# amathislab/HOISDF

Hardware: AMD Instinct MI355X
Metric: samples/sec (img + 2048 SDF queries) fwd+bwd at 1/2/4/8 MI355X (higher is better)
Workload: dtype f32 (emulated contractions, f32 accumulate, f16x2 form: operands as scaled hi + lo f16 pieces x 3 products - 22 operand bits, one power-of-two scale per ROW of a linear layer's row operand, per (sample, head) of the attention operands, per weight matrix; the attention backward's dS as three pieces x

## Files before the change

### hoisdf_amd/_lib.py

```python
from __future__ import annotations

import ctypes as C
import os
from typing import Dict, List

_HERE = os.path.dirname(os.path.abspath(__file__))
LIB_PATH = os.environ.get("HOISDF_LIB", os.path.join(_HERE, "libhoisdf_hip.so"))
HEADER_PATH = os.path.join(os.path.dirname(_HERE), "include", "hoisdf.h")
MAX_LEVELS = 8


class HoisdfLibraryError(RuntimeError):
    pass


class HoisdfError(RuntimeError):
    def __init__(self, code: int, msg: str):
        super().__init__(f"libhoisdf_hip status {code}: {msg}")
        self.code = code


class Pyramid(C.Structure):
    _fields_ = [("n_levels", C.c_int), ("B", C.c_int), ("data", C.c_void_p * MAX_LEVELS),
                ("C", C.c_int * MAX_LEVELS), ("H", C.c_int * MAX_LEVELS), ("W", C.c_int * MAX_LEVELS)]
# ... 7 lines not shown
                ("emu_img", C.c_void_p * 6), ("emu_img_t", C.c_void_p * 6)]


class EncoderLayerDesc(C.Structure):
    _fields_ = [("B", C.c_int), ("S", C.c_int), ("E", C.c_int), ("F", C.c_int), ("H", C.c_int), ("n_query", C.c_int),
                ("n_inter", C.c_int), ("eps", C.c_float), ("drop_p", C.c_float), ("seed", C.c_uint64 * 4), ("attention", C.c_int),
                ("attention_bwd_emulated", C.c_int), ("training", C.c_int), ("x_mag", C.c_void_p)]


_ENC_W = ("w_in", "b_in", "w_out", "b_out", "g1", "be1", "w1", "b1", "w2", "b2", "g2", "be2", "g3", "be3")
_ENC_IMG = ("img_in", "img_in_q", "img_in_kv", "img_out", "img_1", "img_2")


class EncoderLayerWeights(C.Structure):
    _fields_ = [(n, C.c_void_p) for n in _ENC_W + _ENC_IMG + tuple(n.replace("img_", "img_t_") for n in _ENC_IMG)]


class DecoderLayerDesc(C.Structure):
    _fields_ = [("B", C.c_int), ("Q", C.c_int), ("S", C.c_int), ("E", C.c_int), ("F", C.c_int), ("H", C.c_int), ("kv_len", C.c_int),
                ("eps", C.c_float), ("drop_p", C.c_float), ("seed", C.c_uint64 * 6), ("training", C.c_int)]


_DEC_W = ("sa_w_in", "sa_b_in", "sa_w_out", "sa_b_out", "ca_w_in", "ca_b_in", "ca_w_out", "ca_b_out", "w1", "b1", "w2", "b2",
          "g1", "be1", "g2", "be2", "g3", "be3", "g4", "be4")


class DecoderLayerWeights(C.Structure):
    _fields_ = [(n, C.c_void_p) for n in _DEC_W + ("img_ca_kv", "img_t_ca_kv")]


class DecoderLayerGrads(C.Structure):
    _fields_ = [("d" + n, C.c_void_p) for n in _DEC_W]


class EncoderLayerGrads(C.Structure):
    _fields_ = [("d" + n, C.c_void_p) for n in _ENC_W]


_SDF_G = ("d_sdfin_w0", "d_sdfin_b0", "d_sdfin_w1", "d_sdfin_b1", "d_dec_w0", "d_dec_b0", "d_dec_w1", "d_dec_b1", "d_dec_w2", "d_dec_b2",
          "d_dec_w3", "d_dec_b3", "d_dec_w4", "d_dec_b4")


class SdfWeightGrads(C.Structure):
    _fields_ = [(n, C.c_void_p) for n in _SDF_G]


MLP_MAX_LAYERS = 4


class Mlp(C.Structure):
    _fields_ = [("n_layers", C.c_int), ("act_last", C.c_int), ("dims", C.c_int * (MLP_MAX_LAYERS + 1)),
                ("w", C.c_void_p * MLP_MAX_LAYERS), ("b", C.c_void_p * MLP_MAX_LAYERS),
                ("img", C.c_void_p * MLP_MAX_LAYERS), ("img_t", C.c_void_p * MLP_MAX_LAYERS)]


class EmuPrepItem(C.Structure):
    _fields_ = [("W", C.c_void_p), ("image", C.c_void_p), ("first_block", C.c_long), ("ldw", C.c_int), ("N", C.c_int),
                ("K", C.c_int), ("transpose", C.c_int)]


class MlpGrads(C.Structure):
    _fields_ = [("dw", C.c_void_p * MLP_MAX_LAYERS), ("db", C.c_void_p * MLP_MAX_LAYERS)]


POSE_MAX_LAYERS = 12


class PoseDesc(C.Structure):
    _fields_ = [("B", C.c_int), ("num_samp_hand", C.c_int), ("num_samp_obj", C.c_int), ("bins_n", C.c_int), ("img_h", C.c_int),
                ("img_w", C.c_int), ("hand_sdf_scale", C.c_float), ("obj_sdf_scale", C.c_float), ("clamping_distance", C.c_float),
                ("hidden_dim", C.c_int), ("nheads", C.c_int), ("dim_feedforward", C.c_int), ("enc_layers", C.c_int),
                ("dec_layers", C.c_int), ("C", C.c_int), ("use_inverse_kinematics", C.c_int), ("pre_norm", C.c_int),
                ("classifier_branch", C.c_int), ("attention", C.c_int)]


class SdfDecoderParams(C.Structure):
    _fields_ = [("weight_v", C.c_void_p * 4), ("weight_g", C.c_void_p * 4), ("bias", C.c_void_p * 4),
                ("linh4_weight", C.c_void_p), ("linh4_bias", C.c_void_p)]


class PoseWeights(C.Structure):
    _fields_ = [("linear_sdfin", Mlp), ("hand_sdf_decoder", SdfDecoderParams), ("obj_sdf_decoder", SdfDecoderParams),
                ("linear_transformerin", Mlp), ("hand_sigmoid_beta", C.c_void_p), ("obj_sigmoid_beta", C.c_void_p),
                ("hand_encoder", EncoderLayerWeights * POSE_MAX_LAYERS), ("obj_encoder", EncoderLayerWeights * POSE_MAX_LAYERS),
                ("hand_decoder", DecoderLayerWeights * POSE_MAX_LAYERS), ("mano_query_embed", C.c_void_p),
                ("linear_pose", Mlp), ("linear_shape", Mlp), ("linear_handvote", Mlp), ("linear_handcls", Mlp),
                ("linear_obj_rot", Mlp), ("linear_obj_rel_trans", Mlp),
                ("mano_shapedirs", C.c_void_p), ("mano_posedirs", C.c_void_p), ("mano_weights", C.c_void_p),
                ("mano_v_template", C.c_void_p), ("mano_j_regressor", C.c_void_p), ("mano_hands_mean", C.c_void_p)]


class EncoderDesc(C.Structure):
    _fields_ = [("B", C.c_int), ("img_h", C.c_int), ("img_w", C.c_int), ("resnet_type", C.c_int), ("big_decoder", C.c_int)]


_POSE_OUT = ("hand_joints_out", "obj_rot_out", "obj_trans_out", "mano_mesh_out", "mano_joints_out", "mano_shape_out",
             "hand_points_out", "obj_points_out", "hand_sdf_out", "obj_sdf_out")


class PoseOutputs(C.Structure):
    _fields_ = [(n, C.c_void_p) for n in _POSE_OUT]


_P, _I, _L, _F, _U64, _D = C.c_void_p, C.c_int, C.c_long, C.c_float, C.c_uint64, C.c_double
_PYR = C.POINTER(Pyramid)
_SDFW = C.POINTER(SdfWeights)

SIGNATURES: Dict[str, List] = {
    "hoisdf_project_gather_fwd": [_PYR, _P, _P, _L, _I, _P, _P, _F, _I, _I, _P, _I, _P, _P, _P],
    "hoisdf_project_gather_bwd": [_PYR, _P, _P, _L, _I, _P, _P, _F, _I, _I, _P, _I, _P],
    "hoisdf_linear_fwd": [_P, _I, _P, _I, _P, _P, _I, _L, _I, _I, _I, _F, _U64, _P, _P],
    "hoisdf_linear_bwd_input": [_P, _I, _P, _F, _P, _I, _P, _I, _L, _I, _I, _I, _P],
    "hoisdf_linear_bwd_weight": [_P, _I, _P, _F, _P, _I, _P, _I, _P, _L, _I, _I, _P, _L, _P],
    "hoisdf_linear_emu_prepare": [_P, _I, _I, _I, _I, _P, _P],
    "hoisdf_linear_emu_prepare_batch": [_P, _I, _L, _P],
    "hoisdf_linear_fwd_emu": [_P, _I, _P, _P, _P, _I, _L, _I, _I, _I, _F, _U64, _P, _P],
    "hoisdf_mag_measure": [_P, _L, _L, _I, _P, _P],
    "hoisdf_head_mag_measure": [_P, _L, _L, _I, _I, _P, _P],
    "hoisdf_linear_fwd_emu_heads": [_P, _I, _P, _P, _P, _I, _L, _I, _I, _P, _P, _P, _I, _P],
    "hoisdf_linear_bwd_input_emu_heads": [_P, _I, _P, _P, _I, _L, _I, _I, _P, _P, _P, _I, _P],
    "hoisdf_linear_fwd_emu_mag": [_P, _I, _P, _P, _P, _I, _L, _I, _I, _I, _F, _U64, _P, _P, _P, _P],
    "hoisdf_linear_bwd_input_emu": [_P, _I, _P, _F, _P, _P, _I, _L, _I, _I, _I, _P],
    "hoisdf_linear_bwd_input_emu_mag": [_P, _I, _P, _F, _P, _P, _I, _L, _I, _I, _I, _P, _P, _P],
    "hoisdf_linear_fwd_emu_small": [_P, _I, _P, _I, _P, _P, _I, _L, _I, _I, _I, _F, _U64, _P, _P],
    "hoisdf_linear_bwd_input_emu_small": [_P, _I, _P, _F, _P, _I, _P, _I, _L, _I, _I, _I, _P],
    "hoisdf_linear_bwd_weight_emu_small": [_P, _I, _P, _F, _P, _I, _P, _I, _P, _L, _I, _I, _P],
    "hoisdf_linear_bwd_weight_emu": [_P, _I, _P, _F, _P, _I, _P, _I, _P, _L, _I, _I, _P, _L, _P],
    "hoisdf_linear_bwd_weight_emu_mag": [_P, _I, _P, _F, _P, _I, _P, _I, _P, _L, _I, _I, _P, _L, _P, _P, _P],
    "hoisdf_relu_dropout_bwd": [_P, _I, _P, _I, _P, _I, _L, _I, _F, _P],
    "hoisdf_posenc_fwd": [_P, _L, _P, _I, _I, _P, _P],
    "hoisdf_sdf_query_fwd": [_PYR, _P, _P, _L, _I, _P, _P, _F, _I, _I, _P, _P, _SDFW, _F, _F, _U64, _P, _P, _P, _P, _P, _L, _P],
    "hoisdf_weightnorm_fwd": [_P, _P, _P, _I, _P, _I, _I, _P],
    "hoisdf_weightnorm_bwd": [_P, _P, _P, _I, _P, _P, _I, _I, _P],
    "hoisdf_sdf_head_fwd": [_P, _I, _P, _P, _P, _P, _L, _I, _F, _P],
    "hoisdf_sdf_head_bwd": [_P, _P, _P, _I, _P, _P, _I, _P, _P, _L, _I, _F, _P],
    "hoisdf_lattice_count": [_P, _P, _P, _F, _I, _I, _P, _P],
    "hoisdf_lattice_fill": [_P, _P, _P, _F, _I, _I, _P, _P, _P, _P, _P],
    "hoisdf_select_smallest_abs": [_P, _P, _P, _I, _I, _P, _P],
    "hoisdf_gather_rows": [_P, _I, _P, _L, _I, _P, _I, _P],
    "hoisdf_sdf_sample_keys": [_P, _I, _P, _P, _P, _P, _I, _I, _F, _U64, _P, _P, _P],
    "hoisdf_adamw_step": [_P, _I, _D, _D, _D, _D, _D, _L, _F, _P],
    "hoisdf_aux_image_losses_fwd": [_P, _L, _L, _L, _L, _P, _P, _P, _I, _I, _I, _I, _F, _P, _P, _P, _P, _P],
    "hoisdf_aux_image_losses_bwd": [_P, _L, _L, _L, _L, _P, _P, _P, _P, _P, _P, _I, _I, _I, _P, _P],
    "hoisdf_bn_stats": [_P, _L, _L, _I, _P, _P, _P, _P, _F, _F, _P, _L, _P],
    "hoisdf_bn_apply_fwd": [_P, _L, _P, _L, _P, _P, _I, _F, _P, _P, _I, _P, _P, _L, _I, _P],
    "hoisdf_bn_bwd": [_P, _L, _P, _L, _P, _P, _P, _P, _P, _P, _P, _P, _L, _I, _P, _L, _P],
    "hoisdf_token_build_fwd": [_P, _P, _P, _P, _I, _P, _P, _P, _I, _I, _I, _I, _I, _P],
    "hoisdf_token_build_bwd": [_P, _P, _I, _P, _P, _P, _I, _P, _I, _I, _I, _I, _I, _P],
    "hoisdf_token_build_bwd_ordered": [_P, _P, _I, _P, _P, _P, _I, _P, _P, _I, _I, _I, _I, _I, _P],
    "hoisdf_attention_fwd": [_P, _I, _P, _I, _P, _I, _P, _I, _P, _I, _I, _I, _I, _I, _F, _U64, _P],
    "hoisdf_attention_bwd": [_P, _I, _P, _I, _P, _I, _P, _I, _P, _I, _P, _P, _P, _P, _P, _I, _I, _I, _I,
                             _I, _F, _U64, _P],
    "hoisdf_attention_fwd_bf16x2": [_P, _I, _P, _I, _P, _I, _P, _I, _I, _I, _I, _I, _I, _P, _L, _P],
    "hoisdf_attention_fwd_emu": [_P, _I, _P, _I, _P, _I, _P, _I, _P, _I, _I, _I, _I, _I, _F, _U64, _P, _L, _I, _P],
    "hoisdf_attention_fwd_emu_mag": [_P, _I, _P, _I, _P, _I, _P, _I, _P, _I, _I, _I, _I, _I, _F, _U64, _P, _L, _I, _P, _P, _P, _P, _P],
    "hoisdf_attention_bwd_emu": [_P, _I, _P, _I, _P, _I, _P, _I, _P, _I, _P, _P, _P, _P, _P, _I, _I, _I, _I, _I, _F, _U64, _P, _P,
                                 _L, _P],
    "hoisdf_attention_bwd_emu_mag": [_P, _I, _P, _I, _P, _I, _P, _I, _P, _I, _P, _P, _P, _P, _P, _I, _I, _I, _I, _I, _F, _U64, _P, _P,
                                 _L, _P, _P, _P, _P, _P, _P],
    "hoisdf_attention_small_fwd": [_P, _I, _P, _I, _P, _I, _P, _P, _I, _P, _I, _I, _I, _I, _F, _U64, _P],
    "hoisdf_attention_small_bwd": [_P, _I, _P, _I, _P, _I, _P, _P, _I, _P, _P, _P, _I, _I, _I, _I, _F,
                                   _U64, _P],
    "hoisdf_add_layernorm_fwd": [_P, _P, _P, _P, _P, _P, _P, _L, _I, _F, _F, _U64, _P],
    "hoisdf_add_layernorm_bwd": [_P, _P, _P, _P, _P, _P, _P, _P, _P, _P, _P, _L, _I, _F, _U64, _P],
    "hoisdf_residual_dropout": [_P, _P, _P, _L, _I, _F, _U64, _P],
    "hoisdf_layernorm_rows_fwd": [_P, _P, _P, _P, _P, _P, _L, _I, _I, _I, _F, _P],
    "hoisdf_layernorm_rows_bwd": [_P, _P, _P, _P, _P, _P, _P, _P, _P, _L, _I, _I, _I, _P],
    "hoisdf_sdf_query_train_fwd": [_PYR, _P, _P, _L, _I, _P, _P, _F, _I, _I, _SDFW, _F, _F, _U64, _P, _P, _P, _P, _L, _P, _L, _P],
    "hoisdf_sdf_query_bwd": [_PYR, _P, _P, _L, _I, _P, _P, _F, _I, _I, _SDFW, _F, _F, _P, _L, _P, _P, _P, _L, _P],
    "hoisdf_sdf_infer_count": [_P, _P, _P, _F, _I, _I, _P, _P, _P, _P],
    "hoisdf_sdf_infer_count_begin": [_P, _P, _P, _F, _I, _I, _P, _P, _P],
    "hoisdf_sdf_infer": [_PYR, _P, _P, _P, _F, _I, _I, _P, _P, _I, _I, _I, _SDFW, _F, _F, _U64, _P, _P, _P, _P, _L, _P],
    "hoisdf_decoder_layer_fwd": [_P, _P, _P, _P, _P, _P, _P, _P, _P, _L, _P, _L, _P],
    "hoisdf_decoder_layer_bwd": [_P, _P, _P, _P, _P, _P, _P, _L, _P, _P, _P, _P, _I, _P, _P, _P, _L, _P],
    "hoisdf_encoder_layer_fwd": [_P, _P, _P, _P, _P, _P, _L, _P, _L, _P],
    "hoisdf_encoder_layer_bwd": [_P, _P, _P, _P, _P, _L, _P, _P, _P, _P, _P, _L, _P],
    "hoisdf_mano_prepare": [_P, _P, _P, _P, _P],
    "hoisdf_mano_head_fwd": [_P, _I, _I, _P, _I, _I, _P, _P, _P, _P, _P, _P, _P, _P, _P, _I, _I, _P, _P, _P, _P, _P],
    "hoisdf_mano_head_bwd": [_P, _P, _I, _P, _P, _P, _P, _P, _P, _P, _P, _P, _I, _I, _P, _P, _P, _P, _P, _P, _P],
# ... 115 lines not shown
```

### hoisdf_amd/csrc/attention_emu.hip

```cpp
#include "attention_emu.h"

namespace hoisdf {
using namespace emu_attn;

namespace {
constexpr int RP = 72;
constexpr int TPH = 36;
constexpr int ROWS_T = 32 * RP;
constexpr int TRN_T = 64 * TPH;
constexpr float QS2 = 0.125f * 1.4426950408889634f;
#define CR(r, h) (((r) & 3) + 8 * ((r) >> 2) + 4 * (h))
#define MB(a, b, c) __builtin_amdgcn_mfma_f32_32x32x16_bf16((a), (b), (c), 0, 0, 0)
#define MB6(acc, x0, x1, x2, y0, y1, y2) \
  do {                                   \
    acc = MB(x2, y0, acc);               \
    acc = MB(x0, y2, acc);               \
    acc = MB(x1, y1, acc);               \
    acc = MB(x1, y0, acc);               \
    acc = MB(x0, y1, acc);               \
    acc = MB(x0, y0, acc);               \
  } while (0)

#define SPLIT1(x, i)                             \
  do {                                           \
    const __bf16 a_ = (__bf16)(x);               \
    const float r1_ = (x) - (float)a_;           \
    const __bf16 b_ = (__bf16)r1_;               \
    const float r2_ = r1_ - (float)b_;           \
    p0[i] = a_; p1[i] = b_; p2[i] = (__bf16)r2_; \
  } while (0)

__device__ __forceinline__ u32x4 ld_rows(const __bf16* base, size_t row0, int tid) {
  return *reinterpret_cast<const u32x4*>(base + (row0 + (tid >> 3)) * D + (tid & 7) * 8);
}
__device__ __forceinline__ void st_rows(__bf16* lds, const u32x4 v, int tid) {
  *reinterpret_cast<u32x4*>(lds + (tid >> 3) * RP + (tid & 7) * 8) = v;
}
__device__ __forceinline__ u32x4 ld_trn(const __bf16* base, size_t Lp, size_t col0, int tid) {
  return *reinterpret_cast<const u32x4*>(base + (size_t)(tid >> 2) * Lp + col0 + (tid & 3) * 8);
}
__device__ __forceinline__ void st_trn(__bf16* lds, const u32x4 v, int tid) {
  u32x2* p = reinterpret_cast<u32x2*>(lds + (tid >> 2) * TPH + (tid & 3) * 8);
  p[0] = u32x2{v.x, v.y};
  p[1] = u32x2{v.z, v.w};
}
__device__ __forceinline__ bf16x8 frag_trn(const __bf16* tile, int row, int jj, int h) {
  const bf16x4 a = *reinterpret_cast<const bf16x4*>(tile + row * TPH + 16 * jj + 4 * h);
  const bf16x4 b = *reinterpret_cast<const bf16x4*>(tile + row * TPH + 16 * jj + 8 + 4 * h);
  return bf16x8{a[0], a[1], a[2], a[3], b[0], b[1], b[2], b[3]};
}
}

template <bool F16>
__global__ __launch_bounds__(256) void emu_attn_convert_kernel(const float* __restrict__ src, int ld, int L, int Lp, int B, int H,
                                                               float scale, __bf16* __restrict__ r0, __bf16* __restrict__ r1,
                                                               __bf16* __restrict__ r2, __bf16* __restrict__ t0,
                                                               __bf16* __restrict__ t1, __bf16* __restrict__ t2,
                                                               const uint32_t* __restrict__ mag) {
  constexpr int TP = 72;
  __shared__ __attribute__((aligned(16))) __bf16 tile[3][64 * TP];
  const int tid = threadIdx.x;
  const int nb = Lp / 64;
  const int kb = blockIdx.x % nb, bh = blockIdx.x / nb, b = bh / H, head = bh - b * H;
  if (F16) { f16_saturate_on(); scale *= mag_scale(mag[head * B + b]); }
  const int r = tid >> 2, dc = (tid & 3) * 16;
  const int row = kb * 64 + r;
  const bool valid = row < L;
  const float* sr = src + ((size_t)b * L + (valid ? row : 0)) * ld + head * D + dc;
  bf16x8 pa[2][3];
#pragma unroll
  for (int i = 0; i < 2; ++i) {
    float4 u = valid ? *reinterpret_cast<const float4*>(sr + 8 * i) : make_float4(0.f, 0.f, 0.f, 0.f);
    float4 w = valid ? *reinterpret_cast<const float4*>(sr + 8 * i + 4) : make_float4(0.f, 0.f, 0.f, 0.f);
    u.x *= scale; u.y *= scale; u.z *= scale; u.w *= scale;
    w.x *= scale; w.y *= scale; w.z *= scale; w.w *= scale;
    if (F16) {
      const float e_[8] = {u.x, u.y, u.z, u.w, w.x, w.y, w.z, w.w};
      f16x8 hi, lo;
#pragma unroll
      for (int j = 0; j < 8; ++j) { hi[j] = (_Float16)e_[j]; lo[j] = (_Float16)(e_[j] - (float)hi[j]); }
      pa[i][0] = __builtin_bit_cast(bf16x8, hi); pa[i][1] = __builtin_bit_cast(bf16x8, lo); pa[i][2] = pa[i][1];
    } else {
      bf16x8 p0, p1, p2;
      SPLIT1(u.x, 0); SPLIT1(u.y, 1); SPLIT1(u.z, 2); SPLIT1(u.w, 3);
      SPLIT1(w.x, 4); SPLIT1(w.y, 5); SPLIT1(w.z, 6); SPLIT1(w.w, 7);
      pa[i][0] = p0; pa[i][1] = p1; pa[i][2] = p2;
    }
  }
  if (r0) {
    const size_t o = ((size_t)bh * Lp + row) * D + dc;
#pragma unroll
    for (int i = 0; i < 2; ++i) {
      *reinterpret_cast<bf16x8*>(r0 + o + 8 * i) = pa[i][0];
      *reinterpret_cast<bf16x8*>(r1 + o + 8 * i) = pa[i][1];
      if (!F16 && r2) *reinterpret_cast<bf16x8*>(r2 + o + 8 * i) = pa[i][2];
    }
  }
  if (t0) {
#pragma unroll
    for (int i = 0; i < 2; ++i)
#pragma unroll
      for (int e = 0; e < 8; ++e) {
        tile[0][(dc + 8 * i + e) * TP + r] = pa[i][0][e];
        tile[1][(dc + 8 * i + e) * TP + r] = pa[i][1][e];
        if (!F16) tile[2][(dc + 8 * i + e) * TP + r] = pa[i][2][e];
      }
    __syncthreads();
    const int d = tid >> 2, rc = (tid & 3) * 16;
    const size_t o = ((size_t)bh * D + d) * Lp + kb * 64 + rc;
#pragma unroll
    for (int i = 0; i < 2; ++i) {
      *reinterpret_cast<u32x4*>(t0 + o + 8 * i) = *reinterpret_cast<const u32x4*>(&tile[0][d * TP + rc + 8 * i]);
      *reinterpret_cast<u32x4*>(t1 + o + 8 * i) = *reinterpret_cast<const u32x4*>(&tile[1][d * TP + rc + 8 * i]);
      if (!F16 && t2) *reinterpret_cast<u32x4*>(t2 + o + 8 * i) = *reinterpret_cast<const u32x4*>(&tile[2][d * TP + rc + 8 * i]);
    }
  }
}

template <bool DROP, int NPL, bool F16>
__global__ __launch_bounds__(256, 2) void emu_attn_fwd2_kernel(EmuAttn a) {
  static_assert(!F16 || NPL == 2, "the f16 form has two planes");
  __shared__ __attribute__((aligned(16))) __bf16 Kb0[3 * ROWS_T];
  __shared__ __attribute__((aligned(16))) __bf16 Kb1[3 * ROWS_T];
  __shared__ __attribute__((aligned(16))) __bf16 Vb0[3 * TRN_T];
  __shared__ __attribute__((aligned(16))) __bf16 Vb1[3 * TRN_T];
  const int tid = threadIdx.x, lane = tid & 63, wave = tid >> 6;
  const int h = lane >> 5, c = lane & 31;
  int qtile, bh;
  if (!emu_block((a.Lq + 127) / 128, a.B * a.H, qtile, bh)) return;
  const int b = bh / a.H, head = bh - b * a.H;
  const int qrow = qtile * 128 + wave * 32 + c;
  const __bf16* kp[3] = {a.k[0] + (size_t)bh * a.Lkp * D, a.k[1] + (size_t)bh * a.Lkp * D, a.k[NPL == 3 ? 2 : 1] + (size_t)bh * a.Lkp * D};
  const __bf16* vp[3] = {a.vt[0] + (size_t)bh * D * a.Lkp, a.vt[1] + (size_t)bh * D * a.Lkp, a.vt[NPL == 3 ? 2 : 1] + (size_t)bh * D * a.Lkp};
  float cs = 1.f, vinv = 1.f;
  constexpr float PB = F16 ? 6.f : 0.f;
  if (F16) {
    f16_saturate_on();
    const float iq_ = mag_inv_scale(a.q_hm[head * a.B + b]), ik_ = mag_inv_scale(a.k_hm[head * a.B + b]);
    cs = fmaxf(iq_ * ik_, 0x1p-100f); vinv = mag_inv_scale(a.v_hm[head * a.B + b]);
  }
// ... 159 lines not shown
    if ((t) + 1 <= lastt) FWD2_TILE_STATS((t) + 1, false);                \
    s_cur = s_nxt;                                                                                                     \
    __syncthreads();                                                                                                     \
  } while (0)
  int t = 0;
  for (; t + 1 < ntiles; t += 2) {
    FWD2_ITER(t, Kb1, Kb0, Vb0, Vb1);
    FWD2_ITER(t + 1, Kb0, Kb1, Vb1, Vb0);
  }
  if (t < ntiles) FWD2_ITER(t, Kb1, Kb0, Vb0, Vb1);
#undef KFRAG
#undef VFRAG
#undef PE1
#undef PE2
#undef PE3
#undef PE4
#undef PM
#undef PH1
#undef PH2
#undef PH3
#undef STK
#undef STV
#undef LDK
#undef LDV
#undef FWD2_S
#undef FWD2_PV
#undef FWD2_S2
#undef FWD2_PV2
#undef PE3B
#undef FWD2_TILE_STATS
#undef FWD2_ITER
  const float ltot = lsum + __shfl_xor(lsum, 32, 64);
  uint32_t omax = 0u;
  if (qrow < a.Lq) {
    const float inv = vinv / ltot;
    float* op = a.out + ((size_t)b * a.Lq + qrow) * a.ldo + head * D;
#pragma unroll
    for (int tt = 0; tt < 2; ++tt)
#pragma unroll
      for (int g = 0; g < 4; ++g) {
        const float4 ov = make_float4(o[tt][4 * g + 0] * inv, o[tt][4 * g + 1] * inv, o[tt][4 * g + 2] * inv, o[tt][4 * g + 3] * inv);
        *reinterpret_cast<float4*>(op + 32 * tt + 8 * g + 4 * h) = ov;
        omax = max(omax, mag_bits4(ov));
      }
    if (h == 0 && a.lse) a.lse[(size_t)bh * a.Lq + qrow] = (F16 ? m * cs - PB : m) + log2f(ltot);
  }
  if (a.mag) {
    omax = max(omax, (uint32_t)__shfl_xor((int)omax, 32, 64));
    if (h == 0 && qrow < a.Lq) atomicMax(a.mag + (size_t)b * a.Lq + qrow, omax);
  }
}
#pragma pop_macro("MB")

__global__ __launch_bounds__(256) void emu_attn_delta_kernel(const float* __restrict__ o, int ldo, const float* __restrict__ dout,
                                                             int lddo, float* __restrict__ delta, int B, int H, int Lq) {
  const long g = ((long)blockIdx.x * 256 + threadIdx.x) >> 4;
  const int l16 = threadIdx.x & 15;
  if (g >= (long)B * Lq * H) return;
  const int head = (int)(g % H);
  const long bq = g / H;
  const int q = (int)(bq % Lq), b = (int)(bq / Lq);
  const float4 x = *reinterpret_cast<const float4*>(o + ((size_t)b * Lq + q) * ldo + head * D + l16 * 4);
  const float4 y = *reinterpret_cast<const float4*>(dout + ((size_t)b * Lq + q) * lddo + head * D + l16 * 4);
  float s = x.x * y.x + x.y * y.y + x.z * y.z + x.w * y.w;
#pragma unroll
  for (int off = 8; off > 0; off >>= 1) s += __shfl_xor(s, off, 16);
  if (l16 == 0) delta[((size_t)b * H + head) * Lq + q] = s;
}

__global__ __launch_bounds__(256) void emu_attn_dq_reduce_kernel(const float* __restrict__ part, int nkb, float* __restrict__ dq,
                                                                 int ldq, int B, int H, int Lq, uint32_t* __restrict__ mag,
                                                                 const float* __restrict__ scale) {
  const long i = (long)(gridDim.x - 1 - blockIdx.x) * 256 + threadIdx.x;
  const long n = (long)B * H * Lq * 16;
  uint32_t qmax = 0u;
  if (i < n) {
    const int d4 = (int)(i & 15);
    const long bq = i >> 4;
    const int q = (int)(bq % Lq);
    const int bh = (int)(bq / Lq), b = bh / H, head = bh - b * H;
    const size_t stride = (size_t)B * H * Lq * D;
    const float* p = part + ((size_t)bh * Lq + q) * D + d4 * 4;
    float4 s = *reinterpret_cast<const float4*>(p);
    for (int k0 = 1; k0 < nkb; k0 += 8) {
      f32x4 v[8];
#pragma unroll
      for (int j = 0; j < 8; ++j)
        v[j] = k0 + j < nkb ? __builtin_nontemporal_load(reinterpret_cast<const f32x4*>(p + (size_t)(k0 + j) * stride)) : f32x4{0.f, 0.f, 0.f, 0.f};
#pragma unroll
      for (int j = 0; j < 8; ++j)
        if (k0 + j < nkb) { s.x += v[j].x; s.y += v[j].y; s.z += v[j].z; s.w += v[j].w; }
    }
    const float sc = scale ? scale[bh] : 0.125f;
    const float4 r = make_float4(s.x * sc, s.y * sc, s.z * sc, s.w * sc);
    *reinterpret_cast<float4*>(dq + ((size_t)b * Lq + q) * ldq + head * D + d4 * 4) = r;
    qmax = mag_bits4(r);
    if (mag) {
      qmax = group_max_u32<16>(qmax);
      if (d4 == 0) atomicMax(mag + (size_t)b * Lq + q, qmax);
    }
  }
}

}

using namespace hoisdf;

namespace {
inline long pad128(long L) { return (L + 127) / 128 * 128; }
inline size_t plane_elems(int B, int H, long Lp) { return (size_t)B * H * Lp * 64; }

struct Planes { __bf16 *r[3], *t[3]; };
inline Planes carve(__bf16*& w, size_t n, bool rows, bool trn, int npl = 3) {
  Planes p{};
  for (int i = 0; i < npl; ++i) { p.r[i] = rows ? w : nullptr; if (rows) w += n; }
  for (int i = 0; i < npl; ++i) { p.t[i] = trn ? w : nullptr; if (trn) w += n; }
  return p;
}
struct QkvPlaneSet { Planes q, k, v; };
inline QkvPlaneSet carve_qkv(__bf16*& w, int B, int H, int Lq, int Lk, bool v_rows, bool v_trn, int npl = 3) {
  const size_t nq = plane_elems(B, H, pad128(Lq)), nk = plane_elems(B, H, pad128(Lk));
  QkvPlaneSet s;
  s.q = carve(w, nq, true, false, npl);
  s.k = carve(w, nk, true, false, npl);
  s.v = carve(w, nk, v_rows, v_trn, npl);
  return s;
}
inline QkvPlaneSet fwd_planes(void* workspace, int B, int H, int Lq, int Lk, int keep) {
  __bf16* w = reinterpret_cast<__bf16*>(workspace);
  return carve_qkv(w, B, H, Lq, Lk, keep != 0, true);
}
inline EmuAttn emu_args(int B, int H, int Lq, int Lk, int kv_len, float drop_p, uint64_t seed) {
  EmuAttn a{};
  a.B = B; a.H = H; a.Lq = Lq; a.Lk = Lk; a.Lqp = (int)pad128(Lq); a.Lkp = (int)pad128(Lk); a.kv_len = kv_len;
  a.drop_p = drop_p; a.inv_keep = 1.f / (1.f - drop_p); a.thresh = drop_threshold(drop_p); a.seed = seed;
  return a;
}
int convert(const float* src, int ld, int L, int Lp, int B, int H, float scale, const Planes& p, hipStream_t st, const uint32_t* mag = nullptr) {
  const long nblk = (long)B * H * (Lp / 64);
  if (mag) hipLaunchKernelGGL(emu_attn_convert_kernel<true>, dim3((unsigned)nblk), dim3(256), 0, st, src, ld, L, Lp, B, H, scale, p.r[0], p.r[1],
                              p.r[2], p.t[0], p.t[1], p.t[2], mag);
  else hipLaunchKernelGGL(emu_attn_convert_kernel<false>, dim3((unsigned)nblk), dim3(256), 0, st, src, ld, L, Lp, B, H, scale, p.r[0], p.r[1],
                          p.r[2], p.t[0], p.t[1], p.t[2], mag);
  return check_launch("attention_emu_convert");
}
int convert_qkv(const float* q, int ldq, const float* k, int ldk, const float* v, int ldv, int B, int H, int Lq, int Lk, const QkvPlaneSet& s,
                hipStream_t st, const uint32_t* q_hm = nullptr, const uint32_t* k_hm = nullptr, const uint32_t* v_hm = nullptr) {
  if (int rc = convert(q, ldq, Lq, (int)pad128(Lq), B, H, QS2, s.q, st, q_hm)) return rc;
  if (int rc = convert(k, ldk, Lk, (int)pad128(Lk), B, H, 1.f, s.k, st, k_hm)) return rc;
  return convert(v, ldv, Lk, (int)pad128(Lk), B, H, 1.f, s.v, st, v_hm);
}
int check_emu(const void* q, const void* k, const void* v, int ldq, int ldk, int ldv, int B, int H, int Lq, int Lk, int kv_len,
              float drop_p, const char* who) {
  HOISDF_REQUIRE(q && k && v, HOISDF_ERR_INVALID, "%s: null pointer", who);
  HOISDF_REQUIRE(B > 0 && H > 0 && Lq > 0 && Lk > 0 && kv_len > 0 && kv_len <= Lk, HOISDF_ERR_INVALID,
                 "%s: bad sizes B=%d H=%d Lq=%d Lk=%d kv_len=%d", who, B, H, Lq, Lk, kv_len);
  HOISDF_REQUIRE(ldq >= H * 64 && ldk >= H * 64 && ldv >= H * 64 && ((ldq | ldk | ldv) & 3) == 0 &&
                     (((uintptr_t)q | (uintptr_t)k | (uintptr_t)v) & 15) == 0,
                 HOISDF_ERR_INVALID, "%s: leading dims must be multiples of 4 and >= H*64, pointers 16-byte aligned", who);
  HOISDF_REQUIRE(drop_p >= 0.f && drop_p < 1.f, HOISDF_ERR_INVALID, "%s: drop_p=%f", who, drop_p);
  return HOISDF_OK;
}
}

extern "C" long hoisdf_attention_emu_workspace(int B, int H, int Lq, int Lk, int mode) {
  if (B <= 0 || H <= 0 || Lq <= 0 || Lk <= 0) return 0;
  const size_t q = plane_elems(B, H, pad128(Lq)), k = plane_elems(B, H, pad128(Lk));
  const size_t planes = mode == 0 ? 3 * q + 6 * k : 3 * q + 9 * k;
  return (long)(planes * sizeof(__bf16));
}

namespace {
int fwd_over_planes(float* o, int ldo, float* lse, int B, int H, int Lq, int Lk, int kv_len, float drop_p, uint64_t seed,
                    void* workspace, int keep, hipStream_t st, uint32_t* o_mag, const uint32_t* q_hm = nullptr, const uint32_t* k_hm = nullptr,
                    const uint32_t* v_hm = nullptr) {
  const QkvPlaneSet s = fwd_planes(workspace, B, H, Lq, Lk, keep);
  EmuAttn a = emu_args(B, H, Lq, Lk, kv_len, drop_p, seed);
  for (int i = 0; i < 3; ++i) { a.q[i] = s.q.r[i]; a.k[i] = s.k.r[i]; a.vt[i] = s.v.t[i]; }
  a.out = o; a.lse = lse; a.ldo = ldo; a.mag = o_mag; a.q_hm = q_hm; a.k_hm = k_hm; a.v_hm = v_hm;
  const dim3 fgrid(cdiv(Lq, 128) * 8 * cdiv(B * H, 8));
  if (q_hm) {
    HOISDF_REQUIRE(drop_p < 0.75f, HOISDF_ERR_INVALID, "attention_fwd_emu (f16x2 form): drop_p = %f, must be below 0.75", drop_p);
    if (drop_p > 0.f) hipLaunchKernelGGL((emu_attn_fwd2_kernel<true, 2, true>), fgrid, dim3(256), 0, st, a);
    else hipLaunchKernelGGL((emu_attn_fwd2_kernel<false, 2, true>), fgrid, dim3(256), 0, st, a);
  } else if (drop_p > 0.f) hipLaunchKernelGGL((emu_attn_fwd2_kernel<true, 3, false>), fgrid, dim3(256), 0, st, a);
  else hipLaunchKernelGGL((emu_attn_fwd2_kernel<false, 3, false>), fgrid, dim3(256), 0, st, a);
  return check_launch("attention_fwd_emu");
}
}

extern "C" int hoisdf_attention_fwd_emu(const float* q, int ldq, const float* k, int ldk, const float* v, int ldv, float* o,
                                        int ldo, float* lse, int B, int H, int Lq, int Lk, int kv_len, float drop_p,
                                        uint64_t seed, void* workspace, long workspace_bytes, int keep, void* stream) {
  return attention_fwd_emu_mag(q, ldq, k, ldk, v, ldv, o, ldo, lse, B, H, Lq, Lk, kv_len, drop_p, seed, workspace, workspace_bytes, keep,
                               nullptr, stream, nullptr, nullptr, nullptr);
}
extern "C" int hoisdf_attention_fwd_emu_mag(const float* q, int ldq, const float* k, int ldk, const float* v, int ldv, float* o,
                                            int ldo, float* lse, int B, int H, int Lq, int Lk, int kv_len, float drop_p,
                                            uint64_t seed, void* workspace, long workspace_bytes, int keep, const uint32_t* q_mag,
                                            const uint32_t* k_mag, const uint32_t* v_mag, uint32_t* o_mag, void* stream) {
  HOISDF_REQUIRE(q_mag && k_mag && v_mag, HOISDF_ERR_INVALID, "attention_fwd_emu_mag: the head magnitudes of q, k and v are required (hoisdf_head_mag_measure)");
  return attention_fwd_emu_mag(q, ldq, k, ldk, v, ldv, o, ldo, lse, B, H, Lq, Lk, kv_len, drop_p, seed, workspace, workspace_bytes, keep,
                               o_mag, stream, q_mag, k_mag, v_mag);
// ... 62 lines not shown
  const size_t q = plane_elems(B, H, pad128(Lq)), k = plane_elems(B, H, pad128(Lk));
  size_t bytes = 3 * q * sizeof(__bf16) + (size_t)cdiv(Lk, 128) * B * H * Lq * 64 * sizeof(float);
  if (!kept) bytes += (3 * q + 6 * k) * sizeof(__bf16);
  return (long)bytes;
}

extern "C" int hoisdf_attention_bwd_emu(const float* q, int ldq, const float* k, int ldk, const float* v, int ldv, const float* o,
                                        int ldo, const float* dout, int lddo, const float* lse, float* delta, float* dq, float* dk,
                                        float* dv, int B, int H, int Lq, int Lk, int kv_len, float drop_p, uint64_t seed,
                                        const void* fwd_workspace, void* workspace, long workspace_bytes, void* stream) {
  return attention_bwd_emu_mag(q, ldq, k, ldk, v, ldv, o, ldo, dout, lddo, lse, delta, dq, dk, dv, B, H, Lq, Lk, kv_len, drop_p, seed,
                               fwd_workspace, workspace, workspace_bytes, nullptr, stream, nullptr, nullptr, nullptr, nullptr);
}
extern "C" int hoisdf_attention_bwd_emu_mag(const float* q, int ldq, const float* k, int ldk, const float* v, int ldv, const float* o,
                                            int ldo, const float* dout, int lddo, const float* lse, float* delta, float* dq, float* dk,
                                            float* dv, int B, int H, int Lq, int Lk, int kv_len, float drop_p, uint64_t seed,
                                            const void* fwd_workspace, void* workspace, long workspace_bytes, const uint32_t* q_mag,
                                            const uint32_t* k_mag, const uint32_t* v_mag, const uint32_t* do_mag, uint32_t* g_mag, void* stream) {
  HOISDF_REQUIRE(q_mag && k_mag && v_mag && do_mag, HOISDF_ERR_INVALID, "attention_bwd_emu_mag: the head magnitudes of q, k, v and of dout are required");
  return attention_bwd_emu_mag(q, ldq, k, ldk, v, ldv, o, ldo, dout, lddo, lse, delta, dq, dk, dv, B, H, Lq, Lk, kv_len, drop_p, seed,
                               fwd_workspace, workspace, workspace_bytes, g_mag, stream, q_mag, k_mag, v_mag, do_mag);
}
int hoisdf::attention_bwd_emu_mag(const float* q, int ldq, const float* k, int ldk, const float* v, int ldv, const float* o, int ldo,
                                  const float* dout, int lddo, const float* lse, float* delta, float* dq, float* dk, float* dv, int B,
                                  int H, int Lq, int Lk, int kv_len, float drop_p, uint64_t seed, const void* fwd_workspace,
                                  void* workspace, long workspace_bytes, uint32_t* g_mag, void* stream, const uint32_t* q_hm,
                                  const uint32_t* k_hm, const uint32_t* v_hm, const uint32_t* do_hm) {
  const bool h2 = q_hm && k_hm && v_hm && do_hm;
  HOISDF_REQUIRE(h2 || (!q_hm && !k_hm && !v_hm && !do_hm), HOISDF_ERR_INVALID, "attention_bwd_emu: head magnitudes of all of q, k, v, dout or of none");
  HOISDF_REQUIRE(!g_mag || Lq == Lk, HOISDF_ERR_INVALID, "attention_bwd_emu: one row-magnitude array for dq, dk, dv needs Lq == Lk");
  HOISDF_REQUIRE(!h2 || drop_p < 0.75f, HOISDF_ERR_INVALID, "attention_bwd_emu (f16x2 form): drop_p = %f, must be below 0.75 (as in the forward)", drop_p);
  if (int rc = check_emu(fwd_workspace && !q ? o : q, fwd_workspace && !k ? o : k, fwd_workspace && !v ? o : v, ldq, ldk, ldv, B, H, Lq,
                         Lk, kv_len, drop_p, "attention_bwd_emu")) return rc;
  HOISDF_REQUIRE(o && dout && lse && delta && dq && dk && dv && workspace, HOISDF_ERR_INVALID, "attention_bwd_emu: null pointer");
  HOISDF_REQUIRE(ldo >= H * 64 && lddo >= H * 64 && ((ldo | lddo) & 3) == 0 &&
                     (((uintptr_t)o | (uintptr_t)dout | (uintptr_t)dq | (uintptr_t)dk | (uintptr_t)dv | (uintptr_t)workspace |
                       (uintptr_t)fwd_workspace) & 15) == 0,
                 HOISDF_ERR_INVALID, "attention_bwd_emu: bad leading dims / alignment");
  const long need = hoisdf_attention_bwd_emu_workspace(B, H, Lq, Lk, fwd_workspace ? 1 : 0);
  HOISDF_REQUIRE(workspace_bytes >= need, HOISDF_ERR_WORKSPACE, "attention_bwd_emu: workspace %ld < %ld bytes", workspace_bytes, need);
  hipStream_t st = as_stream(stream);
  __bf16* w = reinterpret_cast<__bf16*>(workspace);
  const Planes pd = carve(w, plane_elems(B, H, pad128(Lq)), true, false);
  float* part = reinterpret_cast<float*>(w);
  w += (size_t)cdiv(Lk, 128) * B * H * Lq * 64 * 2;
  QkvPlaneSet s;
  if (fwd_workspace) {
    __bf16* f = reinterpret_cast<__bf16*>(const_cast<void*>(fwd_workspace));
    s = carve_qkv(f, B, H, Lq, Lk, true, true);
  } else {
    s = carve_qkv(w, B, H, Lq, Lk, true, false);
    if (int rc = convert_qkv(q, ldq, k, ldk, v, ldv, B, H, Lq, Lk, s, st, q_hm, k_hm, v_hm)) return rc;
  }
  if (int rc = convert(dout, lddo, Lq, (int)pad128(Lq), B, H, 1.f, pd, st, do_hm)) return rc;
  const long ng = (long)B * Lq * H;
  hipLaunchKernelGGL(emu_attn_delta_kernel, dim3((unsigned)((ng * 16 + 255) / 256)), dim3(256), 0, st, o, ldo, dout, lddo, delta, B, H, Lq);
  if (int rc = check_launch("attention_emu_delta")) return rc;
  EmuAttn a = emu_args(B, H, Lq, Lk, kv_len, drop_p, seed);
  for (int i = 0; i < 3; ++i) { a.q[i] = s.q.r[i]; a.k[i] = s.k.r[i]; a.v[i] = s.v.r[i]; a.d[i] = pd.r[i]; }
  a.lse_in = lse; a.delta = delta; a.dq_part = part; a.dk = dk; a.dv = dv; a.ldk = ldk; a.ldv = ldv; a.mag = g_mag;
  if (h2) {
    a.q_hm = q_hm; a.k_hm = k_hm; a.v_hm = v_hm; a.d_hm = do_hm;
    a.dq_scale = reinterpret_cast<float*>(pd.r[2]);
  }
  if (int rc = h2 ? attention_bwd4h_emu_launch(a, st) : attention_bwd4_emu_launch(a, st)) return rc;
  const long n4 = (long)B * H * Lq * 16;
  hipLaunchKernelGGL(emu_attn_dq_reduce_kernel, dim3((unsigned)((n4 + 255) / 256)), dim3(256), 0, st, part, cdiv(kv_len, 128), dq, ldq,
                     B, H, Lq, g_mag, (const float*)(h2 ? a.dq_scale : nullptr));
  return check_launch("attention_bwd_emu dq reduce");
}
```

### hoisdf_amd/csrc/chain.h

```cpp
#pragma once
#include <stdlib.h>

#include <mutex>
#include <unordered_map>

#include "common.h"

namespace hoisdf {
namespace {

constexpr long EMU_MIN_ROWS = 2048;
constexpr long EMU_DW_MIN_ROWS = 8192;

inline bool al16(const void* p) { return (reinterpret_cast<uintptr_t>(p) & 15) == 0; }

struct Bump {
  char* base; long cap; long off = 0; bool overflow = false;
  Bump(void* b, long c) : base(static_cast<char*>(b)), cap(c) {}
  void* take(long bytes) {
    off = (off + 255) & ~255L;
    const long at = off;
    off += bytes;
    if (!base) return nullptr;
    if (off > cap) { overflow = true; return nullptr; }
    return base + at;
  }
  float* floats(long n) { return static_cast<float*>(take(n * 4)); }
};

struct SavedMags {
  std::mutex mu;
  std::unordered_map<const void*, int> on;
  void put(const void* key, bool v) { if (!key) return; std::lock_guard<std::mutex> l(mu); if (on.size() > 8192) on.clear(); on[key] = v ? 1 : 0; }
  int get(const void* key) { std::lock_guard<std::mutex> l(mu); auto it = on.find(key); return it == on.end() ? -1 : it->second; }
};
inline SavedMags& saved_mags() { static SavedMags s; return s; }

struct Ctx {
  hipStream_t st; void* stream;
  Bump* ws;
  bool dry;
  bool emu;
  int rc = HOISDF_OK;
  bool ok() const { return rc == HOISDF_OK; }
};

inline bool emu_small(const Ctx& c, long M, const float* a, long lda, const float* W, long ldw, int N, int K) {
  if (!c.emu || M > hoisdf_linear_emu_small_max_rows() || N % 4 || K % 4 || lda % 4 || ldw % 4) return false;
  return c.dry || hoisdf_linear_emu_small_supported(a, lda, W, ldw, M, N, K);
}
bool emu_rows(const Ctx& c, long M, const float* a, long lda, int contraction) {
  return c.emu && M >= EMU_MIN_ROWS && contraction % 4 == 0 && lda % 4 == 0 && (c.dry || al16(a));
}
const void* image_of(Ctx& c, const void* given, const float* W, int ldw, int N, int K, int transpose) {
  if (given) return given;
  void* img = c.ws->take(hoisdf_linear_emu_image_bytes(transpose ? K : N, transpose ? N : K));
  if (c.dry) return nullptr;
  if (!img) { c.rc = HOISDF_ERR_WORKSPACE; return nullptr; }
  c.rc = hoisdf_linear_emu_prepare(W, ldw, N, K, transpose, img, c.stream);
  return img;
}
void lin_fwd(Ctx& c, const float* x, int ldx, const float* W, int ldw, const void* img, const float* b, float* y, int ldy, long M, int N,
             int K, int act, float p, uint64_t seed, uint32_t* bits, int K_pad = 0, const uint32_t* x_mag = nullptr, uint32_t* y_mag = nullptr,
             uint32_t* y_heads = nullptr, int head_L = 0) {
  if (!c.ok()) return;
  if (K_pad < K || (K_pad + 15) / 16 != (K + 15) / 16) K_pad = K;
  if (emu_rows(c, M, x, ldx, K_pad)) {
    const void* im = image_of(c, img, W, ldw, N, K, 0);
    if (c.dry || !c.ok()) return;
    c.rc = linear_fwd_emu_mag(x, ldx, im, b, y, ldy, M, N, K_pad, act, p, seed, bits, x_mag, y_mag, c.stream, y_heads, head_L);
    return;
  }
  if (c.dry) return;
  if (emu_small(c, M, x, ldx, W, ldw, N, K)) { c.rc = hoisdf_linear_fwd_emu_small(x, ldx, W, ldw, b, y, ldy, M, N, K, act, p, seed, bits, c.stream); return; }
  c.rc = hoisdf_linear_fwd(x, ldx, W, ldw, b, y, ldy, M, N, K, act, p, seed, bits, c.stream);
}
void lin_bwd_input(Ctx& c, const float* dy, int lddy, const uint32_t* bits, float p, const float* W, int ldw, const void* img_t, float* dx,
                   int lddx, long M, int N, int K, int accumulate, const uint32_t* dy_mag = nullptr, uint32_t* dx_mag = nullptr,
                   uint32_t* dx_heads = nullptr, int head_L = 0) {
  if (!c.ok()) return;
  if (!bits) p = 0.f;
  if (emu_rows(c, M, dy, lddy, N)) {
    const void* im = image_of(c, img_t, W, ldw, N, K, 1);
    if (c.dry || !c.ok()) return;
    c.rc = linear_bwd_input_emu_mag(dy, lddy, bits, p, im, dx, lddx, M, N, K, accumulate, dy_mag, accumulate ? nullptr : dx_mag, c.stream,
                                    accumulate ? nullptr : dx_heads, head_L);
    return;
  }
  if (c.dry) return;
  if (emu_small(c, M, dy, lddy, W, ldw, N, K)) { c.rc = hoisdf_linear_bwd_input_emu_small(dy, lddy, bits, p, W, ldw, dx, lddx, M, N, K, accumulate, c.stream); return; }
  c.rc = hoisdf_linear_bwd_input(dy, lddy, bits, p, W, ldw, dx, lddx, M, N, K, accumulate, c.stream);
}
void lin_bwd_weight(Ctx& c, const float* dy, int lddy, const uint32_t* bits, float p, const float* x, int ldx, float* dW, float* db, long M,
                    int N, int K, int K_pad = 0, const uint32_t* dy_mag = nullptr, const uint32_t* x_mag = nullptr) {
  if (!c.ok()) return;
  if (!bits) p = 0.f;
  if (K_pad < K) K_pad = K;
  const bool emu = c.emu && M >= EMU_DW_MIN_ROWS && (N < K ? N : K) >= 64 && N % 4 == 0 && K_pad % 4 == 0 && lddy % 4 == 0 && ldx % 4 == 0 &&
                   (c.dry || (al16(dy) && al16(x) && al16(dW)));
  if (emu) {
    const long nws = hoisdf_linear_bwd_weight_emu_workspace(M, N, K_pad);
    float* w = c.ws->floats(nws > 4 ? nws : 4);
    if (!c.dry) {
      if (!w) { c.rc = HOISDF_ERR_WORKSPACE; return; }
      if (dy_mag || x_mag) c.rc = linear_bwd_weight_emu_mag(dy, lddy, bits, p, x, ldx, dW, K_pad, db, M, N, K_pad, w, nws, dy_mag, x_mag, c.stream);
      else c.rc = hoisdf_linear_bwd_weight_emu(dy, lddy, bits, p, x, ldx, dW, K_pad, db, M, N, K_pad, w, nws, c.stream);
    }
    return;
  }
  if (c.emu && M <= hoisdf_linear_emu_small_max_rows()) {
    if (!c.dry) c.rc = hoisdf_linear_bwd_weight_emu_small(dy, lddy, bits, p, x, ldx, dW, K_pad, db, M, N, K_pad, c.stream);
    return;
  }
  long nws = 0; float* w = nullptr;
  if (deterministic_mode()) {
    nws = hoisdf_linear_bwd_weight_workspace(M, N, K_pad);
    if (nws > 0) w = c.ws->floats(nws);
    if (!c.dry && nws > 0 && !w) { c.rc = HOISDF_ERR_WORKSPACE; return; }
  }
  if (c.dry) return;
  c.rc = hoisdf_linear_bwd_weight(dy, lddy, bits, p, x, ldx, dW, K_pad, db, M, N, K_pad, w, nws, c.stream);
}


}
}
```

### hoisdf_amd/csrc/common.h

```cpp
#pragma once
#include <hip/hip_runtime.h>
#include <stdint.h>

#include "../../include/hoisdf.h"

namespace hoisdf {

void set_error(const char* fmt, ...);
int check_launch(const char* what);

#define HOISDF_REQUIRE(cond, code, ...)                 \
  do {                                                  \
    if (!(cond)) {                                      \
      ::hoisdf::set_error(__VA_ARGS__);                 \
      return (code);                                    \
    }                                                   \
  } while (0)

static inline hipStream_t as_stream(void* s) { return reinterpret_cast<hipStream_t>(s); }
static inline int cdiv(long a, long b) { return (int)((a + b - 1) / b); }

__device__ __forceinline__ uint32_t mix32(uint32_t x) {
  x ^= x >> 16; x *= 0x7feb352dU; x ^= x >> 15; x *= 0x846ca68bU; x ^= x >> 16;
  return x;
// ... 39 lines not shown
                          long workspace_bytes, uint32_t* g_mag, void* stream, const uint32_t* q_hm = nullptr,
                          const uint32_t* k_hm = nullptr, const uint32_t* v_hm = nullptr, const uint32_t* do_hm = nullptr);

bool emu_form_h2();
int emu_rowmag_launch(const float* x, long ld, long M, int K, uint32_t* words, hipStream_t st);
int emu_mag_measure(const float* x, long ld, long M, int K, uint32_t* words, hipStream_t st);
int emu_headmag_launch(const float* x, long ld, long M, int groups, int L, uint32_t* words, hipStream_t st);
uint32_t* mag_scratch(hipStream_t st, long words);

__device__ __forceinline__ uint32_t mag_bits(float v) { return __builtin_bit_cast(uint32_t, v) & 0x7fffffffu; }
__device__ __forceinline__ uint32_t mag_bits4(const float4& v) {
  return max(max(mag_bits(v.x), mag_bits(v.y)), max(mag_bits(v.z), mag_bits(v.w)));
}
__device__ __forceinline__ void f16_saturate_on() { __builtin_amdgcn_s_setreg((0 << 11) | (23 << 6) | 1, 1); }
__device__ __forceinline__ void rowmag_publish_wave(uint32_t* words, long row, uint32_t m);
template <int CTRL>
__device__ __forceinline__ uint32_t dpp_u32(uint32_t v) { return (uint32_t)__builtin_amdgcn_update_dpp(0, (int)v, CTRL, 0xf, 0xf, true); }
template <int G>
__device__ __forceinline__ uint32_t group_max_u32(uint32_t m) {
  static_assert(G == 4 || G == 8 || G == 16 || G == 32 || G == 64, "group size");
  m = max(m, dpp_u32<0xB1>(m));
  m = max(m, dpp_u32<0x4E>(m));
  if (G >= 8) m = max(m, dpp_u32<0x141>(m));
  if (G >= 16) m = max(m, dpp_u32<0x140>(m));
  if (G >= 32) m = max(m, (uint32_t)__shfl_xor((int)m, 16, 64));
  if (G >= 64) m = max(m, (uint32_t)__shfl_xor((int)m, 32, 64));
  return m;
}
__device__ __forceinline__ void rowmag_publish_wave(uint32_t* words, long row, uint32_t m) {
  if (!words) return;
  m = group_max_u32<64>(m);
  if ((threadIdx.x & 63) == 0) atomicMax(words + row, m);
}
__device__ __forceinline__ uint32_t mag_exp(uint32_t amax_bits) { return min(max((amax_bits >> 23) & 0xffu, 14u), 254u); }
__device__ __forceinline__ float mag_scale(uint32_t amax_bits) { return __builtin_bit_cast(float, (267u - mag_exp(amax_bits)) << 23); }
__device__ __forceinline__ float mag_inv_scale(uint32_t amax_bits) { return __builtin_bit_cast(float, (mag_exp(amax_bits) - 13u) << 23); }
__device__ __forceinline__ uint32_t block_max_u32(uint32_t v, uint32_t* red4) {
#pragma unroll
  for (int o = 32; o >= 1; o >>= 1) v = max(v, (uint32_t)__shfl_xor((int)v, o));
  if ((threadIdx.x & 63) == 0) red4[threadIdx.x >> 6] = v;
  __syncthreads();
  return max(max(red4[0], red4[1]), max(red4[2], red4[3]));
}
__device__ __forceinline__ long head_words(long groups, long nb) { return groups * nb; }
int linear_fwd_emu_mag(const float* x, int ldx, const void* w_image, const float* bias, float* y, int ldy, long M, int N, int K, int act,
                       float drop_p, uint64_t seed, uint32_t* relu_bits, const uint32_t* x_mag, uint32_t* y_mag, void* stream,
                       uint32_t* y_heads = nullptr, int head_L = 0);
int linear_bwd_input_emu_mag(const float* dy, int lddy, const uint32_t* relu_bits, float drop_p, const void* wt_image, float* dx, int lddx,
                             long M, int N, int K, int accumulate, const uint32_t* dy_mag, uint32_t* dx_mag, void* stream,
                             uint32_t* dx_heads = nullptr, int head_L = 0);
int linear_bwd_weight_emu_mag(const float* dy, int lddy, const uint32_t* relu_bits, float drop_p, const float* x, int ldx, float* dW, int lddw,
                              float* db, long M, int N, int K, float* workspace, long workspace_floats, const uint32_t* dy_mag,
                              const uint32_t* x_mag, void* stream);
int project_gather_fwd_mag(const hoisdf_pyramid* pyr, const float* points, const int32_t* sample_idx, long n_rows, int rows_per_sample,
                           const float* center, const float* cam_intr, float scale, int img_h, int img_w, float* feat, int ldf, float* cam_out,
                           float* uv_out, uint32_t* feat_mag, void* stream);
int posenc_fwd_mag(const float* points, long n_rows, float* x0, int ldx0, int col0, float* pe, uint32_t* x0_mag, void* stream);
int sdf_head_bwd_mag(const float* dsdf, const float* sdf_raw, const float* h, int ldh, const float* w, float* dh, int lddh, float* dw,
                     float* db, long n_rows, int K, float clamp, uint32_t* dh_mag, void* stream);
int add_layernorm_fwd_mag(const float* x, const float* r, const float* gamma, const float* beta, float* y, float* mean, float* rstd, long M,
                          int D, float eps, float drop_p, uint64_t seed, uint32_t* y_mag, void* stream);
int add_layernorm_bwd_mag(const float* dy, const float* x, const float* r, const float* gamma, const float* mean, const float* rstd,
                          const float* dx_add, float* dx, float* dr, float* dgamma, float* dbeta, long M, int D, float drop_p, uint64_t seed,
                          uint32_t* dx_mag, uint32_t* dr_mag, void* stream);

struct ConvProblem {
  int B, H, W, C_in, C_out, KH, KW, stride, pad, act;
  int transposed;
};
struct ConvPlan {
  int tile;
  int splitk, k_per_split;
  long workspace_bytes;
};
ConvPlan conv_plan(long M, int N, int K, int ncls);
int conv_launch(const ConvProblem& c, const float* x, int ldx, const float* w_packed, const float* bias, const float* residual, int ldr,
                float* y, int ldy, int c_off, void* workspace, long workspace_bytes, hipStream_t st);
int conv_pack_launch(const float* w, const float* conv_bias, const float* gamma, const float* beta, const float* mean, const float* var,
                     float eps, int C_out, int C_in, int KH, int KW, int transposed, float* packed, float* bias_out, hipStream_t st);
int maxpool_launch(const float* x, int ldx, float* y, int ldy, int B, int H, int W, int C, hipStream_t st);

bool deterministic_mode();
bool gemm_emu_mode();
struct DetScratch {
  float* part;
  unsigned* ticket;
  int on;
};
DetScratch det_scratch(size_t floats);

__device__ __forceinline__ void block_column_sum(float* dstA, int nA, float* dstB, int nB,
                                                 const float* src, unsigned* s_last ,
                                                 const DetScratch ds) {
  const int n = nA + nB;
  if (!ds.on) {
    for (int c = threadIdx.x; c < n; c += blockDim.x) atomicAdd(c < nA ? dstA + c : dstB + (c - nA), src[c]);
    return;
  }
  for (int c = threadIdx.x; c < n; c += blockDim.x) ds.part[(size_t)blockIdx.x * n + c] = src[c];
  __threadfence();
  __syncthreads();
  if (threadIdx.x == 0) *s_last = (atomicAdd(ds.ticket, 1u) == gridDim.x - 1) ? 1u : 0u;
  __syncthreads();
  if (!*s_last) return;
  __threadfence();
  const volatile float* part = ds.part;
// ... 32 lines not shown
```

### hoisdf_amd/csrc/gemm_emu.h

```cpp
#pragma once
#include "common.h"

namespace hoisdf {

typedef float f32x16 __attribute__((ext_vector_type(16)));
typedef float f32x4 __attribute__((ext_vector_type(4)));
typedef float f32x2 __attribute__((ext_vector_type(2)));
typedef __bf16 bf16x8 __attribute__((ext_vector_type(8)));
typedef __bf16 bf16x2 __attribute__((ext_vector_type(2)));
typedef _Float16 f16x8 __attribute__((ext_vector_type(8)));
typedef _Float16 f16x2 __attribute__((ext_vector_type(2)));
typedef unsigned int u32x4 __attribute__((ext_vector_type(4)));
typedef unsigned int u32x2 __attribute__((ext_vector_type(2)));
#define MFB(a, b, c) __builtin_amdgcn_mfma_f32_32x32x16_bf16((a), (b), (c), 0, 0, 0)
#define MFH(a, b, c) __builtin_amdgcn_mfma_f32_32x32x16_f16((a), (b), (c), 0, 0, 0)

constexpr int TM = 256, TN = 128, KS = 16, NT = 256;
constexpr int WN = TN / 2, NJ = WN / 32;
constexpr int A_U4 = 3 * 2 * TM, B_U4 = 3 * 2 * TN, STAGE_U4 = A_U4 + B_U4;
constexpr int NB = B_U4 / NT;
constexpr int HTM = 256, HTN = 256;
constexpr int HA_U4 = 2 * 2 * HTM, HB_U4 = 2 * 2 * HTN;
constexpr int H_TRAILER = 128;
constexpr int DT = 256;
// ... 276 lines not shown
#pragma unroll
        for (int r = 0; r < 16; ++r) {
          const int row = rbase + i * 32 + (r & 3) + 8 * (r >> 2);
          uint32_t mb = 0u;
#pragma unroll
          for (int j = 0; j < NJ_; ++j) if (cbase + j * 32 < g.N) mb = max(mb, mag_bits(acc[i][j][r]));
          mb = group_max_u32<32>(mb);
          if (l31 == 0 && row < g.M) atomicMax(g.amax_out + row, mb);
        }
    }
  }
  if (g.bits_out) {
    uint32_t wd[2][NJ_];
#pragma unroll
    for (int hh = 0; hh < 2; ++hh)
#pragma unroll
      for (int j = 0; j < NJ_; ++j) wd[hh][j] = 0u;
#pragma unroll
    for (int i = 0; i < 4; ++i)
#pragma unroll
      for (int r = 0; r < 16; ++r) {
        const int rl = (i & 1) * 32 + (r & 3) + 8 * (r >> 2);
#pragma unroll
        for (int j = 0; j < NJ_; ++j) {
          const unsigned long long q = __ballot(acc[i][j][r] > 0.f);
          if (lane == rl) wd[i >> 1][j] = (uint32_t)q;
          if (lane == rl + 4) wd[i >> 1][j] = (uint32_t)(q >> 32);
        }
      }
    const int wcol = (n0 + wn * WN_) >> 5;
    const int nvalid = g.N - (n0 + wn * WN_);
#pragma unroll
    for (int hh = 0; hh < 2; ++hh) {
      const int row = m0 + wm * 128 + hh * 64 + lane;
      if (row < g.M) {
#pragma unroll
        for (int j = 0; j < NJ_; ++j) {
          const int nv = nvalid - 32 * j;
          if (nv > 0) g.bits_out[(size_t)row * g.ldbits_out + wcol + j] = nv >= 32 ? wd[hh][j] : (wd[hh][j] & ((1u << nv) - 1u));
        }
      }
    }
  }
}

int emu_b3_prepare(const float* W, int ldw, int R, int Kc, int transpose, void* image, hipStream_t st);
int emu_b3_prepare_batch(const hoisdf_emu_prep_item* d_items, int n, long total_blocks, hipStream_t st);
int emu_b3_launch(EmuArgs g, hipStream_t st);
int emu_h2_prepare(const float* W, int ldw, int N, int K, int transpose, void* image, hipStream_t st);
int emu_h2_prepare_batch(const hoisdf_emu_prep_item* d_items, int n, long total_blocks, hipStream_t st);
int emu_h2_launch(EmuArgs g, hipStream_t st);
int dw_tile(int K);
void plan_dw(long M, int N, int K, int& splitk, int& mper);
int emu_dw_launch(const DwArgs& g, bool h2, float* dW, float* db, float* workspace, hipStream_t st);
}
```

### hoisdf_amd/csrc/gemm_emu.hip

```cpp
#include <stdlib.h>

#include <map>
#include <mutex>
#include <unordered_map>
#include <utility>

#include "gemm_emu.h"

namespace hoisdf {

__global__ __launch_bounds__(256) void emu_rowmag_kernel(const float* __restrict__ x, long ld, long M, int K, uint32_t* __restrict__ words) {
  constexpr int RPW = 8;
  const int lane = threadIdx.x & 63;
  const long row0 = ((long)blockIdx.x * 4 + (threadIdx.x >> 6)) * RPW;
  const int k4 = K >> 2;
  uint32_t m[RPW];
#pragma unroll
  for (int r = 0; r < RPW; ++r) {
    m[r] = 0u;
    if (row0 + r < M)
      for (int c = lane; c < k4; c += 64) {
        const u32x4 v = *reinterpret_cast<const u32x4*>(x + (row0 + r) * ld + 4 * c);
        m[r] = max(m[r], max(max(v[0] & 0x7fffffffu, v[1] & 0x7fffffffu), max(v[2] & 0x7fffffffu, v[3] & 0x7fffffffu)));
      }
// ... 200 lines not shown
  HOISDF_REQUIRE(y_heads, HOISDF_ERR_INVALID, "linear_fwd_emu_heads: y_heads is required");
  return linear_fwd_emu_mag(x, ldx, w_image, bias, y, ldy, M, N, K, 0, 0.f, 0, nullptr, x_mag, y_mag, stream, y_heads, L);
}
extern "C" int hoisdf_linear_bwd_input_emu_heads(const float* dy, int lddy, const void* wt_image, float* dx, int lddx, long M, int N, int K,
                                                 const uint32_t* dy_mag, uint32_t* dx_mag, uint32_t* dx_heads, int L, void* stream) {
  HOISDF_REQUIRE(dx_heads, HOISDF_ERR_INVALID, "linear_bwd_input_emu_heads: dx_heads is required");
  return linear_bwd_input_emu_mag(dy, lddy, nullptr, 0.f, wt_image, dx, lddx, M, N, K, 0, dy_mag, dx_mag, stream, dx_heads, L);
}
extern "C" int hoisdf_linear_bwd_input_emu(const float* dy, int lddy, const uint32_t* relu_bits, float drop_p,
                                           const void* wt_image, float* dx, int lddx, long M, int N, int K, int accumulate,
                                           void* stream) {
  return linear_bwd_input_emu_mag(dy, lddy, relu_bits, drop_p, wt_image, dx, lddx, M, N, K, accumulate, nullptr, nullptr, stream);
}
extern "C" int hoisdf_linear_bwd_input_emu_mag(const float* dy, int lddy, const uint32_t* relu_bits, float drop_p,
                                               const void* wt_image, float* dx, int lddx, long M, int N, int K, int accumulate,
                                               const uint32_t* dy_mag, uint32_t* dx_mag, void* stream) {
  return linear_bwd_input_emu_mag(dy, lddy, relu_bits, drop_p, wt_image, dx, lddx, M, N, K, accumulate, dy_mag, dx_mag, stream);
}

int hoisdf::linear_bwd_input_emu_mag(const float* dy, int lddy, const uint32_t* relu_bits, float drop_p, const void* wt_image, float* dx,
                                     int lddx, long M, int N, int K, int accumulate, const uint32_t* dy_mag, uint32_t* dx_mag,
                                     void* stream, uint32_t* dx_heads, int head_L) {
  HOISDF_REQUIRE(M == 0 || (dy && wt_image && dx), HOISDF_ERR_INVALID, "linear_bwd_input_emu: null pointer");
  HOISDF_REQUIRE(M >= 0 && N > 0 && K > 0 && lddy >= N && lddx >= K && M < (1L << 31) && drop_p >= 0.f && drop_p < 1.f,
                 HOISDF_ERR_INVALID, "linear_bwd_input_emu: bad sizes");
  if (M == 0) return HOISDF_OK;
  HOISDF_REQUIRE(hoisdf_linear_emu_supported(dy, lddy, N), HOISDF_ERR_INVALID,
                 "linear_bwd_input_emu: dy must be 16-byte aligned with lddy and N multiples of 4");
  EmuArgs g{};
  g.A = dy; g.lda = lddy; g.Bimg = static_cast<const u32x4*>(wt_image);
  g.abits = relu_bits; g.ldbits = (N + 31) / 32; g.ascale = 1.f / (1.f - drop_p);
  g.C = dx; g.ldc = lddx; g.M = (int)M; g.N = K; g.K = N;
  g.inv_keep = 1.f;
  g.beta = accumulate ? 1 : 0;
  g.a_amax = dy_mag; g.amax_out = dx_mag;
  if (dx_heads) {
    HOISDF_REQUIRE(head_L > 0 && K % 64 == 0 && !accumulate, HOISDF_ERR_INVALID, "linear_bwd_input_emu: head magnitudes need K %% 64 == 0, the rows per sample, no accumulation");
    g.head_out = dx_heads; g.head_L = head_L; g.head_nb = cdiv(M, head_L);
  }
  return launch_emu(g, as_stream(stream));
}

extern "C" long hoisdf_linear_bwd_weight_emu_workspace(long M, int N, int K) {
  if (M <= 0 || N <= 0 || K <= 0) return 0;
  int splitk, mper;
  plan_dw(M, N, K, splitk, mper);
  if (splitk <= 1) return 0;
  return (long)splitk * ((long)N * K + N);
}

namespace {
int bwd_weight_emu(const float* dy, int lddy, const uint32_t* relu_bits, float drop_p, const float* x, int ldx, float* dW, int lddw,
                   float* db, long M, int N, int K, float* workspace, long workspace_floats, bool h2, const uint32_t* dy_mag,
                   const uint32_t* x_mag, void* stream) {
  HOISDF_REQUIRE(dW && (M == 0 || (dy && x)), HOISDF_ERR_INVALID, "linear_bwd_weight_emu: null pointer");
  HOISDF_REQUIRE(M > 0 && N > 0 && K > 0 && lddy >= N && ldx >= K && lddw == K && M < (1L << 31) && drop_p >= 0.f && drop_p < 1.f,
                 HOISDF_ERR_INVALID, "linear_bwd_weight_emu: bad sizes (a dense dW, lddw == K, is required)");
  HOISDF_REQUIRE(al16(dy) && al16(x) && al16(dW) && (lddy % 4 == 0) && (ldx % 4 == 0) && (N % 4 == 0) && (K % 4 == 0),
                 HOISDF_ERR_INVALID, "linear_bwd_weight_emu: operands must be 16-byte aligned with N, K and leading dims multiples of 4");
  hipStream_t st = as_stream(stream);
  DwArgs g{};
  g.dy = dy; g.lddy = lddy; g.x = x; g.ldx = ldx;
  g.bits = relu_bits; g.ldbits = (N + 31) / 32; g.ascale = 1.f / (1.f - drop_p);
  g.M = (int)M; g.N = N; g.K = K;
  const int dtk = dw_tile(K);
  g.tiles_n = cdiv(N, DT); g.tiles_k = cdiv(K, dtk);
  plan_dw(M, N, K, g.splitk, g.m_per_split);
  const long need = g.splitk > 1 ? (long)g.splitk * ((long)N * K + N) : 0;
  HOISDF_REQUIRE(need == 0 || (workspace && workspace_floats >= need && al16(workspace)), HOISDF_ERR_WORKSPACE,
                 "linear_bwd_weight_emu: workspace of %ld floats needed", need);
  if (g.splitk > 1) {
    g.C = workspace; g.c_split_stride = (long)N * K;
    g.colsum = db ? workspace + (size_t)g.splitk * N * K : nullptr; g.colsum_split_stride = N;
  } else {
    g.C = dW; g.c_split_stride = 0; g.colsum = db; g.colsum_split_stride = 0;
  }
  if (dtk == 256 && h2) {
    g.dy_amax = dy_mag; g.x_amax = x_mag;
    if (!dy_mag) {
      uint32_t* part = mag_scratch(st, M);
      if (!part) { set_error("linear_bwd_weight_emu: cannot allocate the row magnitudes"); return HOISDF_ERR_LAUNCH; }
      mag_trace("grad-weight dy", M, N);
      if (int rc = emu_rowmag_launch(dy, lddy, M, N, part, st)) return rc;
      g.dy_amax = part;
    }
    if (!x_mag) {
      uint32_t* part = mag_scratch(st, M);
      if (!part) { set_error("linear_bwd_weight_emu: cannot allocate the row magnitudes"); return HOISDF_ERR_LAUNCH; }
      mag_trace("grad-weight x", M, K);
      if (int rc = emu_rowmag_launch(x, ldx, M, K, part, st)) return rc;
      g.x_amax = part;
    }
  }
  return emu_dw_launch(g, h2, dW, db, workspace, st);
}
}

extern "C" int hoisdf_linear_bwd_weight_emu(const float* dy, int lddy, const uint32_t* relu_bits, float drop_p, const float* x,
                                            int ldx, float* dW, int lddw, float* db, long M, int N, int K, float* workspace,
                                            long workspace_floats, void* stream) {
  return bwd_weight_emu(dy, lddy, relu_bits, drop_p, x, ldx, dW, lddw, db, M, N, K, workspace, workspace_floats, false, nullptr, nullptr, stream);
}
int hoisdf::linear_bwd_weight_emu_mag(const float* dy, int lddy, const uint32_t* relu_bits, float drop_p, const float* x, int ldx,
                                      float* dW, int lddw, float* db, long M, int N, int K, float* workspace, long workspace_floats,
                                      const uint32_t* dy_mag, const uint32_t* x_mag, void* stream) {
  return bwd_weight_emu(dy, lddy, relu_bits, drop_p, x, ldx, dW, lddw, db, M, N, K, workspace, workspace_floats, form_h2(), dy_mag, x_mag, stream);
}
extern "C" int hoisdf_linear_bwd_weight_emu_mag(const float* dy, int lddy, const uint32_t* relu_bits, float drop_p, const float* x,
                                                int ldx, float* dW, int lddw, float* db, long M, int N, int K, float* workspace,
                                                long workspace_floats, const uint32_t* dy_mag, const uint32_t* x_mag, void* stream) {
  return linear_bwd_weight_emu_mag(dy, lddy, relu_bits, drop_p, x, ldx, dW, lddw, db, M, N, K, workspace, workspace_floats, dy_mag, x_mag, stream);
}
```

### hoisdf_amd/csrc/gemm_emu_dw.hip

```cpp
#include "gemm_emu.h"

namespace hoisdf {

namespace {
__device__ __forceinline__ uint64_t uni64(uint64_t v) {
  const uint32_t lo = __builtin_amdgcn_readfirstlane((uint32_t)v), hi = __builtin_amdgcn_readfirstlane((uint32_t)(v >> 32));
  return ((uint64_t)hi << 32) | lo;
}
}

#define DW_TILE_SETUP(DTK_)                                                                                            \
  const int tid = threadIdx.x, lane = tid & 63, wave = tid >> 6;                                                       \
  const int wm = wave >> 1, wn = wave & 1;                                                                             \
  const int l31 = lane & 31, kh = lane >> 5;                                                                           \
  const int ntile = g.tiles_n * g.tiles_k;                                                                             \
  const int bid = blockIdx.x;                                                                                          \
  const int split = (bid & 7) + 8 * (bid / (8 * ntile));       \
  const int t = (bid >> 3) % ntile;                                                                                    \
  if (split >= g.splitk) return;                                                                                       \
  const int tn = t / g.tiles_k, tk = t - tn * g.tiles_k;                                                               \
  const int n0 = tn * DT, k0 = tk * DTK_;                                                                              \
  const int mbeg = split * g.m_per_split;                                                                              \
  const int mend = min(g.M, mbeg + g.m_per_split);                                                                     \
  const int nslab = (mend - mbeg + KS - 1) / KS;

#define DW2_STORE_COLSUM()                                                                                             \
  do {                                                                                                                 \
    if (HASDB && tk == 0) {                                                                                            \
      float* red = reinterpret_cast<float*>(lds);                                                                      \
      if (isA) *reinterpret_cast<f32x4*>(&red[c * DT + 4 * cg]) = csum * post;                                         \
      __syncthreads();                                                                                                 \
      if (tid < DT) {                                                                                                  \
        const int n = n0 + tid;                                                                                        \
        if (n < g.N) g.colsum[(size_t)split * g.colsum_split_stride + n] = red[tid] + red[DT + tid];                   \
      }                                                                                                                \
      __syncthreads();                                                                                                 \
    }                                                                                                                  \
  } while (0)
#define DW_EPILOGUE(DTK_, VAL)                                                                                         \
  do {                                                                                                                 \
    float* Cb = g.C + (size_t)split * g.c_split_stride;                                                                \
    const bool full = (n0 + DT <= g.N) && (k0 + (DTK_) <= g.K) && (g.K % 4 == 0);                                      \
    constexpr int WK_ = (DTK_) / 2, ES = WK_ + 4;                                                                      \
    constexpr int LPR = WK_ / 4, RPI = 64 / LPR;           \
    float* w = reinterpret_cast<float*>(lds) + wave * (32 * ES);                                                       \
    _Pragma("unroll") for (int i = 0; i < 4; ++i) {                                                                    \
      _Pragma("unroll") for (int j = 0; j < (DTK_) / 64; ++j)                                                          \
        _Pragma("unroll") for (int r = 0; r < 16; ++r) w[((r & 3) + 8 * (r >> 2) + 4 * kh) * ES + j * 32 + l31] = (VAL); \
      _Pragma("unroll") for (int p = 0; p < 32 / RPI; ++p) {                                                           \
        const int rr = p * RPI + lane / LPR, cc = (lane % LPR) * 4;                                                    \
        const int row = n0 + wm * 128 + i * 32 + rr, col = k0 + wn * WK_ + cc;                                         \
        const float4 v = *reinterpret_cast<const float4*>(w + rr * ES + cc);                                           \
        if (full) {                                                                                                    \
// ... 359 lines not shown
#define MM(ax, bx) _Pragma("unroll") for (int i = 0; i < 4; ++i) _Pragma("unroll") for (int j = 0; j < 4; ++j) acc[i][j] = MFH(ax[i], bx[j], acc[i][j])
#include "dw2h_phase.inc"
#define DSTAGE_ALL(st)                                                                                                 \
  do {                                                                                                                 \
    _Pragma("unroll") for (int j = 0; j < 4; ++j) {                                                                    \
      _Pragma("unroll") for (int pr = 0; pr < 4; ++pr) { DU1(j, pr); DU2(j, pr); }                                     \
      DSTA(st, j, 0); DSTA(st, j, 1);                                                                                  \
    }                                                                                                                  \
  } while (0)

  const int nslab2 = (max(nslab, 1) + 1) & ~1;
  f16x8 aH[4], aL[4], bP[4], bQ[4], bL[4];
  DLOAD_ALL(0);
  DLOADM_ALL(0);
  DSTAGE_ALL(s0);
  DLOAD_ALL(1);
  DLOADM_ALL(1);
  __syncthreads();
#pragma unroll
  for (int i = 0; i < 4; ++i) { aL[i] = DLA(s0, 1, i); aH[i] = DLA(s0, 0, i); }
#pragma unroll
  for (int j = 0; j < 4; ++j) { bP[j] = DLB(s0, 0, j); bL[j] = DLB(s0, 1, j); }
  MM(aL, bP); MM(aH, bL);
  DSTAGE_ALL(s1);
  DLOAD_ALL(2);
  DLOADM_ALL(2);
  SYNC();
  for (int s = 1; s + 1 < nslab2; s += 2) {
    DHPHASE(s1, s0, s, bP, bQ);
    SYNC();
    DHPHASE(s0, s1, s + 1, bQ, bP);
    SYNC();
  }
  DHPHASE(s1, s0, nslab2 - 1, bP, bQ);
  SB();
  MM(aH, bQ);
  __syncthreads();
#undef DU1
#undef DU2
#undef DSTA
#undef DLA
#undef DLB
#undef M1
#undef MM
#undef DHPHASE
#undef DSTAGE_ALL
  const float unscale = h2_inv_scale(am_dy) * h2_inv_scale(am_x);
  const float post = MASK ? g.ascale : 1.f;
  u32x4* lds = lds_all;
  DW2_STORE_COLSUM();
  DW_EPILOGUE(DT, acc[i][j][r] * (MASK ? post * unscale : unscale));
}

__global__ __launch_bounds__(1024) void emu_reduce_partials_kernel(const float* __restrict__ part, long stride, int splits,
                                                                   float* __restrict__ out, long n, int blocks0,
                                                                   const float* __restrict__ part1, long stride1,
                                                                   float* __restrict__ out1, long n1) {
  __shared__ float4 red[16][64];
  const int lane = threadIdx.x & 63, w = threadIdx.x >> 6;
  int blk = blockIdx.x;
  if (blk >= blocks0) { blk -= blocks0; part = part1; stride = stride1; out = out1; n = n1; }
  const long i = ((long)blk * 64 + lane) * 4;
  float4 s = make_float4(0.f, 0.f, 0.f, 0.f);
  if (i < n) {
    const float* p = part + i;
    int k = w;
    for (; k + 16 < splits; k += 32) {
      const float4 u = *reinterpret_cast<const float4*>(p + (size_t)k * stride);
      const float4 v = *reinterpret_cast<const float4*>(p + (size_t)(k + 16) * stride);
      s.x += u.x; s.y += u.y; s.z += u.z; s.w += u.w;
      s.x += v.x; s.y += v.y; s.z += v.z; s.w += v.w;
    }
    if (k < splits) {
      const float4 u = *reinterpret_cast<const float4*>(p + (size_t)k * stride);
      s.x += u.x; s.y += u.y; s.z += u.z; s.w += u.w;
    }
  }
  red[w][lane] = s;
  __syncthreads();
  if (w == 0 && i < n) {
    float4 t = red[0][lane];
#pragma unroll
    for (int j = 1; j < 16; ++j) {
      const float4 v = red[j][lane];
      t.x += v.x; t.y += v.y; t.z += v.z; t.w += v.w;
    }
    *reinterpret_cast<float4*>(out + i) = t;
  }
}

int dw_tile(int K) { return K <= 128 ? 128 : 256; }
void plan_dw(long M, int N, int K, int& splitk, int& mper) {
  const int dtk = dw_tile(K);
  const int ntile = cdiv(N, DT) * cdiv(K, dtk);
  const int slabs = cdiv(M, KS);
  const int slots = dtk == 256 ? 256 : 512;
  const int per_xcd = slots / 8 / ntile;
  int want = per_xcd >= 1 ? per_xcd * 8 : (ntile >= slots ? 1 : slots / ntile);
  if (want > slabs / 8) want = slabs / 8 > 0 ? slabs / 8 : 1;
  mper = cdiv(slabs, want) * KS;
  splitk = cdiv(M, mper);
}

int emu_dw_launch(const DwArgs& g, bool h2, float* dW, float* db, float* workspace, hipStream_t st) {
  const int dtk = dw_tile(g.K);
  const unsigned lb = 2u * (3 * 2 * DT + 3 * 2 * 128) * 16u;
  static bool attr_set = false;
  if (!attr_set) {
    auto raise = [&](const void* k) { return hipFuncSetAttribute(k, hipFuncAttributeMaxDynamicSharedMemorySize, (int)lb) == hipSuccess; };
    const bool ok = raise(reinterpret_cast<const void*>(emu_dw_kernel<false, 128>)) && raise(reinterpret_cast<const void*>(emu_dw_kernel<true, 128>));
    if (!ok) {
      set_error("linear_bwd_weight_emu: cannot raise the dynamic LDS limit");
      return HOISDF_ERR_LAUNCH;
    }
    attr_set = true;
  }
  const dim3 grid((unsigned)(g.tiles_n * g.tiles_k * 8 * cdiv(g.splitk, 8))), block(NT);
  const bool mask = g.bits != nullptr, hasdb = g.colsum != nullptr;
  static void (*const dw2h[2][2])(DwArgs) = {{emu_dw2h_kernel<false, false>, emu_dw2h_kernel<false, true>},
                                             {emu_dw2h_kernel<true, false>, emu_dw2h_kernel<true, true>}};
  static void (*const dw2[2][2])(DwArgs) = {{emu_dw2_kernel<false, false>, emu_dw2_kernel<false, true>},
                                            {emu_dw2_kernel<true, false>, emu_dw2_kernel<true, true>}};
  if (dtk == 256) hipLaunchKernelGGL((h2 ? dw2h : dw2)[mask][hasdb], grid, block, 0, st, g);
  else hipLaunchKernelGGL((mask ? emu_dw_kernel<true, 128> : emu_dw_kernel<false, 128>), grid, block, lb, st, g);
  if (int rc = check_launch("linear_bwd_weight_emu")) return rc;
  if (g.splitk > 1) {
    const long n = (long)g.N * g.K;
    const int b0 = (int)((n + 255) / 256), b1 = db ? (g.N + 255) / 256 : 0;
    hipLaunchKernelGGL(emu_reduce_partials_kernel, dim3((unsigned)(b0 + b1)), dim3(1024), 0, st, workspace, n, g.splitk, dW, n, b0,
                       workspace + (size_t)g.splitk * g.N * g.K, (long)g.N, db, (long)g.N);
    return check_launch("linear_bwd_weight_emu reduce");
  }
  return HOISDF_OK;
}

}
```

### hoisdf_amd/csrc/gemm_emu_small.hip

```cpp
#include "gemm_emu.h"

namespace hoisdf {
namespace {
struct Frag { bf16x8 p[3]; };
__device__ __forceinline__ Frag split8(const float (&e)[8]) {
  bf16x8 p0, p1, p2;
  SPLIT1(e[0], 0); SPLIT1(e[1], 1); SPLIT1(e[2], 2); SPLIT1(e[3], 3);
  SPLIT1(e[4], 4); SPLIT1(e[5], 5); SPLIT1(e[6], 6); SPLIT1(e[7], 7);
  Frag f; f.p[0] = p0; f.p[1] = p1; f.p[2] = p2;
  return f;
}
__device__ __forceinline__ f32x16 mul6(const Frag& a, const Frag& b, f32x16 c) {
  c = MFB(a.p[2], b.p[0], c); c = MFB(a.p[0], b.p[2], c); c = MFB(a.p[1], b.p[1], c);
  c = MFB(a.p[1], b.p[0], c); c = MFB(a.p[0], b.p[1], c); c = MFB(a.p[0], b.p[0], c);
  return c;
}

struct SmallArgs {
  const float* A; long lda;
  const float* W; long ldw;
  float* C; long ldc;
  const float* bias;
  const uint32_t* abits; int ldbits; float ascale;
  uint32_t* bits_out; int ldbits_out;
  int M, N, K;
  int act; float drop_p, inv_keep; uint32_t thresh; uint64_t seed;
  int accumulate;
};

__device__ __forceinline__ void ld8(const float* p, int k0, int lim, float (&e)[8]) {
  const float4 u = k0 < lim ? *reinterpret_cast<const float4*>(p + k0) : make_float4(0.f, 0.f, 0.f, 0.f);
  const float4 v = k0 + 4 < lim ? *reinterpret_cast<const float4*>(p + k0 + 4) : make_float4(0.f, 0.f, 0.f, 0.f);
  e[0] = u.x; e[1] = u.y; e[2] = u.z; e[3] = u.w; e[4] = v.x; e[5] = v.y; e[6] = v.z; e[7] = v.w;
}

template <bool DX>
__global__ __launch_bounds__(256) void emu_small_kernel(SmallArgs g) {
  __shared__ float red[3][16][64];
  const int lane = threadIdx.x & 63, wave = threadIdx.x >> 6;
  const int l31 = lane & 31, kh = lane >> 5;
  const int ncol = DX ? g.K : g.N, ncon = DX ? g.N : g.K;
  const int m0 = blockIdx.y * 32, n0 = blockIdx.x * 32;
  const int arow = min(m0 + l31, g.M - 1);
  const bool avalid = m0 + l31 < g.M;
  const int bcol = min(n0 + l31, ncol - 1);
  const float* ap = g.A + (size_t)arow * g.lda;
  const int nslab = (ncon + 15) / 16;
  f32x16 acc;
#pragma unroll
  for (int r = 0; r < 16; ++r) acc[r] = 0.f;
  float ea[8], eb[8], na[8], nb[8];
  uint32_t mw = 0xffu, nmw = 0xffu;
  auto load = [&](int s, float (&a)[8], float (&b)[8], uint32_t& m) {
// ... 12 lines not shown
    const bool more = s + 4 < nslab;
    if (more) load(s + 4, na, nb, nmw);
    if (DX && g.abits) {
#pragma unroll
      for (int e = 0; e < 8; ++e) ea[e] = (mw >> e) & 1u ? ea[e] : 0.f;
    }
    const Frag fa = split8(ea), fb = split8(eb);
    acc = mul6(fa, fb, acc);
    if (more) {
#pragma unroll
      for (int e = 0; e < 8; ++e) { ea[e] = na[e]; eb[e] = nb[e]; }
      mw = nmw;
    }
  }
  if (wave > 0) {
#pragma unroll
    for (int r = 0; r < 16; ++r) red[wave - 1][r][lane] = acc[r];
  }
  __syncthreads();
  if (wave != 0) return;
#pragma unroll
  for (int r = 0; r < 16; ++r) acc[r] = ((acc[r] + red[0][r][lane]) + red[1][r][lane]) + red[2][r][lane];
  const int col = n0 + l31;
  const bool cvalid = col < ncol;
  const float bv = (!DX && g.bias && cvalid) ? g.bias[col] : 0.f;
  const float post = DX && g.abits ? g.ascale : 1.f;
#pragma unroll
  for (int r = 0; r < 16; ++r) {
    const int row = m0 + (r & 3) + 8 * (r >> 2) + 4 * kh;
    float v = acc[r] * post + bv;
    if (!DX) {
      if (g.act == 1) v = fmaxf(v, 0.f);
      if (g.drop_p > 0.f) v *= drop_scale(drop_rowkey(g.seed, (uint32_t)row), (uint32_t)col, g.thresh, g.inv_keep);
      if (g.bits_out) {
        const unsigned long long q = __ballot(cvalid && v > 0.f);
        if (l31 == 0 && row < g.M) g.bits_out[(size_t)row * g.ldbits_out + (n0 >> 5)] = (uint32_t)(kh ? q >> 32 : q);
      }
    }
    if (row < g.M && cvalid) {
      float* cp = g.C + (size_t)row * g.ldc + col;
      *cp = g.accumulate ? *cp + v : v;
    }
  }
}

struct SmallDwArgs {
  const float* dy; long lddy;
  const float* x; long ldx;
  const uint32_t* bits; int ldbits; float ascale;
  float* dW; long lddw; float* db;
  int M, N, K;
};

__global__ __launch_bounds__(256) void emu_small_dw_kernel(SmallDwArgs g) {
  __shared__ float red[3][16][64];
  __shared__ float rdb[4][32];
  const int lane = threadIdx.x & 63, wave = threadIdx.x >> 6;
  const int l31 = lane & 31, kh = lane >> 5;
  const int n0 = blockIdx.y * 32, k0 = blockIdx.x * 32;
  const int ncol = min(n0 + l31, g.N - 1), kcol = min(k0 + l31, g.K - 1);
  const bool nvalid = n0 + l31 < g.N, kvalid = k0 + l31 < g.K;
  const int nslab = (g.M + 15) / 16;
  f32x16 acc;
#pragma unroll
  for (int r = 0; r < 16; ++r) acc[r] = 0.f;
  float colsum = 0.f;
  float ea[8], eb[8], na[8], nb[8];
  auto load = [&](int s, float (&av)[8], float (&bv)[8]) {
    const int mb = s * 16 + 8 * kh;
#pragma unroll
    for (int e = 0; e < 8; ++e) {
      const int m = mb + e;
      float a = 0.f, b = 0.f;
      if (m < g.M) {
        if (nvalid) {
          a = g.dy[(size_t)m * g.lddy + ncol];
          if (g.bits) a = (g.bits[(size_t)m * g.ldbits + (ncol >> 5)] >> (ncol & 31)) & 1u ? a : 0.f;
        }
        if (kvalid) b = g.x[(size_t)m * g.ldx + kcol];
      }
      av[e] = a; bv[e] = b;
    }
  };
  if (wave < nslab) load(wave, ea, eb);
  for (int s = wave; s < nslab; s += 4) {
    const bool more = s + 4 < nslab;
    if (more) load(s + 4, na, nb);
#pragma unroll
    for (int e = 0; e < 8; ++e) colsum += ea[e];
    const Frag fa = split8(ea), fb = split8(eb);
    acc = mul6(fa, fb, acc);
    if (more) {
#pragma unroll
      for (int e = 0; e < 8; ++e) { ea[e] = na[e]; eb[e] = nb[e]; }
    }
  }
  if (wave > 0) {
#pragma unroll
    for (int r = 0; r < 16; ++r) red[wave - 1][r][lane] = acc[r];
  }
  colsum += __shfl_xor(colsum, 32, 64);
  if (kh == 0) rdb[wave][l31] = colsum;
  __syncthreads();
  if (wave != 0) return;
  const float sc = g.bits ? g.ascale : 1.f;
#pragma unroll
  for (int r = 0; r < 16; ++r) {
    const float v = ((acc[r] + red[0][r][lane]) + red[1][r][lane]) + red[2][r][lane];
    const int n = n0 + (r & 3) + 8 * (r >> 2) + 4 * kh, k = k0 + l31;
    if (n < g.N && k < g.K) g.dW[(size_t)n * g.lddw + k] = v * sc;
  }
  if (g.db && blockIdx.x == 0 && kh == 0 && nvalid) g.db[n0 + l31] = (((rdb[0][l31] + rdb[1][l31]) + rdb[2][l31]) + rdb[3][l31]) * sc;
}
}
}

using namespace hoisdf;

static inline bool al16p(const void* p) { return (reinterpret_cast<uintptr_t>(p) & 15) == 0; }

extern "C" int hoisdf_linear_emu_small_max_rows(void) { return 2047; }

extern "C" int hoisdf_linear_emu_small_supported(const float* a, long lda, const float* W, long ldw, long M, int N, int K) {
  return a && W && M >= 1 && M <= hoisdf_linear_emu_small_max_rows() && N >= 1 && K >= 1 && al16p(a) && al16p(W) && lda % 4 == 0 &&
         ldw % 4 == 0 && N % 4 == 0 && K % 4 == 0;
}

extern "C" int hoisdf_linear_fwd_emu_small(const float* x, int ldx, const float* W, int ldw, const float* bias, float* y, int ldy,
                                           long M, int N, int K, int act, float drop_p, uint64_t seed, uint32_t* relu_bits,
                                           void* stream) {
  HOISDF_REQUIRE(M == 0 || (x && W && y), HOISDF_ERR_INVALID, "linear_fwd_emu_small: null pointer");
  HOISDF_REQUIRE(M >= 0 && N > 0 && K > 0 && ldx >= K && ldw >= K && ldy >= N && drop_p >= 0.f && drop_p < 1.f, HOISDF_ERR_INVALID,
                 "linear_fwd_emu_small: bad sizes M=%ld N=%d K=%d", M, N, K);
  if (M == 0) return HOISDF_OK;
  HOISDF_REQUIRE(hoisdf_linear_emu_small_supported(x, ldx, W, ldw, M, N, K), HOISDF_ERR_INVALID,
                 "linear_fwd_emu_small: M <= %d, 16-byte aligned operands, leading dims / N / K multiples of 4", hoisdf_linear_emu_small_max_rows());
  SmallArgs g{};
  g.A = x; g.lda = ldx; g.W = W; g.ldw = ldw; g.C = y; g.ldc = ldy; g.bias = bias;
  g.bits_out = relu_bits; g.ldbits_out = (N + 31) / 32;
  g.M = (int)M; g.N = N; g.K = K; g.act = act; g.drop_p = drop_p; g.inv_keep = 1.f / (1.f - drop_p);
  g.thresh = drop_threshold(drop_p); g.seed = seed;
  const dim3 grid((unsigned)cdiv(N, 32), (unsigned)cdiv((int)M, 32));
  hipLaunchKernelGGL(emu_small_kernel<false>, grid, dim3(256), 0, as_stream(stream), g);
  return check_launch("linear_fwd_emu_small");
}

extern "C" int hoisdf_linear_bwd_input_emu_small(const float* dy, int lddy, const uint32_t* relu_bits, float drop_p, const float* W,
                                                 int ldw, float* dx, int lddx, long M, int N, int K, int accumulate, void* stream) {
  HOISDF_REQUIRE(M == 0 || (dy && W && dx), HOISDF_ERR_INVALID, "linear_bwd_input_emu_small: null pointer");
  HOISDF_REQUIRE(M >= 0 && N > 0 && K > 0 && lddy >= N && ldw >= K && lddx >= K && drop_p >= 0.f && drop_p < 1.f, HOISDF_ERR_INVALID,
                 "linear_bwd_input_emu_small: bad sizes");
  if (M == 0) return HOISDF_OK;
  HOISDF_REQUIRE(hoisdf_linear_emu_small_supported(dy, lddy, W, ldw, M, N, K), HOISDF_ERR_INVALID,
                 "linear_bwd_input_emu_small: M <= %d, 16-byte aligned operands, leading dims / N / K multiples of 4", hoisdf_linear_emu_small_max_rows());
  SmallArgs g{};
  g.A = dy; g.lda = lddy; g.W = W; g.ldw = ldw; g.C = dx; g.ldc = lddx;
  g.abits = relu_bits; g.ldbits = (N + 31) / 32; g.ascale = relu_bits ? 1.f / (1.f - drop_p) : 1.f;
  g.M = (int)M; g.N = N; g.K = K; g.accumulate = accumulate; g.inv_keep = 1.f;
  const dim3 grid((unsigned)cdiv(K, 32), (unsigned)cdiv((int)M, 32));
  hipLaunchKernelGGL(emu_small_kernel<true>, grid, dim3(256), 0, as_stream(stream), g);
  return check_launch("linear_bwd_input_emu_small");
}

extern "C" int hoisdf_linear_bwd_weight_emu_small(const float* dy, int lddy, const uint32_t* relu_bits, float drop_p, const float* x,
                                                  int ldx, float* dW, int lddw, float* db, long M, int N, int K, void* stream) {
  HOISDF_REQUIRE(dW && (M == 0 || (dy && x)), HOISDF_ERR_INVALID, "linear_bwd_weight_emu_small: null pointer");
  HOISDF_REQUIRE(M > 0 && M <= hoisdf_linear_emu_small_max_rows() && N > 0 && K > 0 && lddy >= N && ldx >= K && lddw >= K &&
                     drop_p >= 0.f && drop_p < 1.f,
                 HOISDF_ERR_INVALID, "linear_bwd_weight_emu_small: bad sizes");
  SmallDwArgs g{};
  g.dy = dy; g.lddy = lddy; g.x = x; g.ldx = ldx; g.bits = relu_bits; g.ldbits = (N + 31) / 32;
  g.ascale = relu_bits ? 1.f / (1.f - drop_p) : 1.f;
  g.dW = dW; g.lddw = lddw; g.db = db; g.M = (int)M; g.N = N; g.K = K;
  const dim3 grid((unsigned)cdiv(K, 32), (unsigned)cdiv(N, 32));
  hipLaunchKernelGGL(emu_small_dw_kernel, grid, dim3(256), 0, as_stream(stream), g);
  return check_launch("linear_bwd_weight_emu_small");
}
```

### hoisdf_amd/csrc/heads.hip

```cpp
#include "chain.h"

using namespace hoisdf;

namespace {
constexpr int MLP_MAX = HOISDF_MLP_MAX_LAYERS;
inline long bits_words(int N) { return (N + 31) / 32; }

struct MlpSaved { float* h[MLP_MAX]; uint32_t* bits[MLP_MAX]; uint32_t* mag; };

bool mlp_ok(const hoisdf_mlp* m) {
  if (!m || m->n_layers < 1 || m->n_layers > MLP_MAX) return false;
  for (int i = 0; i <= m->n_layers; ++i) if (m->dims[i] <= 0) return false;
  return true;
}
void mlp_carve(const hoisdf_mlp* m, long M, Bump& b, MlpSaved& s) {
  const int last = m->n_layers - 1;
  for (int i = 0; i < m->n_layers; ++i) {
    s.h[i] = i < last ? b.floats(M * m->dims[i + 1]) : nullptr;
    const bool act = i < last || m->act_last;
    s.bits[i] = act ? static_cast<uint32_t*>(b.take(M * bits_words(m->dims[i + 1]) * 4)) : nullptr;
  }
  s.mag = static_cast<uint32_t*>(b.take((long)m->n_layers * M * 4));
}
inline bool chain_mags_on(const Ctx& c, long M) { return c.emu && emu_form_h2() && M >= EMU_MIN_ROWS; }
// ... 43 lines not shown
    lin_bwd_weight(c, g, ldg, s.bits[i], 0.f, in, ldin, G->dw[i], G->db[i], M, m->dims[i + 1], m->dims[i], 0, g_mag, g_mag ? in_mag : nullptr);
    if (i == 0 && !dx) break;
    float* gin = i > 0 ? c.ws->floats(M * m->dims[i]) : dx;
    const int ldgin = i > 0 ? m->dims[i] : lddx;
    if (!c.dry && c.ok() && !gin) { c.rc = HOISDF_ERR_WORKSPACE; return; }
    uint32_t* gin_mag = mg && i > 0 && emu_rows(c, M, g, ldg, m->dims[i + 1]) ? mg + (long)i * M : nullptr;
    lin_bwd_input(c, g, ldg, s.bits[i], 0.f, m->w[i], m->dims[i], m->img_t[i], gin, ldgin, M, m->dims[i + 1], m->dims[i], i == 0 ? accumulate_dx : 0,
                  g_mag, gin_mag);
    g = gin; ldg = ldgin; g_mag = gin_mag;
  }
}
const uint32_t* enc_mag(const Ctx& c, const hoisdf_mlp* m, const float* x, int ldx, long M, const MlpSaved& s) {
  return chain_mags_on(c, M) && !c.dry && s.mag && saved_mags().get(s.mag) != 0 && emu_rows(c, M, x, ldx, m->dims[0]) ? s.mag : nullptr;
}
bool grads_ok(const hoisdf_mlp* m, const hoisdf_mlp_grads* G) {
  if (!G) return false;
  for (int i = 0; i < m->n_layers; ++i) if (!G->dw[i] || !G->db[i]) return false;
  return true;
}

struct TokSaved { float* feat; float* fea; MlpSaved mlp; };
void tok_carve(const hoisdf_mlp* m, long M, bool own_feat, Bump& b, TokSaved& s) {
  s.feat = own_feat ? b.floats(M * m->dims[0]) : nullptr;
  s.fea = b.floats(M * m->dims[m->n_layers]);
  mlp_carve(m, M, b, s.mlp);
}

struct VoteSaved { float *off, *cls, *stats; MlpSaved vote, cl; };
void vote_carve(const hoisdf_mlp* mv, const hoisdf_mlp* mc, long M, int LB, int J, Bump& b, VoteSaved& s) {
  s.off = b.floats(M * 3 * J); s.cls = b.floats(M * J); s.stats = b.floats((long)LB * J * 2);
  mlp_carve(mv, M, b, s.vote); mlp_carve(mc, M, b, s.cl);
}
}

extern "C" long hoisdf_tokens_saved_bytes(const hoisdf_mlp* mlp, long n_rows, int gather_inside) {
  if (!mlp_ok(mlp) || n_rows <= 0) return 0;
  Bump b(nullptr, 0); TokSaved s;
  tok_carve(mlp, n_rows, gather_inside != 0, b, s);
  return b.off + 256;
}

static int tokens_backward(const hoisdf_mlp* mlp, const hoisdf_mlp_grads* G, const float* feat, long M, TokSaved& s, const float* dtok,
                           const float* sdf, const float* beta, float* dfeat, int accumulate_dfeat, float* dbeta, int B, int P, int S, int row0,
                           int D, Bump& ws, bool dry, void* stream) {
  Ctx c{as_stream(stream), stream, &ws, dry, gemm_emu_mode()};
  const int F = mlp->dims[mlp->n_layers];
  float* dfea = ws.floats(M * F);
  float* part = ws.floats(hoisdf_token_build_bwd_partials());
  if (!dry) {
    if (!dfea || !part) { set_error("tokens_bwd: workspace too small"); return HOISDF_ERR_WORKSPACE; }
    c.rc = hoisdf_token_build_bwd_ordered(dtok, s.fea, F, sdf, beta, dfea, F, dbeta, part, B, P, S, row0, D, stream);
  }
  mlp_backward(c, mlp, G, feat, mlp->dims[0], M, s.mlp, dfea, F, dfeat, mlp->dims[0], accumulate_dfeat);
  if (c.ok() && !dry && ws.overflow) { set_error("tokens_bwd: workspace too small"); return HOISDF_ERR_WORKSPACE; }
  return c.rc;
}

extern "C" long hoisdf_tokens_workspace_bytes(const hoisdf_mlp* mlp, long n_rows, int backward_pass) {
  if (!mlp_ok(mlp) || n_rows <= 0) return 0;
  Bump ws(nullptr, 0), sv(nullptr, 0);
  TokSaved s; tok_carve(mlp, n_rows, false, sv, s);
  Ctx c{nullptr, nullptr, &ws, true, gemm_emu_mode()};
  if (backward_pass) {
    hoisdf_mlp_grads G{};
    (void)tokens_backward(mlp, &G, nullptr, n_rows, s, nullptr, nullptr, nullptr, reinterpret_cast<float*>(1), 0, nullptr, 1, 1, 1, 0, 1, ws, true, nullptr);
  } else {
    mlp_forward(c, mlp, nullptr, mlp->dims[0], n_rows, s.mlp, nullptr, mlp->dims[mlp->n_layers]);
  }
  return ws.off + 256;
}

extern "C" int hoisdf_tokens_fwd(const hoisdf_pyramid* pyr, const float* points, const float* center, const float* cam_intr, float scale,
                                 int img_h, int img_w, const float* feat_in, const float* cam_in, const hoisdf_mlp* mlp, const float* pe,
                                 const float* sdf, const float* beta_ptr, float* tok, float* fea_out, float* cam_out, int B, int P, int S,
                                 int row0, int D, void* saved, long saved_bytes, void* workspace, long workspace_bytes, void* stream) {
  HOISDF_REQUIRE(mlp_ok(mlp) && center && pe && sdf && beta_ptr && tok && saved && workspace, HOISDF_ERR_INVALID, "tokens_fwd: null pointer / bad MLP");
  HOISDF_REQUIRE(B > 0 && P > 0 && S >= row0 + P && row0 >= 0 && mlp->act_last && mlp->dims[mlp->n_layers] == D - 33, HOISDF_ERR_INVALID,
                 "tokens_fwd: bad sizes (the MLP must end in D - 33 = %d activated columns)", D - 33);
  const bool gather = feat_in == nullptr;
  HOISDF_REQUIRE(gather ? (pyr && points && cam_intr && cam_out) : (cam_in != nullptr), HOISDF_ERR_INVALID,
                 "tokens_fwd: either gathered rows + their camera points, or a pyramid + points + cam_out");
  const long M = (long)B * P;
  HOISDF_REQUIRE(saved_bytes >= hoisdf_tokens_saved_bytes(mlp, M, gather), HOISDF_ERR_WORKSPACE, "tokens_fwd: saved buffer of %ld bytes, need %ld", saved_bytes,
                 hoisdf_tokens_saved_bytes(mlp, M, gather));
  Bump sv(saved, saved_bytes), ws(workspace, workspace_bytes);
  TokSaved s; tok_carve(mlp, M, gather, sv, s);
  Ctx c{as_stream(stream), stream, &ws, false, gemm_emu_mode()};
  const int C = mlp->dims[0], F = D - 33;
  const float* feat = feat_in;
  const float* cam = cam_in;
  if (gather) {
    c.rc = hoisdf_project_gather_fwd(pyr, points, nullptr, M, P, center, cam_intr, scale, img_h, img_w, s.feat, C, cam_out, nullptr, stream);
    feat = s.feat; cam = cam_out;
  }
  mlp_forward(c, mlp, feat, C, M, s.mlp, s.fea, F);
  if (c.ok()) c.rc = hoisdf_token_build_fwd(cam, center, pe, s.fea, F, sdf, beta_ptr, tok, B, P, S, row0, D, stream);
  if (c.ok() && fea_out && hipMemcpyAsync(fea_out, s.fea, sizeof(float) * M * F, hipMemcpyDeviceToDevice, c.st) != hipSuccess) c.rc = HOISDF_ERR_LAUNCH;
  if (c.ok() && (sv.overflow || ws.overflow)) c.rc = HOISDF_ERR_WORKSPACE;
  if (c.rc == HOISDF_ERR_WORKSPACE) set_error("tokens_fwd: workspace (%ld bytes) too small", workspace_bytes);
  return c.rc;
}

extern "C" int hoisdf_tokens_bwd(const hoisdf_pyramid_grad* dpyr, const float* points, const float* center, const float* cam_intr, float scale,
                                 int img_h, int img_w, const float* feat_in, const hoisdf_mlp* mlp, const float* sdf, const float* beta_ptr,
                                 const float* dtok, const void* saved, long saved_bytes, const hoisdf_mlp_grads* grads, float* dfeat,
                                 int accumulate_dfeat, float* dbeta, int B, int P, int S, int row0, int D, void* workspace, long workspace_bytes,
                                 void* stream) {
  HOISDF_REQUIRE(mlp_ok(mlp) && grads_ok(mlp, grads) && sdf && beta_ptr && dtok && saved && dbeta && workspace, HOISDF_ERR_INVALID,
                 "tokens_bwd: null pointer (every weight-gradient buffer is required, zero-filled)");
  const bool gather = feat_in == nullptr;
  const long M = (long)B * P;
  HOISDF_REQUIRE(B > 0 && P > 0 && saved_bytes >= hoisdf_tokens_saved_bytes(mlp, M, gather), HOISDF_ERR_INVALID, "tokens_bwd: bad sizes / saved buffer");
  HOISDF_REQUIRE(gather ? (points && center && cam_intr) : true, HOISDF_ERR_INVALID, "tokens_bwd: the gather's arguments are needed again");
  Bump sv(const_cast<void*>(saved), saved_bytes), ws(workspace, workspace_bytes);
  TokSaved s; tok_carve(mlp, M, gather, sv, s);
  const int C = mlp->dims[0];
  float* df = dfeat;
  int acc = accumulate_dfeat;
  if (gather && dpyr && !df) {
    df = ws.floats(M * C); acc = 0;
    if (!df) { set_error("tokens_bwd: workspace too small"); return HOISDF_ERR_WORKSPACE; }
  }
  int rc = tokens_backward(mlp, grads, gather ? s.feat : feat_in, M, s, dtok, sdf, beta_ptr, df, acc, dbeta, B, P, S, row0, D, ws, false, stream);
  if (rc == HOISDF_OK && gather && dpyr && df)
    rc = hoisdf_project_gather_bwd(dpyr, points, nullptr, M, P, center, cam_intr, scale, img_h, img_w, df, C, stream);
  return rc;
}

extern "C" long hoisdf_heads_vote_saved_bytes(const hoisdf_mlp* vote, const hoisdf_mlp* cls, int L, int B, int P, int J) {
  if (!mlp_ok(vote) || !mlp_ok(cls) || L <= 0 || B <= 0 || P <= 0 || J <= 0) return 0;
  Bump b(nullptr, 0); VoteSaved s;
  vote_carve(vote, cls, (long)L * B * P, L * B, J, b, s);
  return b.off + 256;
}

static int heads_vote_backward(const hoisdf_mlp* mv, const hoisdf_mlp* mc, const hoisdf_mlp_grads* Gv, const hoisdf_mlp_grads* Gc, const float* enc,
                               const float* pts, const float* gt, float radius, const float* joints, VoteSaved& s, const float* djoints,
                               const float* dl3d, const float* dbce, float* denc, int L, int B, int P, int J, Bump& ws, bool dry, void* stream) {
  Ctx c{as_stream(stream), stream, &ws, dry, gemm_emu_mode()};
  const long M = (long)L * B * P;
  float* doff = ws.floats(M * 3 * J); float* dcls = ws.floats(M * J);
  if (!dry) {
    if (!doff || !dcls) { set_error("heads_vote_bwd: workspace too small"); return HOISDF_ERR_WORKSPACE; }
    c.rc = hoisdf_vote_loss_bwd(s.off, s.cls, pts, gt, radius, joints, s.stats, djoints, dl3d, dbce, doff, dcls, L, B, P, J, stream);
  }
  const int E = mv->dims[0];
  mlp_backward(c, mv, Gv, enc, E, M, s.vote, doff, 3 * J, denc, E, 0);
  mlp_backward(c, mc, Gc, enc, E, M, s.cl, dcls, J, denc, E, 1, enc_mag(c, mv, enc, E, M, s.vote));
  if (c.ok() && !dry && ws.overflow) { set_error("heads_vote_bwd: workspace too small"); return HOISDF_ERR_WORKSPACE; }
  return c.rc;
}

extern "C" long hoisdf_heads_vote_workspace_bytes(const hoisdf_mlp* vote, const hoisdf_mlp* cls, int L, int B, int P, int J, int backward_pass) {
  if (!mlp_ok(vote) || !mlp_ok(cls) || L <= 0 || B <= 0 || P <= 0 || J <= 0) return 0;
  const long M = (long)L * B * P;
  Bump ws(nullptr, 0), sv(nullptr, 0);
  VoteSaved s; vote_carve(vote, cls, M, L * B, J, sv, s);
  if (backward_pass) {
    hoisdf_mlp_grads G{};
    (void)heads_vote_backward(vote, cls, &G, &G, nullptr, nullptr, nullptr, 0.f, nullptr, s, nullptr, nullptr, nullptr, reinterpret_cast<float*>(1), L, B, P, J, ws,
                              true, nullptr);
  } else {
    Ctx c{nullptr, nullptr, &ws, true, gemm_emu_mode()};
    mlp_forward(c, vote, nullptr, vote->dims[0], M, s.vote, nullptr, 3 * J);
    mlp_forward(c, cls, nullptr, cls->dims[0], M, s.cl, nullptr, J);
  }
  return ws.off + 256;
}

extern "C" int hoisdf_heads_vote_fwd(const float* enc, const hoisdf_mlp* vote, const hoisdf_mlp* cls, const float* pts, const float* joint_gt_mm,
                                     float radius, float* joints, float* l3d_sum, float* bce_sum, float* near_sum, int L, int B, int P, int J,
                                     void* saved, long saved_bytes, void* workspace, long workspace_bytes, void* stream) {
  HOISDF_REQUIRE(enc && mlp_ok(vote) && mlp_ok(cls) && pts && joint_gt_mm && joints && l3d_sum && bce_sum && near_sum && saved && workspace,
                 HOISDF_ERR_INVALID, "heads_vote_fwd: null pointer / bad MLP");
  HOISDF_REQUIRE(L > 0 && B > 0 && P > 0 && J > 0 && vote->dims[vote->n_layers] == 3 * J && cls->dims[cls->n_layers] == J &&
                     vote->dims[0] == cls->dims[0] && !vote->act_last && !cls->act_last,
                 HOISDF_ERR_INVALID, "heads_vote_fwd: the vote MLP must end in 3 J = %d, the class MLP in J = %d plain columns", 3 * J, J);
  HOISDF_REQUIRE(saved_bytes >= hoisdf_heads_vote_saved_bytes(vote, cls, L, B, P, J), HOISDF_ERR_WORKSPACE, "heads_vote_fwd: saved buffer too small");
  const long M = (long)L * B * P;
  Bump sv(saved, saved_bytes), ws(workspace, workspace_bytes);
  VoteSaved s; vote_carve(vote, cls, M, L * B, J, sv, s);
  Ctx c{as_stream(stream), stream, &ws, false, gemm_emu_mode()};
  const int E = vote->dims[0];
  mlp_forward(c, vote, enc, E, M, s.vote, s.off, 3 * J);
  mlp_forward(c, cls, enc, E, M, s.cl, s.cls, J, enc_mag(c, vote, enc, E, M, s.vote));
  if (c.ok()) c.rc = hoisdf_vote_loss_fwd(s.off, s.cls, pts, joint_gt_mm, radius, joints, s.stats, l3d_sum, bce_sum, near_sum, L, B, P, J, stream);
  if (c.ok() && (sv.overflow || ws.overflow)) c.rc = HOISDF_ERR_WORKSPACE;
  if (c.rc == HOISDF_ERR_WORKSPACE) set_error("heads_vote_fwd: workspace (%ld bytes) too small", workspace_bytes);
  return c.rc;
}

extern "C" int hoisdf_heads_vote_bwd(const float* enc, const hoisdf_mlp* vote, const hoisdf_mlp* cls, const float* pts, const float* joint_gt_mm,
                                     float radius, const float* joints, const void* saved, long saved_bytes, const float* djoints,
                                     const float* dl3d_sum, const float* dbce_sum, const hoisdf_mlp_grads* vote_grads,
                                     const hoisdf_mlp_grads* cls_grads, float* denc, int L, int B, int P, int J, void* workspace,
                                     long workspace_bytes, void* stream) {
  HOISDF_REQUIRE(enc && mlp_ok(vote) && mlp_ok(cls) && grads_ok(vote, vote_grads) && grads_ok(cls, cls_grads) && pts && joint_gt_mm && joints && saved &&
                     denc && workspace,
                 HOISDF_ERR_INVALID, "heads_vote_bwd: null pointer (every weight-gradient buffer is required, zero-filled)");
  HOISDF_REQUIRE(L > 0 && B > 0 && P > 0 && J > 0 && saved_bytes >= hoisdf_heads_vote_saved_bytes(vote, cls, L, B, P, J), HOISDF_ERR_INVALID,
                 "heads_vote_bwd: bad sizes / saved buffer");
// ... 6 lines not shown
```

### hoisdf_amd/csrc/layers.hip

```cpp
#include <stdlib.h>

#include <mutex>
#include <unordered_map>

#include "chain.h"

namespace hoisdf {
namespace {

__global__ void rows_copy_add_kernel(float* __restrict__ dst, long dst_gs, const float* __restrict__ src, long src_gs, int rows, int E4,
                                     long total, int add) {
  const long i = (long)blockIdx.x * blockDim.x + threadIdx.x;
  if (i >= total) return;
  const long per = (long)rows * E4;
  const long g = i / per, r = i - g * per;
  float4* d = reinterpret_cast<float4*>(dst + g * dst_gs) + r;
  const float4 s = reinterpret_cast<const float4*>(src + g * src_gs)[r];
  if (add) { float4 t = *d; t.x += s.x; t.y += s.y; t.z += s.z; t.w += s.w; *d = t; }
  else *d = s;
}
int rows_copy_add(float* dst, long dst_gs, const float* src, long src_gs, int groups, int rows, int E, int add, hipStream_t st) {
  const long total = (long)groups * rows * (E / 4);
  if (total == 0) return HOISDF_OK;
  hipLaunchKernelGGL(rows_copy_add_kernel, dim3((unsigned)cdiv(total, 256)), dim3(256), 0, st, dst, dst_gs, src, src_gs, rows, E / 4, total, add);
// ... 180 lines not shown
  enum { MAG_DF = 0, MAG_DH = 1, MAG_DA = 2, MAG_BROWS = 3 };
  const long bmag_bytes = ((long)MAG_BROWS * M + Ms + (long)g.H * g.B) * 4;
  uint32_t* bmag = static_cast<uint32_t*>(ws.take(bmag_bytes));
  const bool mags = layer_mags(c, g) && (dry || bmag);
  auto mg = [&](int i) -> uint32_t* { return mags && bmag ? bmag + (long)i * M : nullptr; };
  uint32_t* const mag_dqkv = mags && bmag ? bmag + (long)MAG_BROWS * M : nullptr;
  uint32_t* const head_do = mags && bmag ? bmag + (long)MAG_BROWS * M + Ms : nullptr;
  auto fm = [&](int i) -> const uint32_t* { return mags && fwd_mags && s.mag ? s.mag + (long)i * M : nullptr; };
  uint32_t* const smag = mags && fwd_mags ? s.mag : nullptr;
  if (mags && !dry && c.ok() && hipMemsetAsync(bmag, 0, (size_t)bmag_bytes, c.st) != hipSuccess) c.rc = HOISDF_ERR_LAUNCH;
  if (!dry && c.ok()) c.rc = add_layernorm_bwd_mag(dx2, s.x1, s.f, w->g2, st + 2 * M, st + 3 * M, nullptr, dx1, df, G->dg2, G->dbe2, M, E, g.p, d->seed[3], nullptr, mg(MAG_DF), stream);
  lin_bwd_input(c, df, E, nullptr, 0.f, w->w2, F, w->img_t_2, dh, F, M, E, F, 0, mg(MAG_DF), mg(MAG_DH));
  lin_bwd_weight(c, df, E, nullptr, 0.f, s.h, F, G->dw2, G->db2, M, E, F, 0, mg(MAG_DF), fm(MAG_H));
  lin_bwd_input(c, dh, F, s.bits, g.p, w->w1, E, w->img_t_1, dx1, E, M, F, E, 1, mg(MAG_DH), nullptr);
  lin_bwd_weight(c, dh, F, s.bits, g.p, s.x1, E, G->dw1, G->db1, M, F, E, 0, mg(MAG_DH), fm(MAG_X1));
  const float* xq2 = g.full ? x : s.xq;
  if (!dry && c.ok()) c.rc = add_layernorm_bwd_mag(dx1, xq2, s.a, w->g1, st, st + M, nullptr, dxq, da, G->dg1, G->dbe1, M, E, g.p, d->seed[1], nullptr, mg(MAG_DA), stream);
  lin_bwd_input(c, da, E, nullptr, 0.f, w->w_out, E, w->img_t_out, dO, E, M, E, E, 0, mg(MAG_DA), nullptr, g.att_h2 ? head_do : nullptr, g.nq);
  lin_bwd_weight(c, da, E, nullptr, 0.f, s.o, E, G->dw_out, G->db_out, M, E, E, 0, mg(MAG_DA), g.att == 2 ? fm(MAG_O) : nullptr);
  const bool amag = mags && g.att_bwd_emu && g.full;
  auto attn_bwd = [&](const float* q, int ldq, const float* k, const float* v, int ldkv, float* dq, float* dk, float* dv) {
    if (g.att_bwd_emu) {
      const long ab = hoisdf_attention_bwd_emu_workspace(g.B, g.H, g.nq, g.S, s.planes ? 1 : 0);
      void* aw = ws.take(ab);
      if (dry || !c.ok()) return;
      if (!aw) { c.rc = HOISDF_ERR_WORKSPACE; return; }
      const bool hm = g.att_h2 && smag && head_do;
      if (g.att_h2 && !hm) { set_error("encoder_layer_bwd: the forward ran the f16x2 attention but the head magnitudes are not available"); c.rc = HOISDF_ERR_INVALID; return; }
      c.rc = attention_bwd_emu_mag(q, ldq, k, ldkv, v, ldkv, s.o, E, dO, E, s.lse, delta, dq, dk, dv, g.B, g.H, g.nq, g.S, g.S, g.p, d->seed[0],
                                   s.planes, aw, ab, amag ? mag_dqkv : nullptr, stream, hm ? head_q(g, smag) : nullptr,
                                   hm ? head_k(g, smag) : nullptr, hm ? head_v(g, smag) : nullptr, hm ? head_do : nullptr);
    } else if (!dry && c.ok()) {
      c.rc = hoisdf_attention_bwd(q, ldq, k, ldkv, v, ldkv, s.o, E, dO, E, s.lse, delta, dq, dk, dv, g.B, g.H, g.nq, g.S, g.S, g.p, d->seed[0], stream);
    }
  };
  if (g.full) {
    float* dqkv = ws.floats(Ms * 3 * E);
    if (!dry && !dqkv) { set_error("encoder_layer_bwd: workspace too small"); return HOISDF_ERR_WORKSPACE; }
    if (g.fused_qkv) attn_bwd(nullptr, 3 * E, nullptr, nullptr, 3 * E, dqkv, dqkv + E, dqkv + 2 * E);
    else attn_bwd(s.qkv, 3 * E, s.qkv + E, s.qkv + 2 * E, 3 * E, dqkv, dqkv + E, dqkv + 2 * E);
    lin_bwd_input(c, dqkv, 3 * E, nullptr, 0.f, w->w_in, E, w->img_t_in, dxq, E, Ms, 3 * E, E, 1, amag ? mag_dqkv : nullptr, nullptr);
    lin_bwd_weight(c, dqkv, 3 * E, nullptr, 0.f, x, E, G->dw_in, G->db_in, Ms, 3 * E, E, 0, amag ? mag_dqkv : nullptr, amag ? d->x_mag : nullptr);
  } else {
    float* dq = ws.floats(M * E); float* dkv = ws.floats(Ms * 2 * E);
    if (!dry && (!dq || !dkv)) { set_error("encoder_layer_bwd: workspace too small"); return HOISDF_ERR_WORKSPACE; }
    if (g.fused_qkv) attn_bwd(nullptr, E, nullptr, nullptr, 2 * E, dq, dkv, dkv + E);
    else attn_bwd(s.qbuf, E, s.kvbuf, s.kvbuf + E, 2 * E, dq, dkv, dkv + E);
    lin_bwd_input(c, dq, E, nullptr, 0.f, w->w_in, E, w->img_t_in_q, dxq, E, M, E, E, 1);
    lin_bwd_weight(c, dq, E, nullptr, 0.f, s.xq, E, G->dw_in, G->db_in, M, E, E);
    lin_bwd_input(c, dkv, 2 * E, nullptr, 0.f, w->w_in + (size_t)E * E, E, w->img_t_in_kv, dx, E, Ms, 2 * E, E, 0);
    lin_bwd_weight(c, dkv, 2 * E, nullptr, 0.f, x, E, G->dw_in + (size_t)E * E, G->db_in ? G->db_in + E : nullptr, Ms, 2 * E, E);
    if (!dry && c.ok()) c.rc = rows_copy_add(dx, (long)g.S * E, dxq, (long)g.nq * E, g.B, g.nq, E, 1, c.st);
  }
  if (c.ok() && !dry && ws.overflow) { set_error("encoder_layer_bwd: workspace too small"); return HOISDF_ERR_WORKSPACE; }
  return c.rc;
}

}
}

using namespace hoisdf;

extern "C" long hoisdf_encoder_layer_saved_bytes(const hoisdf_encoder_layer_desc* d) {
  Geo g;
  if (geometry(d, g) != HOISDF_OK) return -1;
  Bump b(nullptr, 0); Saved s;
  carve_saved(g, b, s);
  return b.off + 256;
}

extern "C" const uint32_t* hoisdf_encoder_layer_out_mag(const hoisdf_encoder_layer_desc* d, const void* saved) {
  Geo g;
  if (!saved || geometry(d, g) != HOISDF_OK || !d->training) return nullptr;
  Ctx c{nullptr, nullptr, nullptr, false, gemm_emu_mode()};
  if (!layer_mags(c, g)) return nullptr;
  Bump b(const_cast<void*>(saved), 1L << 62); Saved s;
  carve_saved(g, b, s);
  return s.mag ? s.mag + (long)MAG_XOUT * g.M : nullptr;
}

extern "C" long hoisdf_encoder_layer_workspace_bytes(const hoisdf_encoder_layer_desc* d, int backward_pass) {
  Geo g;
  if (geometry(d, g) != HOISDF_OK) return -1;
  hoisdf_encoder_layer_weights w{};
  hoisdf_encoder_layer_grads G{};
  float dummy = 0.f;
  w.g3 = &dummy;
  Bump saved(nullptr, 0), ws(nullptr, 0);
  if (backward_pass) (void)backward(nullptr, nullptr, &w, d, g, saved, &dummy, &dummy, nullptr, &G, ws, true, nullptr);
  else (void)forward(nullptr, &w, d, g, nullptr, nullptr, saved, ws, true, nullptr);
  return ws.off + 256;
}

extern "C" int hoisdf_encoder_layer_fwd(const float* x, const hoisdf_encoder_layer_weights* w, const hoisdf_encoder_layer_desc* d, float* x_out,
                                        float* y_out, void* saved, long saved_bytes, void* workspace, long workspace_bytes, void* stream) {
  Geo g;
  if (int rc = geometry(d, g)) return rc;
  HOISDF_REQUIRE(x && w && x_out && w->w_in && w->w_out && w->w1 && w->w2 && w->g1 && w->be1 && w->g2 && w->be2, HOISDF_ERR_INVALID,
                 "encoder_layer_fwd: null pointer");
  HOISDF_REQUIRE(!w->g3 || (w->be3 && y_out), HOISDF_ERR_INVALID, "encoder_layer_fwd: inter_norm needs be3 and y_out");
  HOISDF_REQUIRE(!d->training || saved, HOISDF_ERR_WORKSPACE, "encoder_layer_fwd: training needs the saved buffer (hoisdf_encoder_layer_saved_bytes)");
  HOISDF_REQUIRE(workspace || workspace_bytes == 0, HOISDF_ERR_WORKSPACE, "encoder_layer_fwd: null workspace");
  HOISDF_REQUIRE(al16(x) && al16(x_out) && al16(saved) && al16(workspace), HOISDF_ERR_INVALID, "encoder_layer_fwd: buffers must be 16-byte aligned");
  Bump sv(saved, saved_bytes), ws(workspace, workspace_bytes);
  static char none;
  if (!sv.base) { sv.base = &none; sv.cap = 0; }
// ... 78 lines not shown
}

int dforward(const float* tgt, const float* memory, const float* qpos, const uint8_t* mask, const hoisdf_decoder_layer_weights* w,
             const hoisdf_decoder_layer_desc* d, const DGeo& g, float* out, float* y_out, Bump& saved, Bump& ws, bool dry, void* stream) {
  Ctx c{as_stream(stream), stream, &ws, dry, gemm_emu_mode()};
  DSaved s;
  dcarve(g, d->training ? saved : ws, s);
  const int E = g.E, F = g.F;
  const long M = g.M;
  float* st = s.st;
  if (!dry && c.ok()) c.rc = add_bcast(s.tq1, tgt, qpos, g, c.st);
  lin_fwd(c, s.tq1, E, w->sa_w_in, E, nullptr, w->sa_b_in, s.qk, 2 * E, M, 2 * E, E, 0, 0.f, 0, nullptr);
  lin_fwd(c, tgt, E, w->sa_w_in + (size_t)2 * E * E, E, nullptr, w->sa_b_in ? w->sa_b_in + 2 * E : nullptr, s.v, E, M, E, E, 0, 0.f, 0, nullptr);
  if (!dry && c.ok())
    c.rc = hoisdf_attention_small_fwd(s.qk, 2 * E, s.qk + E, 2 * E, s.v, E, mask, s.o1, E, s.probs, g.B, g.H, g.Q, g.Q, g.p, d->seed[0], stream);
  lin_fwd(c, s.o1, E, w->sa_w_out, E, nullptr, w->sa_b_out, s.a1, E, M, E, E, 0, 0.f, 0, nullptr);
  if (!dry && c.ok()) c.rc = hoisdf_add_layernorm_fwd(tgt, s.a1, w->g1, w->be1, s.x1, st, st + M, M, E, g.eps, g.p, d->seed[1], stream);
  if (!dry && c.ok()) c.rc = add_bcast(s.tq2, s.x1, qpos, g, c.st);
  lin_fwd(c, s.tq2, E, w->ca_w_in, E, nullptr, w->ca_b_in, s.q2, E, M, E, E, 0, 0.f, 0, nullptr);
  lin_fwd(c, memory, E, w->ca_w_in + (size_t)E * E, E, w->img_ca_kv, w->ca_b_in ? w->ca_b_in + E : nullptr, s.kv, 2 * E, g.Ms, 2 * E, E, 0, 0.f, 0, nullptr);
  if (!dry && c.ok())
    c.rc = hoisdf_attention_fwd(s.q2, E, s.kv, 2 * E, s.kv + E, 2 * E, s.o2, E, s.lse2, g.B, g.H, g.Q, g.S, g.kv, g.p, d->seed[2], stream);
  lin_fwd(c, s.o2, E, w->ca_w_out, E, nullptr, w->ca_b_out, s.a2, E, M, E, E, 0, 0.f, 0, nullptr);
  if (!dry && c.ok()) c.rc = hoisdf_add_layernorm_fwd(s.x1, s.a2, w->g2, w->be2, s.x2, st + 2 * M, st + 3 * M, M, E, g.eps, g.p, d->seed[3], stream);
  lin_fwd(c, s.x2, E, w->w1, E, nullptr, w->b1, s.h, F, M, F, E, 1, g.p, d->seed[4], s.bits);
  lin_fwd(c, s.h, F, w->w2, F, nullptr, w->b2, s.f, E, M, E, F, 0, 0.f, 0, nullptr);
  if (!dry && c.ok()) c.rc = hoisdf_add_layernorm_fwd(s.x2, s.f, w->g3, w->be3, out, st + 4 * M, st + 5 * M, M, E, g.eps, g.p, d->seed[5], stream);
  if (w->g4 && !dry && c.ok()) c.rc = hoisdf_add_layernorm_fwd(out, nullptr, w->g4, w->be4, y_out, st + 6 * M, st + 7 * M, M, E, g.eps, 0.f, 0, stream);
  return c.rc;
}

int dbackward(const float* tgt, const float* memory, const uint8_t* mask, const float* out, const hoisdf_decoder_layer_weights* w,
              const hoisdf_decoder_layer_desc* d, const DGeo& g, Bump& saved, const float* g_out, const float* g_y, float* d_tgt, float* d_memory,
              int accumulate_memory, float* d_qpos, const hoisdf_decoder_layer_grads* G, Bump& ws, bool dry, void* stream) {
  Ctx c{as_stream(stream), stream, &ws, dry, gemm_emu_mode()};
  DSaved s;
  dcarve(g, saved, s);
  (void)mask;
  const int E = g.E, F = g.F;
  const long M = g.M, Ms = g.Ms;
  const float* st = s.st;
  const float* dx3 = g_out;
  if (g_y && w->g4) {
    float* t = ws.floats(M * E);
    if (!dry && c.ok()) {
      if (!t) c.rc = HOISDF_ERR_WORKSPACE;
      else c.rc = hoisdf_add_layernorm_bwd(g_y, out, nullptr, w->g4, st + 6 * M, st + 7 * M, g_out, t, nullptr, G->dg4, G->dbe4, M, E, 0.f, 0, stream);
    }
    dx3 = t;
  }
  float* dx2 = ws.floats(M * E); float* df = ws.floats(M * E); float* dh = ws.floats(M * F);
  float* dx1 = ws.floats(M * E); float* da2 = ws.floats(M * E); float* do2 = ws.floats(M * E); float* dq2 = ws.floats(M * E);
  float* dkv = ws.floats(Ms * 2 * E); float* delta = ws.floats((long)g.B * g.H * g.Q); float* dtq2 = ws.floats(M * E);
  float* da1 = ws.floats(M * E); float* do1 = ws.floats(M * E); float* dqk = ws.floats(M * 2 * E); float* dv = ws.floats(M * E);
  float* dtq1 = ws.floats(M * E);
  if (!dry && (!dx2 || !df || !dh || !dx1 || !da2 || !do2 || !dq2 || !dkv || !delta || !dtq2 || !da1 || !do1 || !dqk || !dv || !dtq1)) {
    set_error("decoder_layer_bwd: workspace too small");
    return HOISDF_ERR_WORKSPACE;
  }
  if (!dry && !dx3) { set_error("decoder_layer_bwd: no upstream gradient (g_out and g_y both null)"); return HOISDF_ERR_INVALID; }
  if (!dry && c.ok()) c.rc = hoisdf_add_layernorm_bwd(dx3, s.x2, s.f, w->g3, st + 4 * M, st + 5 * M, nullptr, dx2, df, G->dg3, G->dbe3, M, E, g.p, d->seed[5], stream);
  lin_bwd_input(c, df, E, nullptr, 0.f, w->w2, F, nullptr, dh, F, M, E, F, 0);
  lin_bwd_weight(c, df, E, nullptr, 0.f, s.h, F, G->dw2, G->db2, M, E, F);
  lin_bwd_input(c, dh, F, s.bits, g.p, w->w1, E, nullptr, dx2, E, M, F, E, 1);
  lin_bwd_weight(c, dh, F, s.bits, g.p, s.x2, E, G->dw1, G->db1, M, F, E);
  if (!dry && c.ok()) c.rc = hoisdf_add_layernorm_bwd(dx2, s.x1, s.a2, w->g2, st + 2 * M, st + 3 * M, nullptr, dx1, da2, G->dg2, G->dbe2, M, E, g.p, d->seed[3], stream);
  lin_bwd_input(c, da2, E, nullptr, 0.f, w->ca_w_out, E, nullptr, do2, E, M, E, E, 0);
  lin_bwd_weight(c, da2, E, nullptr, 0.f, s.o2, E, G->dca_w_out, G->dca_b_out, M, E, E);
  if (!dry && c.ok())
    c.rc = hoisdf_attention_bwd(s.q2, E, s.kv, 2 * E, s.kv + E, 2 * E, s.o2, E, do2, E, s.lse2, delta, dq2, dkv, dkv + E, g.B, g.H, g.Q, g.S, g.kv, g.p,
                                d->seed[2], stream);
  lin_bwd_input(c, dq2, E, nullptr, 0.f, w->ca_w_in, E, nullptr, dtq2, E, M, E, E, 0);
  lin_bwd_weight(c, dq2, E, nullptr, 0.f, s.tq2, E, G->dca_w_in, G->dca_b_in, M, E, E);
  lin_bwd_input(c, dkv, 2 * E, nullptr, 0.f, w->ca_w_in + (size_t)E * E, E, w->img_t_ca_kv, d_memory, E, Ms, 2 * E, E, accumulate_memory ? 1 : 0);
  lin_bwd_weight(c, dkv, 2 * E, nullptr, 0.f, memory, E, G->dca_w_in + (size_t)E * E, G->dca_b_in ? G->dca_b_in + E : nullptr, Ms, 2 * E, E);
  if (!dry && c.ok()) c.rc = rows_copy_add(dx1, M * E, dtq2, M * E, 1, (int)M, E, 1, c.st);
  if (!dry && c.ok()) c.rc = hoisdf_add_layernorm_bwd(dx1, tgt, s.a1, w->g1, st, st + M, nullptr, d_tgt, da1, G->dg1, G->dbe1, M, E, g.p, d->seed[1], stream);
  lin_bwd_input(c, da1, E, nullptr, 0.f, w->sa_w_out, E, nullptr, do1, E, M, E, E, 0);
  lin_bwd_weight(c, da1, E, nullptr, 0.f, s.o1, E, G->dsa_w_out, G->dsa_b_out, M, E, E);
  if (!dry && c.ok()) {
    if (hipMemsetAsync(dqk, 0, sizeof(float) * M * 2 * E, c.st) != hipSuccess || hipMemsetAsync(dv, 0, sizeof(float) * M * E, c.st) != hipSuccess) {
      set_error("decoder_layer_bwd: clearing the self-attention gradients failed");
      return HOISDF_ERR_LAUNCH;
    }
    c.rc = hoisdf_attention_small_bwd(s.qk, 2 * E, s.qk + E, 2 * E, s.v, E, s.probs, do1, E, dqk, dqk + E, dv, g.B, g.H, g.Q, g.Q, g.p, d->seed[0], stream);
  }
  lin_bwd_input(c, dqk, 2 * E, nullptr, 0.f, w->sa_w_in, E, nullptr, dtq1, E, M, 2 * E, E, 0);
  lin_bwd_weight(c, dqk, 2 * E, nullptr, 0.f, s.tq1, E, G->dsa_w_in, G->dsa_b_in, M, 2 * E, E);
  lin_bwd_input(c, dv, E, nullptr, 0.f, w->sa_w_in + (size_t)2 * E * E, E, nullptr, d_tgt, E, M, E, E, 1);
  lin_bwd_weight(c, dv, E, nullptr, 0.f, tgt, E, G->dsa_w_in + (size_t)2 * E * E, G->dsa_b_in ? G->dsa_b_in + 2 * E : nullptr, M, E, E);
  if (!dry && c.ok()) c.rc = rows_copy_add(d_tgt, M * E, dtq1, M * E, 1, (int)M, E, 1, c.st);
  if (d_qpos && !dry && c.ok()) {
    hipLaunchKernelGGL(sum_bcast_grad_kernel, dim3((unsigned)cdiv((long)g.Q * (E / 4), 256)), dim3(256), 0, c.st, d_qpos, dtq1, dtq2, g.B, g.Q, E / 4);
    c.rc = check_launch("decoder_layer query_pos gradient");
  }
  if (c.ok() && !dry && ws.overflow) { set_error("decoder_layer_bwd: workspace too small"); return HOISDF_ERR_WORKSPACE; }
  return c.rc;
}

}
}

extern "C" long hoisdf_decoder_layer_saved_bytes(const hoisdf_decoder_layer_desc* d) {
  DGeo g;
  if (dgeometry(d, g) != HOISDF_OK) return -1;
  Bump b(nullptr, 0); DSaved s;
  dcarve(g, b, s);
  return b.off + 256;
}

extern "C" long hoisdf_decoder_layer_workspace_bytes(const hoisdf_decoder_layer_desc* d, int backward_pass) {
  DGeo g;
  if (dgeometry(d, g) != HOISDF_OK) return -1;
  hoisdf_decoder_layer_weights w{};
  hoisdf_decoder_layer_grads G{};
  float dummy = 0.f;
  w.g4 = &dummy;
  Bump saved(nullptr, 0), ws(nullptr, 0);
  if (backward_pass) (void)dbackward(nullptr, nullptr, nullptr, nullptr, &w, d, g, saved, &dummy, &dummy, nullptr, nullptr, 0, nullptr, &G, ws, true, nullptr);
  else (void)dforward(nullptr, nullptr, nullptr, nullptr, &w, d, g, nullptr, nullptr, saved, ws, true, nullptr);
  return ws.off + 256;
}

extern "C" int hoisdf_decoder_layer_fwd(const float* tgt, const float* memory, const float* query_pos, const uint8_t* tgt_mask,
                                        const hoisdf_decoder_layer_weights* w, const hoisdf_decoder_layer_desc* d, float* out, float* y_out,
                                        void* saved, long saved_bytes, void* workspace, long workspace_bytes, void* stream) {
  DGeo g;
  if (int rc = dgeometry(d, g)) return rc;
  HOISDF_REQUIRE(tgt && memory && query_pos && tgt_mask && w && out && w->sa_w_in && w->sa_w_out && w->ca_w_in && w->ca_w_out && w->w1 && w->w2 &&
                     w->g1 && w->be1 && w->g2 && w->be2 && w->g3 && w->be3,
                 HOISDF_ERR_INVALID, "decoder_layer_fwd: null pointer");
  HOISDF_REQUIRE(!w->g4 || (w->be4 && y_out), HOISDF_ERR_INVALID, "decoder_layer_fwd: the stack norm needs be4 and y_out");
  HOISDF_REQUIRE(!d->training || saved, HOISDF_ERR_WORKSPACE, "decoder_layer_fwd: training needs the saved buffer (hoisdf_decoder_layer_saved_bytes)");
  HOISDF_REQUIRE(al16(tgt) && al16(memory) && al16(query_pos) && al16(out) && al16(saved) && al16(workspace), HOISDF_ERR_INVALID,
                 "decoder_layer_fwd: buffers must be 16-byte aligned");
  static char none;
  Bump sv(saved, saved_bytes), ws(workspace, workspace_bytes);
  if (!sv.base) { sv.base = &none; sv.cap = 0; }
  if (!ws.base) { ws.base = &none; ws.cap = 0; }
  int rc = dforward(tgt, memory, query_pos, tgt_mask, w, d, g, out, y_out, sv, ws, false, stream);
  if (rc == HOISDF_OK && (sv.overflow || ws.overflow)) rc = HOISDF_ERR_WORKSPACE;
  if (rc == HOISDF_ERR_WORKSPACE) set_error("decoder_layer_fwd: workspace (%ld bytes) or saved buffer (%ld bytes) too small", workspace_bytes, saved_bytes);
  return rc;
}

extern "C" int hoisdf_decoder_layer_bwd(const float* tgt, const float* memory, const uint8_t* tgt_mask, const float* out,
                                        const hoisdf_decoder_layer_weights* w, const hoisdf_decoder_layer_desc* d, const void* saved, long saved_bytes,
                                        const float* g_out, const float* g_y, float* d_tgt, float* d_memory, int accumulate_memory,
// ... 19 lines not shown
```

### hoisdf_amd/csrc/sdf_query.hip

```cpp
#include "common.h"

using namespace hoisdf;

namespace {
constexpr int HID0 = 512, LAT = 256, PF = 33, H1 = 223, X0 = LAT + PF, CAT_K = 516, X0_COL = 224;
constexpr int CAT_LD = 544;
inline long align64(long v) { return (v + 63) / 64 * 64; }
constexpr long EMU_MIN_ROWS_Q = 2048;

inline long emu_scratch_bytes(int C) {
  const long a = hoisdf_linear_emu_image_bytes(HID0, C), b = hoisdf_linear_emu_image_bytes(HID0, CAT_K);
  return ((a > b ? a : b) + 255) / 256 * 256;
}

int layer(const float* x, int ldx, const float* W, int ldw, const float* b, float* y, int ldy, long M, int N, int K,
          int K_pad, float drop_p, uint64_t seed, void* emu_img, const void* given, void* stream, const uint32_t* x_mag = nullptr,
          uint32_t* y_mag = nullptr, bool* y_has = nullptr) {
  if (y_has) *y_has = false;
  if (emu_img && M >= EMU_MIN_ROWS_Q && hoisdf_linear_emu_supported(x, ldx, K_pad) && (K_pad + 15) / 16 == (K + 15) / 16) {
    if (!given) { if (int rc = hoisdf_linear_emu_prepare(W, ldw, N, K, 0, emu_img, stream)) return rc; }
    if (y_has) *y_has = y_mag != nullptr;
    return linear_fwd_emu_mag(x, ldx, given ? given : emu_img, b, y, ldy, M, N, K_pad, 1, drop_p, seed, nullptr, x_mag, y_mag, stream);
  }
  return hoisdf_linear_fwd(x, ldx, W, ldw, b, y, ldy, M, N, K, 1, drop_p, seed, nullptr, stream);
// ... 205 lines not shown
  if (!dry) saved_mags().put(s.mag, mags);
  auto mg = [&](int i) -> uint32_t* { return mags ? s.mag + (long)i * n : nullptr; };
  if (!dry) {
    if (mags) c.rc = hipMemsetAsync(s.mag, 0, (size_t)TM_N * n * 4, c.st) == hipSuccess ? HOISDF_OK : HOISDF_ERR_LAUNCH;
    if (c.ok()) c.rc = project_gather_fwd_mag(pyr, points, sample_idx, n, rps, center, cam_intr, scale, img_h, img_w, s.feat, C, cam_out, nullptr, mg(TM_FEAT), stream);
    if (c.ok()) c.rc = hipMemsetAsync(s.cat, 0, sizeof(float) * n * CAT_LD, c.st) == hipSuccess ? HOISDF_OK : HOISDF_ERR_LAUNCH;
  }
  float* x0 = dry ? nullptr : s.cat + X0_COL;
  lin_fwd(c, s.feat, C, w->sdfin_w0, C, w->emu_img[0], w->sdfin_b0, s.ha, HID0, n, HID0, C, 1, 0.f, 0, s.ba, 0, mg(TM_FEAT), mg(TM_HA));
  lin_fwd(c, s.ha, HID0, w->sdfin_w1, HID0, w->emu_img[1], w->sdfin_b1, x0, CAT_LD, n, LAT, HID0, 1, 0.f, 0, s.bf, 0, mg(TM_HA), mg(TM_CAT));
  if (!dry && c.ok()) c.rc = posenc_fwd_mag(points, n, s.cat, CAT_LD, X0_COL + LAT, pe, mg(TM_CAT), stream);
  lin_fwd(c, x0, CAT_LD, w->dec_w0, w->dec_ld0, w->emu_img[2], w->dec_b0, s.h0, HID0, n, HID0, X0, 1, drop_p, seed, s.b0, X0 + 3, mg(TM_CAT), mg(TM_H0));
  lin_fwd(c, s.h0, HID0, w->dec_w1, HID0, w->emu_img[3], w->dec_b1, s.cat, CAT_LD, n, H1 + 1, HID0, 1, drop_p, seed + 1, s.b1, 0, mg(TM_H0), mg(TM_CAT));
  lin_fwd(c, s.cat, CAT_LD, w->dec_w2, CAT_K, w->emu_img[4], w->dec_b2, s.h2, HID0, n, HID0, CAT_K, 1, drop_p, seed + 2, s.b2, 0, mg(TM_CAT), mg(TM_H2));
  lin_fwd(c, s.h2, HID0, w->dec_w3, HID0, w->emu_img[5], w->dec_b3, s.h3, HID0, n, HID0, HID0, 1, drop_p, seed + 3, s.b3, 0, mg(TM_H2), nullptr);
  if (!dry && c.ok()) c.rc = hoisdf_sdf_head_fwd(s.h3, HID0, w->dec_w4, w->dec_b4, s.raw, sdf, n, HID0, clamp, stream);
  return c.rc;
}

static int sdf_train_backward(const hoisdf_pyramid_grad* dpyr, const float* points, const int32_t* sample_idx, long n, int rps, const float* center,
                              const float* cam_intr, float scale, int img_h, int img_w, const hoisdf_sdf_weights* w, float clamp, float drop_p,
                              const float* d_sdf, const hoisdf_sdf_weight_grads* G, Bump& saved, Bump& ws, bool dry, void* stream) {
  Ctx c{as_stream(stream), stream, &ws, dry, gemm_emu_mode()};
  TrainSaved s;
  const int C = w ? w->C : 1;
  train_carve(n, C, saved, s);
  float* dh3 = ws.floats(n * HID0); float* dh2 = ws.floats(n * HID0); float* dcat = ws.floats(n * CAT_LD); float* dh0 = ws.floats(n * HID0);
  float* dha = ws.floats(n * HID0); float* dfeat = ws.floats(n * (long)C);
  if (!dry && (!dh3 || !dh2 || !dcat || !dh0 || !dha || !dfeat)) { set_error("sdf_query_bwd: workspace too small"); return HOISDF_ERR_WORKSPACE; }
  enum { BM_DH3 = 0, BM_DH2 = 1, BM_DCAT = 2, BM_DH0 = 3, BM_DHA = 4, BM_N = 5 };
  uint32_t* bmag = static_cast<uint32_t*>(ws.take((long)BM_N * n * 4));
  const bool mags = train_mags(c, n) && !dry && bmag && s.mag;
  const bool fmags = mags && saved_mags().get(s.mag) != 0;
  auto mg = [&](int i) -> uint32_t* { return mags ? bmag + (long)i * n : nullptr; };
  auto fm = [&](int i) -> const uint32_t* { return fmags ? s.mag + (long)i * n : nullptr; };
  if (mags) c.rc = hipMemsetAsync(bmag, 0, (size_t)BM_N * n * 4, c.st) == hipSuccess ? HOISDF_OK : HOISDF_ERR_LAUNCH;
  if (!dry && c.ok()) c.rc = sdf_head_bwd_mag(d_sdf, s.raw, s.h3, HID0, w->dec_w4, dh3, HID0, G->d_dec_w4, G->d_dec_b4, n, HID0, clamp, mg(BM_DH3), stream);
  lin_bwd_input(c, dh3, HID0, s.b3, drop_p, w->dec_w3, HID0, w->emu_img_t[5], dh2, HID0, n, HID0, HID0, 0, mg(BM_DH3), mg(BM_DH2));
  lin_bwd_weight(c, dh3, HID0, s.b3, drop_p, s.h2, HID0, G->d_dec_w3, G->d_dec_b3, n, HID0, HID0, 0, mg(BM_DH3), fm(TM_H2));
  lin_bwd_input(c, dh2, HID0, s.b2, drop_p, w->dec_w2, CAT_K, w->emu_img_t[4], dcat, CAT_LD, n, HID0, CAT_K, 0, mg(BM_DH2), mg(BM_DCAT));
  lin_bwd_weight(c, dh2, HID0, s.b2, drop_p, s.cat, CAT_LD, G->d_dec_w2, G->d_dec_b2, n, HID0, CAT_K, 0, mg(BM_DH2), fm(TM_CAT));
  lin_bwd_input(c, dcat, CAT_LD, s.b1, drop_p, w->dec_w1, HID0, w->emu_img_t[3], dh0, HID0, n, H1 + 1, HID0, 0, mg(BM_DCAT), mg(BM_DH0));
  lin_bwd_weight(c, dcat, CAT_LD, s.b1, drop_p, s.h0, HID0, G->d_dec_w1, G->d_dec_b1, n, H1 + 1, HID0, 0, mg(BM_DCAT), fm(TM_H0));
  float* dx0 = dry ? nullptr : dcat + X0_COL;
  const float* x0 = dry ? nullptr : s.cat + X0_COL;
  lin_bwd_input(c, dh0, HID0, s.b0, drop_p, w->dec_w0, w->dec_ld0, w->emu_img_t[2], dx0, CAT_LD, n, HID0, X0, 1, mg(BM_DH0), nullptr);
  lin_bwd_weight(c, dh0, HID0, s.b0, drop_p, x0, CAT_LD, G->d_dec_w0, G->d_dec_b0, n, HID0, X0, X0 + 3, mg(BM_DH0), fm(TM_CAT));
  lin_bwd_input(c, dx0, CAT_LD, s.bf, 0.f, w->sdfin_w1, HID0, w->emu_img_t[1], dha, HID0, n, LAT, HID0, 0, nullptr, mg(BM_DHA));
  lin_bwd_weight(c, dx0, CAT_LD, s.bf, 0.f, s.ha, HID0, G->d_sdfin_w1, G->d_sdfin_b1, n, LAT, HID0, 0, nullptr, fm(TM_HA));
  lin_bwd_input(c, dha, HID0, s.ba, 0.f, w->sdfin_w0, C, w->emu_img_t[0], dfeat, C, n, HID0, C, 0, mg(BM_DHA), nullptr);
  lin_bwd_weight(c, dha, HID0, s.ba, 0.f, s.feat, C, G->d_sdfin_w0, G->d_sdfin_b0, n, HID0, C, 0, mg(BM_DHA), fm(TM_FEAT));
  if (!dry && c.ok() && dpyr)
    c.rc = hoisdf_project_gather_bwd(dpyr, points, sample_idx, n, rps, center, cam_intr, scale, img_h, img_w, dfeat, C, stream);
  if (c.ok() && !dry && ws.overflow) { set_error("sdf_query_bwd: workspace too small"); return HOISDF_ERR_WORKSPACE; }
  return c.rc;
}

extern "C" long hoisdf_sdf_query_train_workspace_bytes(long n_rows, int C, int backward_pass) {
  if (n_rows <= 0 || C <= 0) return 0;
  hoisdf_sdf_weights w{}; w.C = C; w.dec_ld0 = X0;
  hoisdf_sdf_weight_grads G{};
  Bump saved(nullptr, 0), ws(nullptr, 0);
  if (backward_pass) (void)sdf_train_backward(nullptr, nullptr, nullptr, n_rows, 1, nullptr, nullptr, 1.f, 1, 1, &w, 0.f, 0.f, nullptr, &G, saved, ws, true, nullptr);
  else (void)sdf_train_forward(nullptr, nullptr, nullptr, n_rows, 1, nullptr, nullptr, 1.f, 1, 1, &w, 0.f, 0.f, 0, nullptr, nullptr, nullptr, saved, ws, true, nullptr);
  return ws.off + 256;
}

extern "C" int hoisdf_sdf_query_train_fwd(const hoisdf_pyramid* pyr, const float* points, const int32_t* sample_idx, long n_rows, int rows_per_sample,
                                          const float* center, const float* cam_intr, float scale, int img_h, int img_w,
                                          const hoisdf_sdf_weights* w, float clamp, float drop_p, uint64_t seed, float* sdf, float* pe,
                                          float* cam_out, void* saved, long saved_bytes, void* workspace, long workspace_bytes, void* stream) {
  HOISDF_REQUIRE(pyr && points && w && sdf && saved && workspace && center && cam_intr, HOISDF_ERR_INVALID, "sdf_query_train_fwd: null pointer");
  HOISDF_REQUIRE(n_rows > 0 && n_rows < (1L << 31) && w->C > 0 && w->C % 4 == 0 && w->dec_ld0 >= X0, HOISDF_ERR_INVALID, "sdf_query_train_fwd: bad sizes");
  HOISDF_REQUIRE(drop_p >= 0.f && drop_p < 1.f, HOISDF_ERR_INVALID, "sdf_query_train_fwd: drop_p=%f", drop_p);
  HOISDF_REQUIRE(saved_bytes >= hoisdf_sdf_query_train_saved_bytes(n_rows, w->C), HOISDF_ERR_WORKSPACE, "sdf_query_train_fwd: saved buffer of %ld bytes, need %ld",
                 saved_bytes, hoisdf_sdf_query_train_saved_bytes(n_rows, w->C));
  Bump sv(saved, saved_bytes), ws(workspace, workspace_bytes);
  int rc = sdf_train_forward(pyr, points, sample_idx, n_rows, rows_per_sample, center, cam_intr, scale, img_h, img_w, w, clamp, drop_p, seed, sdf, pe, cam_out,
                             sv, ws, false, stream);
  if (rc == HOISDF_OK && (sv.overflow || ws.overflow)) rc = HOISDF_ERR_WORKSPACE;
  if (rc == HOISDF_ERR_WORKSPACE) set_error("sdf_query_train_fwd: workspace (%ld bytes) too small", workspace_bytes);
  return rc;
}

extern "C" int hoisdf_sdf_query_bwd(const hoisdf_pyramid_grad* dpyr, const float* points, const int32_t* sample_idx, long n_rows, int rows_per_sample,
                                    const float* center, const float* cam_intr, float scale, int img_h, int img_w, const hoisdf_sdf_weights* w,
                                    float clamp, float drop_p, const void* saved, long saved_bytes, const float* d_sdf,
                                    const hoisdf_sdf_weight_grads* grads, void* workspace, long workspace_bytes, void* stream) {
  HOISDF_REQUIRE(points && w && saved && d_sdf && grads && workspace && center && cam_intr, HOISDF_ERR_INVALID, "sdf_query_bwd: null pointer");
  HOISDF_REQUIRE(grads->d_sdfin_w0 && grads->d_sdfin_b0 && grads->d_sdfin_w1 && grads->d_sdfin_b1 && grads->d_dec_w0 && grads->d_dec_b0 && grads->d_dec_w1 &&
                     grads->d_dec_b1 && grads->d_dec_w2 && grads->d_dec_b2 && grads->d_dec_w3 && grads->d_dec_b3 && grads->d_dec_w4 && grads->d_dec_b4,
                 HOISDF_ERR_INVALID, "sdf_query_bwd: every weight gradient buffer is required (zero-filled)");
  HOISDF_REQUIRE(n_rows > 0 && n_rows < (1L << 31) && saved_bytes >= hoisdf_sdf_query_train_saved_bytes(n_rows, w->C), HOISDF_ERR_INVALID,
                 "sdf_query_bwd: bad sizes / saved buffer");
  Bump sv(const_cast<void*>(saved), saved_bytes), ws(workspace, workspace_bytes);
  int rc = sdf_train_backward(dpyr, points, sample_idx, n_rows, rows_per_sample, center, cam_intr, scale, img_h, img_w, w, clamp, drop_p, d_sdf, grads, sv, ws,
                              false, stream);
  if (rc == HOISDF_ERR_WORKSPACE) set_error("sdf_query_bwd: workspace (%ld bytes) too small", workspace_bytes);
  return rc;
}
```

### include/hoisdf.h

```cpp
#ifndef HOISDF_H_
#define HOISDF_H_

#include <stdint.h>

#ifdef __cplusplus
extern "C" {
#endif

#define HOISDF_VERSION_MAJOR 0
#define HOISDF_VERSION_MINOR 1

typedef enum hoisdf_status {
  HOISDF_OK = 0,
  HOISDF_ERR_INVALID = -1,
  HOISDF_ERR_LAUNCH = -2,
  HOISDF_ERR_TOO_FEW = -3,
  HOISDF_ERR_WORKSPACE = -4
} hoisdf_status;

#define HOISDF_MAX_LEVELS 8

typedef struct hoisdf_pyramid {
  int n_levels;
  int B;
// ... 31 lines not shown

int hoisdf_linear_fwd(const float* x, int ldx, const float* W, int ldw, const float* bias,
                      float* y, int ldy, long M, int N, int K, int act, float drop_p,
                      uint64_t seed, uint32_t* relu_bits, void* stream);
int hoisdf_linear_bwd_input(const float* dy, int lddy, const uint32_t* relu_bits, float drop_p,
                            const float* W, int ldw, float* dx, int lddx, long M, int N, int K,
                            int accumulate ,
                            void* stream);
long hoisdf_linear_bwd_weight_workspace(long M, int N, int K);
int hoisdf_linear_bwd_weight(const float* dy, int lddy, const uint32_t* relu_bits, float drop_p,
                             const float* x, int ldx, float* dW, int lddw, float* db, long M, int N,
                             int K, float* workspace, long workspace_floats, void* stream);
long hoisdf_linear_emu_image_bytes(int rows, int K);
int hoisdf_linear_emu_prepare(const float* W, int ldw, int N, int K, int transpose, void* image, void* stream);
typedef struct hoisdf_emu_prep_item {
  const float* W;
  void* image;
  long first_block;
  int ldw, N, K, transpose;
} hoisdf_emu_prep_item;
long hoisdf_linear_emu_prepare_blocks(int N, int K, int transpose);
int hoisdf_linear_emu_prepare_batch(const hoisdf_emu_prep_item* d_items, int n, long total_blocks, void* stream);
int hoisdf_linear_emu_supported(const float* a, long lda, int contraction);
int hoisdf_linear_emu_pieces(void);
long hoisdf_mag_words(long rows);
int hoisdf_mag_measure(const float* x, long ldx, long M, int K, uint32_t* words, void* stream);
long hoisdf_head_mag_words(long M, int groups, int L);
int hoisdf_head_mag_measure(const float* x, long ldx, long M, int groups, int L, uint32_t* words, void* stream);
int hoisdf_linear_fwd_emu_heads(const float* x, int ldx, const void* w_image, const float* bias, float* y, int ldy, long M, int N,
                                int K, const uint32_t* x_mag, uint32_t* y_mag, uint32_t* y_heads, int L, void* stream);
int hoisdf_linear_bwd_input_emu_heads(const float* dy, int lddy, const void* wt_image, float* dx, int lddx, long M, int N, int K,
                                      const uint32_t* dy_mag, uint32_t* dx_mag, uint32_t* dx_heads, int L, void* stream);
int hoisdf_linear_fwd_emu_mag(const float* x, int ldx, const void* w_image, const float* bias, float* y, int ldy, long M, int N,
                              int K, int act, float drop_p, uint64_t seed, uint32_t* relu_bits, const uint32_t* x_mag,
                              uint32_t* y_mag, void* stream);
int hoisdf_linear_bwd_input_emu_mag(const float* dy, int lddy, const uint32_t* relu_bits, float drop_p, const void* wt_image,
                                    float* dx, int lddx, long M, int N, int K, int accumulate, const uint32_t* dy_mag,
                                    uint32_t* dx_mag, void* stream);
int hoisdf_linear_bwd_weight_emu_mag(const float* dy, int lddy, const uint32_t* relu_bits, float drop_p, const float* x, int ldx,
                                     float* dW, int lddw, float* db, long M, int N, int K, float* workspace, long workspace_floats,
                                     const uint32_t* dy_mag, const uint32_t* x_mag, void* stream);
int hoisdf_linear_fwd_emu(const float* x, int ldx, const void* w_image, const float* bias, float* y, int ldy, long M, int N,
                          int K, int act, float drop_p, uint64_t seed, uint32_t* relu_bits, void* stream);
int hoisdf_linear_bwd_input_emu(const float* dy, int lddy, const uint32_t* relu_bits, float drop_p, const void* wt_image,
                                float* dx, int lddx, long M, int N, int K, int accumulate, void* stream);
int hoisdf_linear_emu_small_max_rows(void);
int hoisdf_linear_emu_small_supported(const float* a, long lda, const float* W, long ldw, long M, int N, int K);
int hoisdf_linear_fwd_emu_small(const float* x, int ldx, const float* W, int ldw, const float* bias, float* y, int ldy, long M,
                                int N, int K, int act, float drop_p, uint64_t seed, uint32_t* relu_bits, void* stream);
int hoisdf_linear_bwd_input_emu_small(const float* dy, int lddy, const uint32_t* relu_bits, float drop_p, const float* W, int ldw,
                                      float* dx, int lddx, long M, int N, int K, int accumulate, void* stream);
int hoisdf_linear_bwd_weight_emu_small(const float* dy, int lddy, const uint32_t* relu_bits, float drop_p, const float* x, int ldx,
                                       float* dW, int lddw, float* db, long M, int N, int K, void* stream);
long hoisdf_linear_bwd_weight_emu_workspace(long M, int N, int K);
int hoisdf_linear_bwd_weight_emu(const float* dy, int lddy, const uint32_t* relu_bits, float drop_p, const float* x, int ldx,
                                 float* dW, int lddw, float* db, long M, int N, int K, float* workspace, long workspace_floats,
                                 void* stream);
int hoisdf_relu_dropout_bwd(const float* y, int ldy, const float* dy, int lddy, float* dpre,
                            int ldd, long M, int N, float drop_p, void* stream);

int hoisdf_posenc_fwd(const float* points, long n_rows, float* x0, int ldx0, int col0,
                      float* pe, void* stream);
int hoisdf_weightnorm_fwd(const float* v, const float* g, float* W, int ldw, float* norms,
                          int out, int in, void* stream);
int hoisdf_weightnorm_bwd(const float* v, const float* g, const float* dW, int ldw, float* dv,
                          float* dg, int out, int in, void* stream);
int hoisdf_sdf_head_fwd(const float* h, int ldh, const float* w, const float* b, float* sdf_raw,
                        float* sdf, long n_rows, int K, float clamp, void* stream);
int hoisdf_sdf_head_bwd(const float* dsdf, const float* sdf_raw, const float* h, int ldh,
                        const float* w, float* dh, int lddh, float* dw, float* db, long n_rows,
                        int K, float clamp, void* stream);

typedef struct hoisdf_sdf_weights {
  int C;
  const float *sdfin_w0, *sdfin_b0;
  const float *sdfin_w1, *sdfin_b1;
  const float *dec_w0, *dec_b0;
  int dec_ld0;
  const float *dec_w1, *dec_b1;
  const float *dec_w2, *dec_b2;
  const float *dec_w3, *dec_b3;
  const float *dec_w4, *dec_b4;
  const void* emu_img[6];
  const void* emu_img_t[6];
} hoisdf_sdf_weights;
long hoisdf_sdf_query_workspace(long n_rows, int C, int need_feat);
int hoisdf_sdf_query_fwd(const hoisdf_pyramid* pyr, const float* points, const int32_t* sample_idx, long n_rows,
                         int rows_per_sample, const float* center, const float* cam_intr, float scale, int img_h,
                         int img_w, const float* feat_in, float* feat_out, const hoisdf_sdf_weights* w, float clamp,
                         float drop_p, uint64_t seed, float* sdf, float* sdf_raw, float* pe, float* cam_out,
                         void* workspace, long workspace_bytes, void* stream);

int hoisdf_lattice_count(const float* center, const float* cam_intr, const float* bbox, float scale,
                         int bins_n, int B, int32_t* counts, void* stream);
int hoisdf_lattice_fill(const float* center, const float* cam_intr, const float* bbox, float scale,
                        int bins_n, int B, const int32_t* offsets, float* points,
                        int32_t* sample_idx, int32_t* lattice_idx, void* stream);
int hoisdf_select_smallest_abs(const float* sdf_raw, const int32_t* offsets, const int32_t* counts,
                               int B, int k, int32_t* sel, void* stream);
int hoisdf_gather_rows(const float* src, int lds, const int32_t* sel, long n_sel, int width,
                       float* out, int ldo, void* stream);
typedef struct hoisdf_sdf_weight_grads {
  float *d_sdfin_w0, *d_sdfin_b0, *d_sdfin_w1, *d_sdfin_b1;
  float *d_dec_w0, *d_dec_b0, *d_dec_w1, *d_dec_b1, *d_dec_w2, *d_dec_b2, *d_dec_w3, *d_dec_b3, *d_dec_w4, *d_dec_b4;
} hoisdf_sdf_weight_grads;
long hoisdf_sdf_query_train_saved_bytes(long n_rows, int C);
// ... 354 lines not shown
```

Before: 440.7.

## Batch small kernels: fuse Q/K/V converts, delta into convert, defer dW reductions

Combines the separate Q, K and V convert launches into one launch driven by a per-operand block table, and folds the attention-backward delta dot product into the dout convert kernel, which removes the standalone delta kernel. Small-M weight-gradient GEMMs and split-K partial reductions are queued in the chain context and issued as grouped launches at the end of each backward layer. The decoder also clears the dq/dk/dv buffers with one memset instead of two. The aim is to cut kernel launch count and launch overhead, at the cost of deferring work to the end of each layer, which removes overlap and adds bookkeeping and ordering risk.

New measurement: 442.0 (median of 6 runs). About the same (+0.3%).

```diff
diff --git a/hoisdf_amd/_lib.py b/hoisdf_amd/_lib.py
--- a/hoisdf_amd/_lib.py
+++ b/hoisdf_amd/_lib.py
@@ -83,6 +83,12 @@
     _fields_ = [("n_layers", C.c_int), ("act_last", C.c_int), ("dims", C.c_int * (MLP_MAX_LAYERS + 1)),
                 ("w", C.c_void_p * MLP_MAX_LAYERS), ("b", C.c_void_p * MLP_MAX_LAYERS),
                 ("img", C.c_void_p * MLP_MAX_LAYERS), ("img_t", C.c_void_p * MLP_MAX_LAYERS)]
+
+
+class SmallDwItem(C.Structure):
+    _fields_ = [("dy", C.c_void_p), ("lddy", C.c_int), ("relu_bits", C.c_void_p), ("drop_p", C.c_float), ("x", C.c_void_p),
+                ("ldx", C.c_int), ("dW", C.c_void_p), ("lddw", C.c_int), ("db", C.c_void_p), ("M", C.c_long), ("N", C.c_int),
+                ("K", C.c_int)]
 
 
 class EmuPrepItem(C.Structure):
@@ -156,6 +162,7 @@
     "hoisdf_linear_fwd_emu_small": [_P, _I, _P, _I, _P, _P, _I, _L, _I, _I, _I, _F, _U64, _P, _P],
     "hoisdf_linear_bwd_input_emu_small": [_P, _I, _P, _F, _P, _I, _P, _I, _L, _I, _I, _I, _P],
     "hoisdf_linear_bwd_weight_emu_small": [_P, _I, _P, _F, _P, _I, _P, _I, _P, _L, _I, _I, _P],
+    "hoisdf_linear_bwd_weight_emu_small_batch": [_P, _I, _P],
     "hoisdf_linear_bwd_weight_emu": [_P, _I, _P, _F, _P, _I, _P, _I, _P, _L, _I, _I, _P, _L, _P],
     "hoisdf_linear_bwd_weight_emu_mag": [_P, _I, _P, _F, _P, _I, _P, _I, _P, _L, _I, _I, _P, _L, _P, _P, _P],
     "hoisdf_relu_dropout_bwd": [_P, _I, _P, _I, _P, _I, _L, _I, _F, _P],
diff --git a/hoisdf_amd/csrc/attention_emu.hip b/hoisdf_amd/csrc/attention_emu.hip
--- a/hoisdf_amd/csrc/attention_emu.hip
+++ b/hoisdf_amd/csrc/attention_emu.hip
@@ -1,4 +1,5 @@
 #include "attention_emu.h"
+#include "launch_tables.h"
 
 namespace hoisdf {
 using namespace emu_attn;
@@ -51,27 +52,48 @@
 }
 }
 
-template <bool F16>
-__global__ __launch_bounds__(256) void emu_attn_convert_kernel(const float* __restrict__ src, int ld, int L, int Lp, int B, int H,
-                                                               float scale, __bf16* __restrict__ r0, __bf16* __restrict__ r1,
-                                                               __bf16* __restrict__ r2, __bf16* __restrict__ t0,
-                                                               __bf16* __restrict__ t1, __bf16* __restrict__ t2,
-                                                               const uint32_t* __restrict__ mag) {
+struct ConvOp {
+  const float* src; int ld, L, Lp; float scale;
+  __bf16 *r[3], *t[3];
+  const uint32_t* mag;
+};
+struct ConvArgs {
+  ConvOp op[3];
+  int end[3];
+  int B, H;
+  const float* o; int ldo; float* delta;
+};
+template <bool F16, bool DELTA>
+__global__ __launch_bounds__(256) void emu_attn_convert_kernel(ConvArgs a) {
   constexpr int TP = 72;
   __shared__ __attribute__((aligned(16))) __bf16 tile[3][64 * TP];
   const int tid = threadIdx.x;
+  const int which = (int)(blockIdx.x >= (unsigned)a.end[0]) + (int)(blockIdx.x >= (unsigned)a.end[1]);
+  const ConvOp g = which == 0 ? a.op[0] : which == 1 ? a.op[1] : a.op[2];
+  const int blk = (int)blockIdx.x - (which == 0 ? 0 : which == 1 ? a.end[0] : a.end[1]);
+  const int B = a.B, H = a.H, L = g.L, Lp = g.Lp;
+  __bf16 *const r0 = g.r[0], *const r1 = g.r[1], *const r2 = g.r[2], *const t0 = g.t[0], *const t1 = g.t[1], *const t2 = g.t[2];
+  float scale = g.scale;
   const int nb = Lp / 64;
-  const int kb = blockIdx.x % nb, bh = blockIdx.x / nb, b = bh / H, head = bh - b * H;
-  if (F16) { f16_saturate_on(); scale *= mag_scale(mag[head * B + b]); }
+  const int kb = blk % nb, bh = blk / nb, b = bh / H, head = bh - b * H;
+  if (F16) { f16_saturate_on(); scale *= mag_scale(g.mag[head * B + b]); }
   const int r = tid >> 2, dc = (tid & 3) * 16;
   const int row = kb * 64 + r;
   const bool valid = row < L;
-  const float* sr = src + ((size_t)b * L + (valid ? row : 0)) * ld + head * D + dc;
+  const float* sr = g.src + ((size_t)b * L + (valid ? row : 0)) * g.ld + head * D + dc;
+  const float* orow = DELTA ? a.o + ((size_t)b * L + (valid ? row : 0)) * a.ldo + head * D + dc : nullptr;
+  float ds[4];
   bf16x8 pa[2][3];
 #pragma unroll
   for (int i = 0; i < 2; ++i) {
     float4 u = valid ? *reinterpret_cast<const float4*>(sr + 8 * i) : make_float4(0.f, 0.f, 0.f, 0.f);
     float4 w = valid ? *reinterpret_cast<const float4*>(sr + 8 * i + 4) : make_float4(0.f, 0.f, 0.f, 0.f);
+    if (DELTA) {
+      const float4 x = valid ? *reinterpret_cast<const float4*>(orow + 8 * i) : make_float4(0.f, 0.f, 0.f, 0.f);
+      const float4 z = valid ? *reinterpret_cast<const float4*>(orow + 8 * i + 4) : make_float4(0.f, 0.f, 0.f, 0.f);
+      ds[2 * i] = x.x * u.x + x.y * u.y + x.z * u.z + x.w * u.w;
+      ds[2 * i + 1] = z.x * w.x + z.y * w.y + z.z * w.z + z.w * w.w;
+    }
     u.x *= scale; u.y *= scale; u.z *= scale; u.w *= scale;
     w.x *= scale; w.y *= scale; w.z *= scale; w.w *= scale;
     if (F16) {
@@ -86,6 +108,14 @@
       SPLIT1(w.x, 4); SPLIT1(w.y, 5); SPLIT1(w.z, 6); SPLIT1(w.w, 7);
       pa[i][0] = p0; pa[i][1] = p1; pa[i][2] = p2;
     }
+  }
+  if (DELTA) {
+#pragma unroll
+    for (int j = 0; j < 4; ++j) ds[j] += __shfl_xor(ds[j], 2, 64);
+#pragma unroll
+    for (int j = 0; j < 4; ++j) ds[j] += __shfl_xor(ds[j], 1, 64);
+    const float lo = ds[0] + ds[2], hi = ds[1] + ds[3];
+    if (valid && (tid & 3) == 0) a.delta[((size_t)b * H + head) * L + row] = lo + hi;
   }
   if (r0) {
     const size_t o = ((size_t)bh * Lp + row) * D + dc;
@@ -351,22 +381,6 @@
 }
 #pragma pop_macro("MB")
 
-__global__ __launch_bounds__(256) void emu_attn_delta_kernel(const float* __restrict__ o, int ldo, const float* __restrict__ dout,
-                                                             int lddo, float* __restrict__ delta, int B, int H, int Lq) {
-  const long g = ((long)blockIdx.x * 256 + threadIdx.x) >> 4;
-  const int l16 = threadIdx.x & 15;
-  if (g >= (long)B * Lq * H) return;
-  const int head = (int)(g % H);
-  const long bq = g / H;
-  const int q = (int)(bq % Lq), b = (int)(bq / Lq);
-  const float4 x = *reinterpret_cast<const float4*>(o + ((size_t)b * Lq + q) * ldo + head * D + l16 * 4);
-  const float4 y = *reinterpret_cast<const float4*>(dout + ((size_t)b * Lq + q) * lddo + head * D + l16 * 4);
-  float s = x.x * y.x + x.y * y.y + x.z * y.z + x.w * y.w;
-#pragma unroll
-  for (int off = 8; off > 0; off >>= 1) s += __shfl_xor(s, off, 16);
-  if (l16 == 0) delta[((size_t)b * H + head) * Lq + q] = s;
-}
-
 __global__ __launch_bounds__(256) void emu_attn_dq_reduce_kernel(const float* __restrict__ part, int nkb, float* __restrict__ dq,
                                                                  int ldq, int B, int H, int Lq, uint32_t* __restrict__ mag,
                                                                  const float* __restrict__ scale) {
@@ -435,19 +449,29 @@
   a.drop_p = drop_p; a.inv_keep = 1.f / (1.f - drop_p); a.thresh = drop_threshold(drop_p); a.seed = seed;
   return a;
 }
-int convert(const float* src, int ld, int L, int Lp, int B, int H, float scale, const Planes& p, hipStream_t st, const uint32_t* mag = nullptr) {
-  const long nblk = (long)B * H * (Lp / 64);
-  if (mag) hipLaunchKernelGGL(emu_attn_convert_kernel<true>, dim3((unsigned)nblk), dim3(256), 0, st, src, ld, L, Lp, B, H, scale, p.r[0], p.r[1],
-                              p.r[2], p.t[0], p.t[1], p.t[2], mag);
-  else hipLaunchKernelGGL(emu_attn_convert_kernel<false>, dim3((unsigned)nblk), dim3(256), 0, st, src, ld, L, Lp, B, H, scale, p.r[0], p.r[1],
-                          p.r[2], p.t[0], p.t[1], p.t[2], mag);
+inline ConvOp conv_op(const float* src, int ld, int L, float scale, const Planes& p, const uint32_t* mag) {
+  ConvOp c{};
+  c.src = src; c.ld = ld; c.L = L; c.Lp = (int)pad128(L); c.scale = scale; c.mag = mag;
+  for (int i = 0; i < 3; ++i) { c.r[i] = p.r[i]; c.t[i] = p.t[i]; }
+  return c;
+}
+int convert(const ConvOp* ops, int n, int B, int H, hipStream_t st, const float* o = nullptr, int ldo = 0, float* delta = nullptr) {
+  ConvArgs a{};
+  long count[3] = {0, 0, 0};
+  for (int i = 0; i < n; ++i) { a.op[i] = ops[i]; count[i] = (long)B * H * (ops[i].Lp / 64); }
+  const long nblk = block_prefix<3>(count, n, a.end);
+  HOISDF_REQUIRE(n >= 1 && nblk > 0 && (!delta || (n == 1 && o)), HOISDF_ERR_INVALID, "attention_emu_convert: bad operand table");
+  a.B = B; a.H = H; a.o = o; a.ldo = ldo; a.delta = delta;
+  const bool f16 = ops[0].mag != nullptr;
+  void (*const kern)(ConvArgs) = delta ? (f16 ? emu_attn_convert_kernel<true, true> : emu_attn_convert_kernel<false, true>)
+                                       : (f16 ? emu_attn_convert_kernel<true, false> : emu_attn_convert_kernel<false, false>);
+  hipLaunchKernelGGL(kern, dim3((unsigned)nblk), dim3(256), 0, st, a);
   return check_launch("attention_emu_convert");
 }
 int convert_qkv(const float* q, int ldq, const float* k, int ldk, const float* v, int ldv, int B, int H, int Lq, int Lk, const QkvPlaneSet& s,
                 hipStream_t st, const uint32_t* q_hm = nullptr, const uint32_t* k_hm = nullptr, const uint32_t* v_hm = nullptr) {
-  if (int rc = convert(q, ldq, Lq, (int)pad128(Lq), B, H, QS2, s.q, st, q_hm)) return rc;
-  if (int rc = convert(k, ldk, Lk, (int)pad128(Lk), B, H, 1.f, s.k, st, k_hm)) return rc;
-  return convert(v, ldv, Lk, (int)pad128(Lk), B, H, 1.f, s.v, st, v_hm);
+  const ConvOp ops[3] = {conv_op(q, ldq, Lq, QS2, s.q, q_hm), conv_op(k, ldk, Lk, 1.f, s.k, k_hm), conv_op(v, ldv, Lk, 1.f, s.v, v_hm)};
+  return convert(ops, 3, B, H, st);
 }
 int check_emu(const void* q, const void* k, const void* v, int ldq, int ldk, int ldv, int B, int H, int Lq, int Lk, int kv_len,
               float drop_p, const char* who) {
@@ -616,10 +640,8 @@
     s = carve_qkv(w, B, H, Lq, Lk, true, false);
     if (int rc = convert_qkv(q, ldq, k, ldk, v, ldv, B, H, Lq, Lk, s, st, q_hm, k_hm, v_hm)) return rc;
   }
-  if (int rc = convert(dout, lddo, Lq, (int)pad128(Lq), B, H, 1.f, pd, st, do_hm)) return rc;
-  const long ng = (long)B * Lq * H;
-  hipLaunchKernelGGL(emu_attn_delta_kernel, dim3((unsigned)((ng * 16 + 255) / 256)), dim3(256), 0, st, o, ldo, dout, lddo, delta, B, H, Lq);
-  if (int rc = check_launch("attention_emu_delta")) return rc;
+  const ConvOp od = conv_op(dout, lddo, Lq, 1.f, pd, do_hm);
+  if (int rc = convert(&od, 1, B, H, st, o, ldo, delta)) return rc;
   EmuAttn a = emu_args(B, H, Lq, Lk, kv_len, drop_p, seed);
   for (int i = 0; i < 3; ++i) { a.q[i] = s.q.r[i]; a.k[i] = s.k.r[i]; a.v[i] = s.v.r[i]; a.d[i] = pd.r[i]; }
   a.lse_in = lse; a.delta = delta; a.dq_part = part; a.dk = dk; a.dv = dv; a.ldk = ldk; a.ldv = ldv; a.mag = g_mag;
diff --git a/hoisdf_amd/csrc/chain.h b/hoisdf_amd/csrc/chain.h
--- a/hoisdf_amd/csrc/chain.h
+++ b/hoisdf_amd/csrc/chain.h
@@ -43,7 +43,23 @@
   bool emu;
   int rc = HOISDF_OK;
   bool ok() const { return rc == HOISDF_OK; }
+  static constexpr int SMALL_DW_MAX = 16;
+  hoisdf_small_dw_item small_dw[SMALL_DW_MAX];
+  int n_small_dw = 0;
+  EmuReduceList reduces;
 };
+
+inline void flush_small_dw(Ctx& c) {
+  const int n = c.n_small_dw;
+  c.n_small_dw = 0;
+  if (n > 0 && c.ok()) c.rc = hoisdf_linear_bwd_weight_emu_small_batch(c.small_dw, n, c.stream);
+}
+inline void flush_reduces(Ctx& c) {
+  const int n = c.reduces.n;
+  c.reduces.n = 0;
+  if (n > 0 && c.ok()) c.rc = emu_reduce_launch(c.reduces.r, n, c.st);
+}
+inline void flush_deferred(Ctx& c) { flush_small_dw(c); flush_reduces(c); }
 
 inline bool emu_small(const Ctx& c, long M, const float* a, long lda, const float* W, long ldw, int N, int K) {
   if (!c.emu || M > hoisdf_linear_emu_small_max_rows() || N % 4 || K % 4 || lda % 4 || ldw % 4) return false;
@@ -103,13 +119,14 @@
     float* w = c.ws->floats(nws > 4 ? nws : 4);
     if (!c.dry) {
       if (!w) { c.rc = HOISDF_ERR_WORKSPACE; return; }
-      if (dy_mag || x_mag) c.rc = linear_bwd_weight_emu_mag(dy, lddy, bits, p, x, ldx, dW, K_pad, db, M, N, K_pad, w, nws, dy_mag, x_mag, c.stream);
-      else c.rc = hoisdf_linear_bwd_weight_emu(dy, lddy, bits, p, x, ldx, dW, K_pad, db, M, N, K_pad, w, nws, c.stream);
+      c.rc = linear_bwd_weight_emu_chain(dy, lddy, bits, p, x, ldx, dW, K_pad, db, M, N, K_pad, w, nws, dy_mag, x_mag, c.stream, &c.reduces);
     }
     return;
   }
   if (c.emu && M <= hoisdf_linear_emu_small_max_rows()) {
-    if (!c.dry) c.rc = hoisdf_linear_bwd_weight_emu_small(dy, lddy, bits, p, x, ldx, dW, K_pad, db, M, N, K_pad, c.stream);
+    if (c.dry) return;
+    if (c.n_small_dw == Ctx::SMALL_DW_MAX) flush_small_dw(c);
+    if (c.ok()) c.small_dw[c.n_small_dw++] = hoisdf_small_dw_item{dy, lddy, bits, p, x, ldx, dW, K_pad, db, M, N, K_pad};
     return;
   }
   long nws = 0; float* w = nullptr;
diff --git a/hoisdf_amd/csrc/common.h b/hoisdf_amd/csrc/common.h
--- a/hoisdf_amd/csrc/common.h
+++ b/hoisdf_amd/csrc/common.h
@@ -115,6 +115,13 @@
 int linear_bwd_weight_emu_mag(const float* dy, int lddy, const uint32_t* relu_bits, float drop_p, const float* x, int ldx, float* dW, int lddw,
                               float* db, long M, int N, int K, float* workspace, long workspace_floats, const uint32_t* dy_mag,
                               const uint32_t* x_mag, void* stream);
+struct EmuReduce { const float* part; long stride; int splits; float* out; long n; };
+constexpr int EMU_REDUCE_GROUP = 16;
+struct EmuReduceList { EmuReduce r[2 * EMU_REDUCE_GROUP]; int n = 0; };
+int emu_reduce_launch(const EmuReduce* r, int n, hipStream_t st);
+int linear_bwd_weight_emu_chain(const float* dy, int lddy, const uint32_t* relu_bits, float drop_p, const float* x, int ldx, float* dW, int lddw,
+                                float* db, long M, int N, int K, float* workspace, long workspace_floats, const uint32_t* dy_mag,
+                                const uint32_t* x_mag, void* stream, EmuReduceList* defer);
 int project_gather_fwd_mag(const hoisdf_pyramid* pyr, const float* points, const int32_t* sample_idx, long n_rows, int rows_per_sample,
                            const float* center, const float* cam_intr, float scale, int img_h, int img_w, float* feat, int ldf, float* cam_out,
                            float* uv_out, uint32_t* feat_mag, void* stream);
diff --git a/hoisdf_amd/csrc/gemm_emu.h b/hoisdf_amd/csrc/gemm_emu.h
--- a/hoisdf_amd/csrc/gemm_emu.h
+++ b/hoisdf_amd/csrc/gemm_emu.h
@@ -352,5 +352,5 @@
 int emu_h2_launch(EmuArgs g, hipStream_t st);
 int dw_tile(int K);
 void plan_dw(long M, int N, int K, int& splitk, int& mper);
-int emu_dw_launch(const DwArgs& g, bool h2, float* dW, float* db, float* workspace, hipStream_t st);
+int emu_dw_launch(const DwArgs& g, bool h2, float* dW, float* db, float* workspace, hipStream_t st, EmuReduceList* defer = nullptr);
 }
diff --git a/hoisdf_amd/csrc/gemm_emu.hip b/hoisdf_amd/csrc/gemm_emu.hip
--- a/hoisdf_amd/csrc/gemm_emu.hip
+++ b/hoisdf_amd/csrc/gemm_emu.hip
@@ -276,7 +276,7 @@
 namespace {
 int bwd_weight_emu(const float* dy, int lddy, const uint32_t* relu_bits, float drop_p, const float* x, int ldx, float* dW, int lddw,
                    float* db, long M, int N, int K, float* workspace, long workspace_floats, bool h2, const uint32_t* dy_mag,
-                   const uint32_t* x_mag, void* stream) {
+                   const uint32_t* x_mag, void* stream, EmuReduceList* defer = nullptr) {
   HOISDF_REQUIRE(dW && (M == 0 || (dy && x)), HOISDF_ERR_INVALID, "linear_bwd_weight_emu: null pointer");
   HOISDF_REQUIRE(M > 0 && N > 0 && K > 0 && lddy >= N && ldx >= K && lddw == K && M < (1L << 31) && drop_p >= 0.f && drop_p < 1.f,
                  HOISDF_ERR_INVALID, "linear_bwd_weight_emu: bad sizes (a dense dW, lddw == K, is required)");
@@ -316,8 +316,16 @@
       g.x_amax = part;
     }
   }
-  return emu_dw_launch(g, h2, dW, db, workspace, st);
-}
+  return emu_dw_launch(g, h2, dW, db, workspace, st, defer);
+}
+}
+
+int hoisdf::linear_bwd_weight_emu_chain(const float* dy, int lddy, const uint32_t* relu_bits, float drop_p, const float* x, int ldx, float* dW,
+                                        int lddw, float* db, long M, int N, int K, float* workspace, long workspace_floats,
+                                        const uint32_t* dy_mag, const uint32_t* x_mag, void* stream, EmuReduceList* defer) {
+  const bool mags = dy_mag || x_mag;
+  return bwd_weight_emu(dy, lddy, relu_bits, drop_p, x, ldx, dW, lddw, db, M, N, K, workspace, workspace_floats, mags && form_h2(),
+                        mags ? dy_mag : nullptr, mags ? x_mag : nullptr, stream, defer);
 }
 
 extern "C" int hoisdf_linear_bwd_weight_emu(const float* dy, int lddy, const uint32_t* relu_bits, float drop_p, const float* x,
diff --git a/hoisdf_amd/csrc/gemm_emu_dw.hip b/hoisdf_amd/csrc/gemm_emu_dw.hip
--- a/hoisdf_amd/csrc/gemm_emu_dw.hip
+++ b/hoisdf_amd/csrc/gemm_emu_dw.hip
@@ -1,4 +1,5 @@
 #include "gemm_emu.h"
+#include "launch_tables.h"
 
 namespace hoisdf {
 
@@ -464,14 +465,22 @@
   DW_EPILOGUE(DT, acc[i][j][r] * (MASK ? post * unscale : unscale));
 }
 
-__global__ __launch_bounds__(1024) void emu_reduce_partials_kernel(const float* __restrict__ part, long stride, int splits,
-                                                                   float* __restrict__ out, long n, int blocks0,
-                                                                   const float* __restrict__ part1, long stride1,
-                                                                   float* __restrict__ out1, long n1) {
+struct ReduceGroup {
+  EmuReduce r[EMU_REDUCE_GROUP];
+  int end[EMU_REDUCE_GROUP];
+};
+__global__ __launch_bounds__(1024) void emu_reduce_partials_kernel(ReduceGroup grp) {
   __shared__ float4 red[16][64];
   const int lane = threadIdx.x & 63, w = threadIdx.x >> 6;
-  int blk = blockIdx.x;
-  if (blk >= blocks0) { blk -= blocks0; part = part1; stride = stride1; out = out1; n = n1; }
+  int which = 0;
+#pragma unroll
+  for (int j = 0; j < EMU_REDUCE_GROUP - 1; ++j) which += (int)(blockIdx.x >= (unsigned)grp.end[j]);
+  const EmuReduce& e = grp.r[which];
+  const int blk = (int)blockIdx.x - (which ? grp.end[which - 1] : 0);
+  const float* __restrict__ part = e.part;
+  float* __restrict__ out = e.out;
+  const long stride = e.stride, n = e.n;
+  const int splits = e.splits;
   const long i = ((long)blk * 64 + lane) * 4;
   float4 s = make_float4(0.f, 0.f, 0.f, 0.f);
   if (i < n) {
@@ -499,6 +508,21 @@
     }
     *reinterpret_cast<float4*>(out + i) = t;
   }
+}
+
+int emu_reduce_launch(const EmuReduce* r, int n, hipStream_t st) {
+  for (int gi = 0; gi < launch_groups(n, EMU_REDUCE_GROUP); ++gi) {
+    int first, len;
+    launch_group(n, EMU_REDUCE_GROUP, gi, first, len);
+    ReduceGroup grp{};
+    long count[EMU_REDUCE_GROUP] = {};
+    for (int j = 0; j < len; ++j) { grp.r[j] = r[first + j]; count[j] = (r[first + j].n + 255) / 256; }
+    const long nblk = block_prefix<EMU_REDUCE_GROUP>(count, len, grp.end);
+    HOISDF_REQUIRE(nblk > 0, HOISDF_ERR_INVALID, "linear_bwd_weight_emu reduce: bad reduction table");
+    hipLaunchKernelGGL(emu_reduce_partials_kernel, dim3((unsigned)nblk), dim3(1024), 0, st, grp);
+    if (int rc = check_launch("linear_bwd_weight_emu reduce")) return rc;
+  }
+  return HOISDF_OK;
 }
 
 int dw_tile(int K) { return K <= 128 ? 128 : 256; }
@@ -514,7 +538,7 @@
   splitk = cdiv(M, mper);
 }
 
-int emu_dw_launch(const DwArgs& g, bool h2, float* dW, float* db, float* workspace, hipStream_t st) {
+int emu_dw_launch(const DwArgs& g, bool h2, float* dW, float* db, float* workspace, hipStream_t st, EmuReduceList* defer) {
   const int dtk = dw_tile(g.K);
   const unsigned lb = 2u * (3 * 2 * DT + 3 * 2 * 128) * 16u;
   static bool attr_set = false;
@@ -538,10 +562,18 @@
   if (int rc = check_launch("linear_bwd_weight_emu")) return rc;
   if (g.splitk > 1) {
     const long n = (long)g.N * g.K;
-    const int b0 = (int)((n + 255) / 256), b1 = db ? (g.N + 255) / 256 : 0;
-    hipLaunchKernelGGL(emu_reduce_partials_kernel, dim3((unsigned)(b0 + b1)), dim3(1024), 0, st, workspace, n, g.splitk, dW, n, b0,
-                       workspace + (size_t)g.splitk * g.N * g.K, (long)g.N, db, (long)g.N);
-    return check_launch("linear_bwd_weight_emu reduce");
+    EmuReduce r[2];
+    int nr = 1;
+    r[0] = EmuReduce{workspace, n, g.splitk, dW, n};
+    if (db) r[nr++] = EmuReduce{workspace + (size_t)g.splitk * g.N * g.K, (long)g.N, g.splitk, db, (long)g.N};
+    if (!defer) return emu_reduce_launch(r, nr, st);
+    constexpr int cap = (int)(sizeof(defer->r) / sizeof(defer->r[0]));
+    if (defer->n + nr > cap) {
+      const int held = defer->n;
+      defer->n = 0;
+      if (int rc = emu_reduce_launch(defer->r, held, st)) return rc;
+    }
+    for (int j = 0; j < nr; ++j) defer->r[defer->n++] = r[j];
   }
   return HOISDF_OK;
 }
diff --git a/hoisdf_amd/csrc/gemm_emu_small.hip b/hoisdf_amd/csrc/gemm_emu_small.hip
--- a/hoisdf_amd/csrc/gemm_emu_small.hip
+++ b/hoisdf_amd/csrc/gemm_emu_small.hip
@@ -1,4 +1,5 @@
 #include "gemm_emu.h"
+#include "launch_tables.h"
 
 namespace hoisdf {
 namespace {
@@ -117,12 +118,25 @@
   int M, N, K;
 };
 
-__global__ __launch_bounds__(256) void emu_small_dw_kernel(SmallDwArgs g) {
+constexpr int SMALL_DW_GROUP = 8;
+struct SmallDwGroup {
+  SmallDwArgs p[SMALL_DW_GROUP];
+  int end[SMALL_DW_GROUP];
+};
+
+__global__ __launch_bounds__(256) void emu_small_dw_kernel(SmallDwGroup grp) {
   __shared__ float red[3][16][64];
   __shared__ float rdb[4][32];
   const int lane = threadIdx.x & 63, wave = threadIdx.x >> 6;
   const int l31 = lane & 31, kh = lane >> 5;
-  const int n0 = blockIdx.y * 32, k0 = blockIdx.x * 32;
+  int which = 0;
+#pragma unroll
+  for (int i = 0; i < SMALL_DW_GROUP - 1; ++i) which += (int)(blockIdx.x >= (unsigned)grp.end[i]);
+  const SmallDwArgs& g = grp.p[which];
+  const int tile = (int)blockIdx.x - (which ? grp.end[which - 1] : 0);
+  const int tiles_k = (g.K + 31) / 32;
+  const int bx = tile % tiles_k, by = tile / tiles_k;
+  const int n0 = by * 32, k0 = bx * 32;
   const int ncol = min(n0 + l31, g.N - 1), kcol = min(k0 + l31, g.K - 1);
   const bool nvalid = n0 + l31 < g.N, kvalid = k0 + l31 < g.K;
   const int nslab = (g.M + 15) / 16;
@@ -175,7 +189,7 @@
     const int n = n0 + (r & 3) + 8 * (r >> 2) + 4 * kh, k = k0 + l31;
     if (n < g.N && k < g.K) g.dW[(size_t)n * g.lddw + k] = v * sc;
   }
-  if (g.db && blockIdx.x == 0 && kh == 0 && nvalid) g.db[n0 + l31] = (((rdb[0][l31] + rdb[1][l31]) + rdb[2][l31]) + rdb[3][l31]) * sc;
+  if (g.db && bx == 0 && kh == 0 && nvalid) g.db[n0 + l31] = (((rdb[0][l31] + rdb[1][l31]) + rdb[2][l31]) + rdb[3][l31]) * sc;
 }
 }
 }
@@ -227,17 +241,39 @@
   return check_launch("linear_bwd_input_emu_small");
 }
 
+extern "C" int hoisdf_linear_bwd_weight_emu_small_batch(const hoisdf_small_dw_item* items, int n, void* stream) {
+  HOISDF_REQUIRE(n >= 0 && (n == 0 || items), HOISDF_ERR_INVALID, "linear_bwd_weight_emu_small_batch: null item table");
+  for (int i = 0; i < n; ++i) {
+    const hoisdf_small_dw_item& t = items[i];
+    HOISDF_REQUIRE(t.dW && t.dy && t.x, HOISDF_ERR_INVALID, "linear_bwd_weight_emu_small: null pointer (item %d)", i);
+    HOISDF_REQUIRE(t.M > 0 && t.M <= hoisdf_linear_emu_small_max_rows() && t.N > 0 && t.K > 0 && t.lddy >= t.N && t.ldx >= t.K && t.lddw >= t.K &&
+                       t.drop_p >= 0.f && t.drop_p < 1.f,
+                   HOISDF_ERR_INVALID, "linear_bwd_weight_emu_small: bad sizes (item %d)", i);
+  }
+  for (int gi = 0; gi < launch_groups(n, SMALL_DW_GROUP); ++gi) {
+    int first, len;
+    launch_group(n, SMALL_DW_GROUP, gi, first, len);
+    SmallDwGroup grp{};
+    long count[SMALL_DW_GROUP] = {};
+    for (int j = 0; j < len; ++j) {
+      const hoisdf_small_dw_item& t = items[first + j];
+      SmallDwArgs& g = grp.p[j];
+      g.dy = t.dy; g.lddy = t.lddy; g.x = t.x; g.ldx = t.ldx; g.bits = t.relu_bits; g.ldbits = (t.N + 31) / 32;
+      g.ascale = t.relu_bits ? 1.f / (1.f - t.drop_p) : 1.f;
+      g.dW = t.dW; g.lddw = t.lddw; g.db = t.db; g.M = (int)t.M; g.N = t.N; g.K = t.K;
+      count[j] = (long)cdiv(t.K, 32) * cdiv(t.N, 32);
+    }
+    const long nblk = block_prefix<SMALL_DW_GROUP>(count, len, grp.end);
+    HOISDF_REQUIRE(nblk > 0, HOISDF_ERR_INVALID, "linear_bwd_weight_emu_small_batch: too many tiles");
+    hipLaunchKernelGGL(emu_small_dw_kernel, dim3((unsigned)nblk), dim3(256), 0, as_stream(stream), grp);
+    if (int rc = check_launch("linear_bwd_weight_emu_small")) return rc;
+  }
+  return HOISDF_OK;
+}
+
 extern "C" int hoisdf_linear_bwd_weight_emu_small(const float* dy, int lddy, const uint32_t* relu_bits, float drop_p, const float* x,
                                                   int ldx, float* dW, int lddw, float* db, long M, int N, int K, void* stream) {
   HOISDF_REQUIRE(dW && (M == 0 || (dy && x)), HOISDF_ERR_INVALID, "linear_bwd_weight_emu_small: null pointer");
-  HOISDF_REQUIRE(M > 0 && M <= hoisdf_linear_emu_small_max_rows() && N > 0 && K > 0 && lddy >= N && ldx >= K && lddw >= K &&
-                     drop_p >= 0.f && drop_p < 1.f,
-                 HOISDF_ERR_INVALID, "linear_bwd_weight_emu_small: bad sizes");
-  SmallDwArgs g{};
-  g.dy = dy; g.lddy = lddy; g.x = x; g.ldx = ldx; g.bits = relu_bits; g.ldbits = (N + 31) / 32;
-  g.ascale = relu_bits ? 1.f / (1.f - drop_p) : 1.f;
-  g.dW = dW; g.lddw = lddw; g.db = db; g.M = (int)M; g.N = N; g.K = K;
-  const dim3 grid((unsigned)cdiv(K, 32), (unsigned)cdiv(N, 32));
-  hipLaunchKernelGGL(emu_small_dw_kernel, grid, dim3(256), 0, as_stream(stream), g);
-  return check_launch("linear_bwd_weight_emu_small");
-}
+  const hoisdf_small_dw_item t{dy, lddy, relu_bits, drop_p, x, ldx, dW, lddw, db, M, N, K};
+  return hoisdf_linear_bwd_weight_emu_small_batch(&t, 1, stream);
+}
diff --git a/hoisdf_amd/csrc/heads.hip b/hoisdf_amd/csrc/heads.hip
--- a/hoisdf_amd/csrc/heads.hip
+++ b/hoisdf_amd/csrc/heads.hip
@@ -119,6 +119,7 @@
     c.rc = hoisdf_token_build_bwd_ordered(dtok, s.fea, F, sdf, beta, dfea, F, dbeta, part, B, P, S, row0, D, stream);
   }
   mlp_backward(c, mlp, G, feat, mlp->dims[0], M, s.mlp, dfea, F, dfeat, mlp->dims[0], accumulate_dfeat);
+  flush_deferred(c);
   if (c.ok() && !dry && ws.overflow) { set_error("tokens_bwd: workspace too small"); return HOISDF_ERR_WORKSPACE; }
   return c.rc;
 }
@@ -214,6 +215,7 @@
   const int E = mv->dims[0];
   mlp_backward(c, mv, Gv, enc, E, M, s.vote, doff, 3 * J, denc, E, 0);
   mlp_backward(c, mc, Gc, enc, E, M, s.cl, dcls, J, denc, E, 1, enc_mag(c, mv, enc, E, M, s.vote));
+  flush_deferred(c);
   if (c.ok() && !dry && ws.overflow) { set_error("heads_vote_bwd: workspace too small"); return HOISDF_ERR_WORKSPACE; }
   return c.rc;
 }
diff --git a/hoisdf_amd/csrc/launch_tables.h b/hoisdf_amd/csrc/launch_tables.h
--- /dev/null
+++ b/hoisdf_amd/csrc/launch_tables.h
@@ -0,0 +1,24 @@
+#pragma once
+
+namespace hoisdf {
+
+template <int CAP>
+inline long block_prefix(const long* count, int n, int (&end)[CAP]) {
+  if (n < 0 || n > CAP) return -1;
+  long total = 0;
+  for (int i = 0; i < n; ++i) {
+    if (count[i] < 0 || count[i] > 0x7fffffffL - total) return -1;
+    total += count[i];
+    end[i] = (int)total;
+  }
+  for (int i = n; i < CAP; ++i) end[i] = (int)total;
+  return total;
+}
+
+inline void launch_group(int n, int cap, int g, int& first, int& len) {
+  first = g * cap;
+  len = first >= n ? 0 : (n - first < cap ? n - first : cap);
+}
+inline int launch_groups(int n, int cap) { return n <= 0 ? 0 : (n + cap - 1) / cap; }
+
+}
diff --git a/hoisdf_amd/csrc/layers.hip b/hoisdf_amd/csrc/layers.hip
--- a/hoisdf_amd/csrc/layers.hip
+++ b/hoisdf_amd/csrc/layers.hip
@@ -256,6 +256,7 @@
     lin_bwd_weight(c, dkv, 2 * E, nullptr, 0.f, x, E, G->dw_in + (size_t)E * E, G->db_in ? G->db_in + E : nullptr, Ms, 2 * E, E);
     if (!dry && c.ok()) c.rc = rows_copy_add(dx, (long)g.S * E, dxq, (long)g.nq * E, g.B, g.nq, E, 1, c.st);
   }
+  flush_deferred(c);
   if (c.ok() && !dry && ws.overflow) { set_error("encoder_layer_bwd: workspace too small"); return HOISDF_ERR_WORKSPACE; }
   return c.rc;
 }
@@ -440,7 +441,8 @@
   float* dx2 = ws.floats(M * E); float* df = ws.floats(M * E); float* dh = ws.floats(M * F);
   float* dx1 = ws.floats(M * E); float* da2 = ws.floats(M * E); float* do2 = ws.floats(M * E); float* dq2 = ws.floats(M * E);
   float* dkv = ws.floats(Ms * 2 * E); float* delta = ws.floats((long)g.B * g.H * g.Q); float* dtq2 = ws.floats(M * E);
-  float* da1 = ws.floats(M * E); float* do1 = ws.floats(M * E); float* dqk = ws.floats(M * 2 * E); float* dv = ws.floats(M * E);
+  float* da1 = ws.floats(M * E); float* do1 = ws.floats(M * E);
+  float* dqk = ws.floats(M * 3 * E); float* dv = dqk ? dqk + M * 2 * E : nullptr;
   float* dtq1 = ws.floats(M * E);
   if (!dry && (!dx2 || !df || !dh || !dx1 || !da2 || !do2 || !dq2 || !dkv || !delta || !dtq2 || !da1 || !do1 || !dqk || !dv || !dtq1)) {
     set_error("decoder_layer_bwd: workspace too small");
@@ -467,7 +469,7 @@
   lin_bwd_input(c, da1, E, nullptr, 0.f, w->sa_w_out, E, nullptr, do1, E, M, E, E, 0);
   lin_bwd_weight(c, da1, E, nullptr, 0.f, s.o1, E, G->dsa_w_out, G->dsa_b_out, M, E, E);
   if (!dry && c.ok()) {
-    if (hipMemsetAsync(dqk, 0, sizeof(float) * M * 2 * E, c.st) != hipSuccess || hipMemsetAsync(dv, 0, sizeof(float) * M * E, c.st) != hipSuccess) {
+    if (hipMemsetAsync(dqk, 0, sizeof(float) * M * 3 * E, c.st) != hipSuccess) {
       set_error("decoder_layer_bwd: clearing the self-attention gradients failed");
       return HOISDF_ERR_LAUNCH;
     }
@@ -482,6 +484,7 @@
     hipLaunchKernelGGL(sum_bcast_grad_kernel, dim3((unsigned)cdiv((long)g.Q * (E / 4), 256)), dim3(256), 0, c.st, d_qpos, dtq1, dtq2, g.B, g.Q, E / 4);
     c.rc = check_launch("decoder_layer query_pos gradient");
   }
+  flush_deferred(c);
   if (c.ok() && !dry && ws.overflow) { set_error("decoder_layer_bwd: workspace too small"); return HOISDF_ERR_WORKSPACE; }
   return c.rc;
 }
diff --git a/hoisdf_amd/csrc/sdf_query.hip b/hoisdf_amd/csrc/sdf_query.hip
--- a/hoisdf_amd/csrc/sdf_query.hip
+++ b/hoisdf_amd/csrc/sdf_query.hip
@@ -281,6 +281,7 @@
   lin_bwd_weight(c, dha, HID0, s.ba, 0.f, s.feat, C, G->d_sdfin_w0, G->d_sdfin_b0, n, HID0, C, 0, mg(BM_DHA), fm(TM_FEAT));
   if (!dry && c.ok() && dpyr)
     c.rc = hoisdf_project_gather_bwd(dpyr, points, sample_idx, n, rps, center, cam_intr, scale, img_h, img_w, dfeat, C, stream);
+  flush_deferred(c);
   if (c.ok() && !dry && ws.overflow) { set_error("sdf_query_bwd: workspace too small"); return HOISDF_ERR_WORKSPACE; }
   return c.rc;
 }
diff --git a/include/hoisdf.h b/include/hoisdf.h
--- a/include/hoisdf.h
+++ b/include/hoisdf.h
@@ -107,6 +107,16 @@
                                       float* dx, int lddx, long M, int N, int K, int accumulate, void* stream);
 int hoisdf_linear_bwd_weight_emu_small(const float* dy, int lddy, const uint32_t* relu_bits, float drop_p, const float* x, int ldx,
                                        float* dW, int lddw, float* db, long M, int N, int K, void* stream);
+typedef struct hoisdf_small_dw_item {
+  const float* dy; int lddy;
+  const uint32_t* relu_bits;
+  float drop_p;
+  const float* x; int ldx;
+  float* dW; int lddw;
+  float* db;
+  long M; int N, K;
+} hoisdf_small_dw_item;
+int hoisdf_linear_bwd_weight_emu_small_batch(const hoisdf_small_dw_item* items, int n, void* stream);
 long hoisdf_linear_bwd_weight_emu_workspace(long M, int N, int K);
 int hoisdf_linear_bwd_weight_emu(const float* dy, int lddy, const uint32_t* relu_bits, float drop_p, const float* x, int ldx,
                                  float* dW, int lddw, float* db, long M, int N, int K, float* workspace, long workspace_floats,
```
